# MasterNobody/x264vfw

Hardware: AMD Instinct MI355X
Metric: 1080p yuv420p frames/sec at preset=medium as the device runs it (see config.toolset_gaps), hot path on MI355X (higher is better)
Workload: dtype u8

## Files before the change

include/x264gpu.h:

```cpp
#ifndef X264GPU_H
#define X264GPU_H
#include <stdint.h>
#include <stddef.h>

#ifdef __cplusplus
extern "C" {
#endif

#define X264GPU_ABI_VERSION 2
enum { X264GPU_OK = 0, X264GPU_EINVAL = -1, X264GPU_EHIP = -2, X264GPU_ENOMEM = -3, X264GPU_ENODEV = -4 };

int  x264gpu_abi_version(void);
int  x264gpu_device_count(void);
int  x264gpu_set_device(int dev);
int  x264gpu_get_device(int *dev);
const char *x264gpu_last_error(void);
int  x264gpu_malloc(void **d_ptr, size_t bytes);
int  x264gpu_free(void *d_ptr);
int  x264gpu_memcpy_h2d(void *d_dst, const void *h_src, size_t bytes, void *stream);
int  x264gpu_memcpy_d2h(void *h_dst, const void *d_src, size_t bytes, void *stream);
int  x264gpu_memcpy_d2d(void *d_dst, const void *d_src, size_t bytes, void *stream);
int  x264gpu_memset(void *d_dst, int value, size_t bytes, void *stream);
int  x264gpu_stream_sync(void *stream);
int  x264gpu_stream_create(void **stream);
int  x264gpu_stream_destroy(void *stream);
int  x264gpu_event_create(void **event);
int  x264gpu_event_destroy(void *event);
int  x264gpu_event_record(void *event, void *stream);
int  x264gpu_event_sync(void *event);
int  x264gpu_stream_wait_event(void *stream, void *event);

int x264gpu_pixel_metric(int metric, const uint8_t *d_a, const uint8_t *d_b, int n, int w, int h,
                         int32_t *d_out, void *stream);
int x264gpu_pixel_var(const uint8_t *d_a, int n, int w, int h, uint64_t *d_out, void *stream);
int x264gpu_pixel_hadamard_ac(const uint8_t *d_a, int n, int w, int h, uint64_t *d_out, void *stream);

int x264gpu_dctq4x4(const uint8_t *d_enc, const uint8_t *d_pred, int n, int qp, int list,
                    int16_t *d_coef, int16_t *d_levels, uint8_t *d_recon, void *stream);
int x264gpu_dctq8x8(const uint8_t *d_enc, const uint8_t *d_pred, int n, int qp, int list,
                    int16_t *d_coef, int16_t *d_levels, uint8_t *d_recon, void *stream);

int x264gpu_intra_predict(int kind, const uint8_t *d_plane, int stride, const int32_t *d_xy,
                          const int32_t *d_mode, const int32_t *d_avail, int n, uint8_t *d_out, void *stream);

int x264gpu_hpel_filter(uint8_t *d_planes, size_t plane_bytes, int stride, int w, int h, int pad, void *stream);
int x264gpu_lowres(const uint8_t *d_src, int ss, int w, int h, uint8_t *d_dst, size_t plane_bytes, int ds,
                   void *stream);
int x264gpu_mc_luma(const uint8_t *d_planes00, size_t plane_bytes, int stride, const int32_t *d_xy,
                    const int32_t *d_mv, int n, int w, int h, uint8_t *d_out, void *stream);
int x264gpu_mc_chroma(const uint8_t *d_nv12_00, int stride, const int32_t *d_xy, const int32_t *d_mv,
                      int n, int w, int h, uint8_t *d_out, void *stream);
int x264gpu_mc_avg(const uint8_t *d_a, const uint8_t *d_b, size_t bytes, int weight1, uint8_t *d_out, void *stream);
int x264gpu_trellis_blocks(const int16_t *d_coefs, int nblk, int cat, int qp, int intra, const uint8_t *d_states460, int16_t *d_levels, uint8_t *d_nz, void *stream);
int x264gpu_trellis_blocks_ex(const int16_t *d_coefs, int nblk, int cat, int qp, int intra, const uint8_t *d_states460, int16_t *d_levels, uint8_t *d_nz, int force_general,
                              uint8_t *d_paths, void *stream);
int x264gpu_trellis_blocks_psy(const int16_t *d_coefs, const int16_t *d_fenc_dct, int nblk, int cat, int qp, int intra, int psy_trellis_q8, const uint8_t *d_states460,
                               int16_t *d_levels, uint8_t *d_nz, int force_general, uint8_t *d_paths, void *stream);
int x264gpu_mc_weight(const uint8_t *d_src, size_t bytes, int scale, int denom, int offset, uint8_t *d_out, void *stream);
int x264gpu_gather_rows(const void *const *d_rows, size_t row_bytes, void *d_dst, int rows, void *stream);
int x264gpu_cabac_level_walk(const int16_t *d_levels, const int32_t *d_what, int n, const uint32_t *d_r, const uint32_t *d_r8, uint32_t *d_r_out, uint32_t *d_r8_out, int32_t *d_bits, void *stream);

enum { X264GPU_CSP_MASK = 0xff, X264GPU_CSP_I420 = 1, X264GPU_CSP_YV12 = 2, X264GPU_CSP_YV16 = 3, X264GPU_CSP_YV24 = 4,
       X264GPU_CSP_NV12 = 5, X264GPU_CSP_YUYV = 6, X264GPU_CSP_UYVY = 7, X264GPU_CSP_BGR = 8, X264GPU_CSP_BGRA = 9,
       X264GPU_CSP_VFLIP = 0x1000 };
long x264gpu_csp_img_fill(int csp, int width, int height, long off[3], int stride[3]);
int x264gpu_csp_to_i420(const uint8_t *const d_src[3], const int src_stride[3], int csp, int width, int height,
                        int colmatrix709, int fullrange, uint8_t *const d_dst[3], const int dst_stride[3], void *stream);
int x264gpu_csp_to_i420_batch(const uint8_t *const d_src[3], const int src_stride[3], size_t src_frame_bytes, int csp, int width,
                              int height, int colmatrix709, int fullrange, uint8_t *const d_dst[3], const int dst_stride[3],
                              size_t dst_frame_bytes, int frames, void *stream);

enum { X264GPU_MB_I4x4 = 0, X264GPU_MB_I8x8 = 1, X264GPU_MB_I16x16 = 2, X264GPU_MB_P_L0 = 4, X264GPU_MB_P_8x8 = 5,
       X264GPU_MB_P_SKIP = 6,
       X264GPU_MB_B_DIRECT = 7, X264GPU_MB_B_SKIP = 8, X264GPU_MB_B_INTER = 9, X264GPU_MB_B_8x8 = 10 };
enum { X264GPU_SLICE_P = 0, X264GPU_SLICE_B = 1, X264GPU_SLICE_I = 2 ,
       X264GPU_SLICE_I_NONIDR = 3  };

typedef struct x264gpu_mb {
    uint8_t  type;
    union {
    uint8_t  i16_mode;
    uint8_t  direct8;
    };
    uint8_t  chroma_mode;
    uint8_t  qp;
    uint8_t  cbp_luma;
    uint8_t  cbp_chroma;
    uint8_t  partition;
    int8_t   ref[4];
    union {
    uint8_t  i4_mode[16];
    int8_t   ref1[4];
    };
    uint8_t  transform8x8;
    int16_t  mv[4][2];
    uint32_t nnz;
    union {
    struct {
    int32_t  cost;
    int32_t  aux[3];
    };
    int16_t  mv1[4][2];
    };
} x264gpu_mb;

#define X264GPU_MB_LEVELS 416
#define X264GPU_LV_LUMA 0
#define X264GPU_LV_LUMA_DC 256
#define X264GPU_LV_CHROMA_DC 272
#define X264GPU_LV_CHROMA_AC 280

typedef struct x264gpu_encoder x264gpu_encoder;

typedef struct x264gpu_config {
    int width, height;
    int streams;
    int refs;
    int qp_i, qp_p;
    int me_range;
    int subme;
    int deblock;
    int deblock_alpha, deblock_beta;
    int chroma_qp_offset;
    int deadzone_inter, deadzone_intra;
    int dct_decimate;
    int partitions;
    int dct8x8;
    int me_method;
    int chroma_me;
    int mixed_refs;
    int aq_mode;
    float aq_strength;
    int fast_pskip;
    int mv_range;
    int cabac;
    int rd;
    int psy;
    int psy_rd_q8;
    int slices;
    int trellis;
    int slices_plain;
    int dpb;
    int weightb;
    int psy_trellis_q8;
} x264gpu_config;

#define X264GPU_MAX_LIST 8
typedef struct x264gpu_pic {
    int slice_type;
    int qp;
    int poc;
    int dst;
    int keep;
    int nref[2];
    int8_t slot[2][X264GPU_MAX_LIST];
    struct { int8_t on, denom; int16_t scale, offset; } wl0[X264GPU_MAX_LIST];
    int blind_dupe;
    float qpm;
    struct { int8_t on[2], denom, pad; int16_t scale[2], offset[2]; } wc0[X264GPU_MAX_LIST];
    int direct_temporal, direct_auto;
} x264gpu_pic;

int  x264gpu_encoder_direct_scores(x264gpu_encoder *enc, int *h_scores);
int  x264gpu_encoder_create(x264gpu_encoder **enc, const x264gpu_config *cfg);
int  x264gpu_encoder_create_view(x264gpu_encoder **enc, x264gpu_encoder *parent);
void x264gpu_encoder_destroy(x264gpu_encoder *enc);
int  x264gpu_encoder_mb_count(const x264gpu_encoder *enc);
int  x264gpu_encode_frames(x264gpu_encoder *enc, const uint8_t *d_i420, int slice_type,
                           x264gpu_mb *d_mb, int16_t *d_levels, void *stream);
int  x264gpu_encode_pictures(x264gpu_encoder *enc, const uint8_t *d_i420, const x264gpu_pic *pics,
                             x264gpu_mb *d_mb, int16_t *d_levels, void *stream);
typedef struct x264gpu_level_index { uint32_t at, groups; } x264gpu_level_index;
int  x264gpu_pack_levels(int16_t *d_levels, int streams, int mb_count, x264gpu_level_index *d_index, uint32_t *d_kept , void *stream);
int x264gpu_encoder_deblock_pictures(x264gpu_encoder *e, const uint8_t *d_i420, const x264gpu_mb *d_mb, uint8_t *d_out, void *stream);
int  x264gpu_encoder_get_recon(x264gpu_encoder *enc, int stream_idx, uint8_t *d_i420_out, void *stream);
int  x264gpu_encoder_get_recon_slot(x264gpu_encoder *enc, int stream_idx, int slot, uint8_t *d_i420_out, void *stream);
typedef struct x264gpu_quality { uint64_t ssd[3]; double ssim_sum; uint32_t ssim_cnt, pad; } x264gpu_quality;
#define X264GPU_QUALITY_PSNR 1
#define X264GPU_QUALITY_SSIM 2
int x264gpu_picture_quality(const uint8_t *d_a, const uint8_t *d_b, int n, int w, int h, int flags, x264gpu_quality *d_out, void *stream);
int x264gpu_encoder_quality(x264gpu_encoder *enc, int flags, x264gpu_quality *d_out , void *stream);
typedef struct x264gpu_nr_offsets { uint16_t off[3][64]; } x264gpu_nr_offsets;
typedef struct x264gpu_nr_sums { uint64_t sum[3][64]; uint32_t count[3], pad; } x264gpu_nr_sums;
int x264gpu_encoder_set_nr(x264gpu_encoder *enc, const x264gpu_nr_offsets *d_off , x264gpu_nr_sums *d_pic );
int x264gpu_nr_update(x264gpu_nr_offsets *d_off, x264gpu_nr_sums *d_state, const x264gpu_nr_sums *d_pic, int streams, int strength, void *stream);
int x264gpu_denoise_blocks(int16_t *d_coefs, int nblk, int cat, const x264gpu_nr_offsets *d_off, x264gpu_nr_sums *d_out, void *stream);
int  x264gpu_encoder_stage_count(void);
const char *x264gpu_encoder_stage_name(int i);
int  x264gpu_encoder_profile_begin(x264gpu_encoder *enc, int max_calls);
int  x264gpu_encoder_set_debug(x264gpu_encoder *enc, void *d_counters);
int  x264gpu_mb_kernels_seen(uint32_t *ids, int max, int reset);
int  x264gpu_encoder_profile_end(x264gpu_encoder *enc, void *stream, double *ms_sum, int *launches);
int  x264gpu_encoder_set_qp(x264gpu_encoder *enc, int qp_i, int qp_p);
int  x264gpu_encoder_set_mb_qp_offsets(x264gpu_encoder *enc, const float *d_offsets);
int  x264gpu_encoder_set_stream_qps(x264gpu_encoder *enc, const int8_t *qps);
int  x264gpu_encoder_set_stream_qpms(x264gpu_encoder *enc, const int8_t *qps, const float *qpms);
int  x264gpu_encoder_set_qpm(x264gpu_encoder *enc, float qpm);
int  x264gpu_encoder_set_lowres_mvs(x264gpu_encoder *enc, const int16_t *d_mvs);
int  x264gpu_encoder_set_lowres_mvs1(x264gpu_encoder *enc, const int16_t *d_mvs);
int  x264gpu_encoder_cabac_states(x264gpu_encoder *enc, int stream, int slice, uint8_t *out460);

typedef struct x264gpu_slicetype x264gpu_slicetype;
int  x264gpu_slicetype_create(x264gpu_slicetype **st, int width, int height, int streams, int slots, int bframes, int me_method, int subme, int me_range,
                              int weightb, int mv_range, int do_edges );
void x264gpu_slicetype_destroy(x264gpu_slicetype *st);
int  x264gpu_slicetype_put_frame(x264gpu_slicetype *st, int slot, const uint8_t *d_i420, void *stream);
int  x264gpu_slicetype_frame_cost(x264gpu_slicetype *st, int slot_p0, int slot_p1, int slot_b, int d0, int d1, int32_t *h_score, void *stream);
int  x264gpu_slicetype_frame_cost_w(x264gpu_slicetype *st, int slot_p0, int slot_p1, int slot_b, int d0, int d1, int on, int scale, int denom, int offset, int32_t *h_score, void *stream);
int  x264gpu_slicetype_intra_mbs(x264gpu_slicetype *st, int slot, int d0, int stream_idx);
int  x264gpu_slicetype_cost_est(x264gpu_slicetype *st, int slot, int d0, int d1, int stream_idx);
const int16_t  *x264gpu_slicetype_lowres_mvs(x264gpu_slicetype *st, int slot, int list, int dist);
const int      *x264gpu_slicetype_lowres_mv_costs(x264gpu_slicetype *st, int slot, int list, int dist);
const int      *x264gpu_slicetype_intra_costs(x264gpu_slicetype *st, int slot);
// ... 31 lines not shown
```

x264vfw_amd/csrc/cabac_layout.hip.h:

```cpp
#pragma once

namespace x264gpu {

__host__ __device__ inline bool cab_locate(int ctx, int &reg, int &lane, int &sh)
{
    const int sig_off[6] = { 105, 120, 134, 149, 152, 402 }, last_off[6] = { 166, 181, 195, 210, 213, 417 }, abs_off[6] = { 227, 237, 247, 257, 266, 426 };
    const int n_sig[6] = { 15, 14, 15, 3, 14, 15 }, n_last[6] = { 15, 14, 15, 3, 14, 9 }, n_abs[6] = { 10, 10, 10, 9, 10, 10 }, byte_of[6] = { 3, 1, 0, 3, 2, 0 };
    if (ctx < 105) { reg = 0; lane = ctx >> 2; sh = (ctx & 3) * 8; return true; }
    if (ctx >= 399 && ctx <= 401) { const int c = ctx - 399 + 105; reg = 0; lane = c >> 2; sh = (c & 3) * 8; return true; }
    for (int cat = 0; cat < 6; cat++) {
        int role = -1, i = 0;
        if (ctx >= sig_off[cat] && ctx < sig_off[cat] + n_sig[cat]) { role = 0; i = ctx - sig_off[cat]; }
        else if (ctx >= last_off[cat] && ctx < last_off[cat] + n_last[cat]) { role = 1; i = ctx - last_off[cat]; }
        else if (ctx >= abs_off[cat] && ctx < abs_off[cat] + n_abs[cat]) { role = 2; i = ctx - abs_off[cat]; }
        if (role < 0) continue;
        reg = cat == 5 ? 2 : 1; sh = 8 * byte_of[cat];
        lane = cat == 3 ? (role == 0 ? 48 + i : role == 1 ? 52 + i : 55 + i) : role * 16 + i;
        return true;
    }
    return false;
}

}
```

x264vfw_amd/csrc/cabac_rd.hip.h:

```cpp
#pragma once
#include <type_traits>
#include "enc_common.hip.h"
#include "cabac_layout.hip.h"
#define CABAC_TABLE static __constant__ const
#define CABAC_NAMESPACE x264gpu_cabac
#include "../host/cabac_tables.hpp"
#undef CABAC_TABLE
#undef CABAC_NAMESPACE

#ifndef CAB_WALK_BINS
#define CAB_WALK_BINS 8
#endif
namespace x264gpu {

static __constant__ const uint16_t c_cabac_entropy[128] = {
#include "cabac_entropy.inc"
};

struct Cab { uint32_t a, r, r8; int f8; int f8v; };

__device__ __forceinline__ uint32_t cab_model(int lane)
{
    return (uint32_t)c_cabac_entropy[2 * lane] | ((uint32_t)c_cabac_entropy[2 * lane + 1] << 9) | ((uint32_t)x264gpu_cabac::cabac_trans_lps[lane] << 20);
}

__device__ __forceinline__ int cab_total(const Cab &cb) { return cb.f8 + wave_sum(cb.f8v); }

__device__ __forceinline__ void cab_init(Cab &cb, int lane, bool pslice, int qp)
{
    namespace T = x264gpu_cabac;
    qp = min(max(qp, 0), 51);
    uint32_t w[3] = { 0, 0, 0 };
    auto seed = [&](int ctx) {
        int m = 0, n = 0;
        if (ctx < 276) { const T::CabacInitRow row = T::cabac_init_0_275[ctx]; m = pslice ? row.mp : row.mi; n = pslice ? row.np : row.ni; }
        else { const T::CabacInitRow row = T::cabac_init_399_435[ctx - 399]; m = pslice ? row.mp : row.mi; n = pslice ? row.np : row.ni; }
        const int pre = min(max(((m * qp) >> 4) + n, 1), 126);
        return (uint32_t)(pre <= 63 ? (63 - pre) << 1 : ((pre - 64) << 1) | 1);
    };
    for (int j = 0; j < 4; j++) {
        const int c = lane * 4 + j;
        if (c < 105) w[0] |= seed(c) << (8 * j); else if (c < 108) w[0] |= seed(399 + c - 105) << (8 * j);
    }
    {
        const int role = lane >> 4, i = lane & 15;
        const int sig_off[5] = { 105, 120, 134, 149, 152 }, last_off[5] = { 166, 181, 195, 210, 213 }, abs_off[5] = { 227, 237, 247, 257, 266 }, n1[5] = { 15, 14, 15, 3, 14 };
        const int cats[3] = { 2, 1, 4 };
        for (int b = 0; b < 3; b++) {
            const int cat = cats[b];
            if (role == 0 && i < n1[cat]) w[1] |= seed(sig_off[cat] + i) << (8 * b);
            else if (role == 1 && i < n1[cat]) w[1] |= seed(last_off[cat] + i) << (8 * b);
            else if (role == 2 && i < 10) w[1] |= seed(abs_off[cat] + i) << (8 * b);
        }
        if (lane < 48) {
            if (role == 0 && i < 15) w[1] |= seed(105 + i) << 24; else if (role == 1 && i < 15) w[1] |= seed(166 + i) << 24; else if (role == 2 && i < 10) w[1] |= seed(227 + i) << 24;
        } else {
            const int l = lane - 48;
            if (l < 3) w[1] |= seed(149 + l) << 24; else if (l >= 4 && l < 7) w[1] |= seed(210 + l - 4) << 24; else if (l >= 7) w[1] |= seed(257 + l - 7) << 24;
        }
        if (role == 0 && i < 15) w[2] = seed(402 + i); else if (role == 1 && i < 9) w[2] = seed(417 + i); else if (role == 2 && i < 10) w[2] = seed(426 + i);
    }
    cb.a = w[0]; cb.r = w[1]; cb.r8 = w[2]; cb.f8 = 0; cb.f8v = 0;
}

__device__ __forceinline__ void cab_bin(Cab &cb, uint32_t model, int lane, int ctx, int bin)
{
    ctx = __builtin_amdgcn_readfirstlane(ctx >= 399 ? ctx - 399 + 105 : ctx); bin = __builtin_amdgcn_readfirstlane(bin);
    const int li = ctx >> 2, sh = (ctx & 3) * 8;
    const uint32_t w = __builtin_amdgcn_readlane(cb.a, li);
    const int st = (w >> sh) & 255, sg = st >> 1, mps = st & 1;
    const uint32_t t = __builtin_amdgcn_readlane(model, sg);
    const bool lps = (mps ^ bin) != 0;
    cb.f8 += lps ? (t >> 9) & 0x7ff : t & 0x1ff;
    const int ns = lps ? (int)(t >> 20) : min(sg + 1, 62);
    const int nm = lps && sg == 0 ? mps ^ 1 : mps;
    const uint32_t nw = (w & ~(255u << sh)) | ((uint32_t)((ns << 1) | nm) << sh);
    cb.a = lane == li ? nw : cb.a;
}
__device__ __forceinline__ void cab_bypass(Cab &cb, int n = 1) { cb.f8 += 256 * n; }
__device__ __forceinline__ void cab_ue_bypass(Cab &cb, int k, int v)
{
    int n = 0;
    while (v >= (1 << k)) { n++; v -= 1 << k; k++; }
    cb.f8 += 256 * (n + 1 + k);
}

__device__ __forceinline__ void cab_step(int &st, int &f8v, uint32_t model, bool mine, int bin)
{
    const int sg = st >> 1, mps = st & 1;
    const uint32_t t = (uint32_t)__builtin_amdgcn_ds_bpermute(sg << 2, (int)model);
    const bool lps = (mps ^ bin) != 0;
    const int cost = lps ? (t >> 9) & 0x7ff : t & 0x1ff;
    const int ns = lps ? (int)(t >> 20) : min(sg + 1, 62);
    const int nm = lps && sg == 0 ? mps ^ 1 : mps;
    f8v += mine ? cost : 0;
    st = mine ? (ns << 1) | nm : st;
}

struct CabLv {
    int cat0;
    unsigned nz0;
    unsigned nzac;
    unsigned nzdc;
    bool ldc;
};

__device__ __forceinline__ int wave_scan_add(int v)
{
    v += __builtin_amdgcn_update_dpp(0, v, 0x111, 0xf, 0xf, false);
    v += __builtin_amdgcn_update_dpp(0, v, 0x112, 0xf, 0xf, false);
    v += __builtin_amdgcn_update_dpp(0, v, 0x114, 0xf, 0xf, false);
    v += __builtin_amdgcn_update_dpp(0, v, 0x118, 0xf, 0xf, false);
    v += __builtin_amdgcn_update_dpp(0, v, 0x142, 0xa, 0xf, false);
    v += __builtin_amdgcn_update_dpp(0, v, 0x143, 0xc, 0xf, false);
    return v;
}
__device__ __forceinline__ int cab_mbcnt(unsigned long long m) { return (int)__builtin_amdgcn_mbcnt_hi((unsigned)(m >> 32), __builtin_amdgcn_mbcnt_lo((unsigned)m, 0u)); }

#define CAB_CHAIN_ENTRIES (511 * 128)
template <int LN>
__device__ __forceinline__ void cab_writelane3(unsigned &lo, unsigned &hi, int &n, unsigned long long val, int nval)
{
    asm("s_nop 1\n\tv_writelane_b32 %0, %3, %6\n\tv_writelane_b32 %1, %4, %6\n\tv_writelane_b32 %2, %5, %6"
        : "+v"(lo), "+v"(hi), "+v"(n) : "s"((unsigned)val), "s"((unsigned)(val >> 32)), "s"(nval), "n"(LN));
}
struct CabChain { int sg, mps; };
__device__ __forceinline__ void cab_run_mps(CabChain &c, int &f8, int cumv, int m62, int n)
{
    const int hi = min(c.sg + n, 62);
    f8 += __builtin_amdgcn_readlane(cumv, hi) - __builtin_amdgcn_readlane(cumv, c.sg) + (c.sg + n - hi) * m62;
    c.sg = hi;
}
__device__ __forceinline__ void cab_one_lps(CabChain &c, int &f8, uint32_t model)
{
    const uint32_t t = (uint32_t)__builtin_amdgcn_readlane((int)model, c.sg);
    f8 += (int)((t >> 9) & 0x7ff);
    c.mps ^= c.sg == 0 ? 1 : 0;
    c.sg = (int)(t >> 20);
}

template <int LANE0, class PROF>
__device__ __forceinline__ void cab_strings_c1(int a, int c1, unsigned &blo, unsigned &bhi, int &N, PROF &pf)
{
    unsigned long long cur[5];
    int pushed[5];
#pragma unroll
    for (int v = 0; v < 5; v++) {
        const bool member = a != 0 && c1 == v;
        cur[v] = __ballot(member);
        pushed[v] = __builtin_amdgcn_ds_permute((member ? cab_mbcnt(cur[v]) : 63) << 2, member && a > 1 ? 1 : 0);
    }
    if (cur[0]) { pf.count(20); cab_writelane3<LANE0 + 0>(blo, bhi, N, __ballot(pushed[0] != 0), __builtin_popcountll(cur[0])); }
    if (cur[1]) { pf.count(20); cab_writelane3<LANE0 + 1>(blo, bhi, N, __ballot(pushed[1] != 0), __builtin_popcountll(cur[1])); }
    if (cur[2]) { pf.count(20); cab_writelane3<LANE0 + 2>(blo, bhi, N, __ballot(pushed[2] != 0), __builtin_popcountll(cur[2])); }
    if (cur[3]) { pf.count(20); cab_writelane3<LANE0 + 3>(blo, bhi, N, __ballot(pushed[3] != 0), __builtin_popcountll(cur[3])); }
    if (cur[4]) { pf.count(20); cab_writelane3<LANE0 + 4>(blo, bhi, N, __ballot(pushed[4] != 0), __builtin_popcountll(cur[4])); }
}
template <int LANE0, int V, class PROF>
__device__ __forceinline__ void cab_strings_cg(int a, int a15, int cg, unsigned &blo, unsigned &bhi, int &N, unsigned long long &serial, PROF &pf)
{
    const bool member = a > 1 && cg == V;
    if (__ballot(member)) {
        pf.count(20);
        const int incl = wave_scan_add(member ? (a15 < 15 ? a15 - 1 : 13) : 0);
        const int total = __builtin_amdgcn_readlane(incl, 63);
        if (total <= 63) {
            const bool closes = member && a15 < 15;
            const int pushed = __builtin_amdgcn_ds_permute((closes ? incl - 1 : 63) << 2, closes ? 1 : 0);
            cab_writelane3<LANE0 + V>(blo, bhi, N, ((1ull << total) - 1ull) & ~__ballot(pushed != 0), total);
        } else serial |= 1ull << (V - 5);
    }
    if constexpr (V < 9 && LANE0 + V + 1 < 64) cab_strings_cg<LANE0, V + 1>(a, a15, cg, blo, bhi, N, serial, pf);
}

template <class PROF>
__device__ __forceinline__ void cab_levels_all(Cab &cb, uint32_t model, int lane, const int16_t *lvs, const CabLv &W, const uint32_t *ctab, PROF &pf)
{
    if (W.cat0 < 0 && !W.nzac && !W.nzdc && !W.ldc) return;
    lane = relane(lane);
    const int cumv = wave_scan_add((int)(model & 0x1ff)) - (int)(model & 0x1ff);
    const int m62 = (int)(__builtin_amdgcn_readlane((int)model, 62) & 0x1ff);
    int f8 = 0;
    auto group = [&](auto a_of, int nwords, unsigned wordmask, int gshift, uint32_t &reg, int sh, auto lane0_tag, int bac, int ncm1, int sigbase, int lastbase) {
        constexpr int LANE0 = decltype(lane0_tag)::value;
        for (int w = 0; w < nwords; w++) {
            if (!((wordmask >> w) & 1u)) continue;
            const int a = a_of(w);
            const unsigned long long nzm = __ballot(a != 0);
            if (!nzm) continue;
            const unsigned long long m1 = __ballot(a == 1), mg = nzm & ~m1;
            int ngt, n1;
            if (gshift == 6) { ngt = cab_mbcnt(mg); n1 = cab_mbcnt(m1); }
            else {
                const int base = lane & ~((1 << gshift) - 1);
                const unsigned sel = (1u << (lane - base)) - 1u;
                ngt = __builtin_popcount((unsigned)(mg >> base) & sel); n1 = __builtin_popcount((unsigned)(m1 >> base) & sel);
            }
            const int node = ngt == 0 ? min(n1, 3) : min(3 + ngt, 7);
            const int c1 = node < 4 ? node + 1 : 0, cg = node < 4 ? 5 : node + 2;
            cb.f8v += a ? 256 + (a >= 15 ? 256 * (2 * (31 - __builtin_clz(a - 14)) + 1) : 0) : 0;
            const int a15 = min(a, 15);
            pf.count(21, __builtin_popcountll(nzm));
            unsigned blo = 0, bhi = 0; int N = 0;
            cab_strings_c1<LANE0>(a, c1, blo, bhi, N, pf);
            unsigned long long serial = 0;
            if (mg) cab_strings_cg<LANE0, 5>(a, a15, cg, blo, bhi, N, serial, pf);
            if (ncm1) {
                const int nslots = 1 << gshift;
                const bool is_s = lane >= sigbase && lane < sigbase + ncm1, is_l = lane >= lastbase && lane < lastbase + ncm1;
                const int pp = is_s ? lane - sigbase : lane - lastbase;
                const int sbit = min(max(nslots - 1 - (pp + bac), 0), 31);
                for (int j = 0; j < (gshift == 4 ? 4 : gshift == 2 ? 2 : 1); j++) {
                    const unsigned field = (unsigned)(nzm >> (j * nslots)) & ((1u << nslots) - 1u);
                    if (!field) continue;
                    const int lastp = nslots - 1 - __builtin_ctz(field) - bac;
                    const unsigned nzb = (field >> sbit) & 1u;
                    const bool cond = is_s ? pp <= lastp : is_l && nzb && pp <= lastp;
                    const unsigned bit = is_s ? nzb : (pp == lastp ? 1u : 0u);
                    blo |= cond ? bit << N : 0u; N += cond ? 1 : 0;
                }
            }
            {
                int st = (int)((reg >> sh) & 255u);
                unsigned long long B = ((unsigned long long)bhi << 32) | blo;
                while (__ballot(N > 0)) {
                    const int k = min(N, CAB_WALK_BINS);
                    const uint32_t e = ctab[((((1 << k) - 1) + ((int)(unsigned)B & ((1 << k) - 1))) << 7) + st];
                    st = (int)(e & 127u); cb.f8v += (int)(e >> 7);
                    B >>= k; N -= k;
                }
                reg = (reg & ~(255u << sh)) | ((uint32_t)st << sh);
            }
            for (int v = 5; serial && v < 10; v++) {
                if (!((serial >> (v - 5)) & 1ull)) continue;
                unsigned long long cur = __ballot(a > 1 && cg == v);
                const int stv = (__builtin_amdgcn_readlane((int)reg, LANE0 + v) >> sh) & 255;
                CabChain c = { stv >> 1, stv & 1 };
                while (cur) {
                    pf.count(20);
                    const int f = __builtin_ctzll(cur);
                    cur &= cur - 1ull;
                    const int av = __builtin_amdgcn_readlane(a15, f);
                    int ones = av - 2;
                    while (ones > 0) {
                        if (c.mps) { cab_run_mps(c, f8, cumv, m62, ones); ones = 0; }
                        else { cab_one_lps(c, f8, model); ones--; }
                    }
                    if (av != 15) { if (c.mps) cab_one_lps(c, f8, model); else cab_run_mps(c, f8, cumv, m62, 1); }
                }
                const uint32_t nst = (uint32_t)((c.sg << 1) | c.mps);
                reg = lane == LANE0 + v ? (reg & ~(255u << sh)) | (nst << sh) : reg;
            }
        }
    };
    const int g = lane >> 4, q = lane & 15;
    if (W.cat0 == 5)
        group([&](int w) { const int pos = 63 - lane; return abs((int)lvs[(w * 4 + (pos & 3)) * 16 + (pos >> 2)]); }, 4, W.nz0 & 15u, 6, cb.r8, 0, std::integral_constant<int, 32>{}, 0, 0, 0, 0);
    else if (W.cat0 >= 0) {
        const bool ac = W.cat0 == 1;
        const unsigned wm = ((W.nz0 & 0xfu) ? 1u : 0u) | ((W.nz0 & 0xf0u) ? 2u : 0u) | ((W.nz0 & 0xf00u) ? 4u : 0u) | ((W.nz0 & 0xf000u) ? 8u : 0u);
        group([&](int w) { const int blk = 4 * w + g, pos = 15 - q; return ((W.nz0 >> blk) & 1u) && !(ac && pos == 0) ? abs((int)lvs[blk * 16 + pos]) : 0; }, 4, wm, 4, cb.r, ac ? 8 : 0, std::integral_constant<int, 32>{}, ac ? 1 : 0, ac ? 14 : 15, 0, 16);
    }
    if (W.ldc) group([&](int) { return lane < 16 ? abs((int)lvs[X264GPU_LV_LUMA_DC + 15 - lane]) : 0; }, 1, 1u, 4, cb.r, 24, std::integral_constant<int, 32>{}, 0, 15, 0, 16);
    if (W.nzdc) group([&](int) { return lane < 8 && ((W.nzdc >> (lane >> 2)) & 1u) ? abs((int)lvs[X264GPU_LV_CHROMA_DC + (lane >> 2) * 4 + 3 - (lane & 3)]) : 0; }, 1, 1u, 2, cb.r, 24, std::integral_constant<int, 55>{}, 0, 3, 48, 52);
    if (W.nzac) {
        const unsigned wm = ((W.nzac & 0xfu) ? 1u : 0u) | ((W.nzac & 0xf0u) ? 2u : 0u);
        group([&](int w) { const int blk = 4 * w + g, pos = 15 - q; return ((W.nzac >> blk) & 1u) && pos ? abs((int)lvs[X264GPU_LV_CHROMA_AC + blk * 16 + pos]) : 0; }, 2, wm, 4, cb.r, 16, std::integral_constant<int, 32>{}, 1, 14, 0, 16);
    }
    cb.f8 += f8;
}

template <int CAT>
__device__ __forceinline__ void cab_block4(Cab &cb, int &st, uint32_t model, int lane, int coef)
{
    constexpr int n1 = CAT == 3 ? 3 : (CAT == 1 || CAT == 4) ? 14 : 15;
    constexpr int sig0 = CAT == 3 ? 48 : 0, last0 = CAT == 3 ? 52 : 16;
    const unsigned long long mask = __ballot(coef != 0);
    const int last = 63 - __builtin_clzll(mask);
    const bool is_s = lane >= sig0 && lane < sig0 + n1, is_l = lane >= last0 && lane < last0 + n1;
    const int p = is_s ? lane - sig0 : lane - last0;
    const int nzp = (int)((mask >> (p & 63)) & 1);
    cab_step(st, cb.f8v, model, (is_s && p <= last) || (is_l && nzp && p <= last), is_s ? nzp : p == last);
}

static __constant__ const unsigned long long c_cabac_pos8[24] = {
#include "cabac_masks8x8.inc"
};

__device__ __forceinline__ void cab_block8(Cab &cb, int &st, uint32_t model, int lane, int coef, bool size)
{
    const unsigned long long mask = __ballot(coef != 0);
    const int last = 63 - __builtin_clzll(mask);
    const unsigned long long upto = last < 63 ? (2ull << last) - 1 : 0x7fffffffffffffffull;
    unsigned long long mine = 0;
    if (lane < 15) mine = c_cabac_pos8[lane] & upto;
    else if (lane >= 16 && lane < 25) mine = c_cabac_pos8[15 + lane - 16] & upto & mask;
    while (__ballot(mine != 0)) {
        const bool have = mine != 0;
        const int i = have ? (size ? 63 - __builtin_clzll(mine) : __builtin_ctzll(mine)) : 0;
        cab_step(st, cb.f8v, model, have, lane < 15 ? (int)((mask >> i) & 1) : i == last);
        mine &= ~(1ull << i);
    }
}

struct CabIn {
    bool pslice, left, top, size;
    int nref, t8mode;
    int type, part, t8, cbp_luma, cbp_chroma, i16mode, cmode, qp, last_qp, last_dqp;
    unsigned nnz;
    int ltype, ttype, lcbp_luma, tcbp_luma, lcbp_chroma, tcbp_chroma, lcmode, tcmode, lt8, tt8;
    unsigned lnnz, tnnz;
    unsigned long long lamvd, tamvd;
    bool bslice; int nref1; unsigned buse;
    int b_r0, b_x0, b_y0, b_r1, b_x1, b_y1;
    unsigned long long lamvd1, tamvd1;
    int pm, pm_b0, pm_b1, pm_dx, pm_dy, pm_sx, pm_sy;
    int pm_lists, pm_dx1, pm_dy1, pm_sx1, pm_sy1;
    unsigned pm_nnzc;
};

static __constant__ const uint8_t c_btype_len[24] = { 1, 3, 3, 6, 6, 6, 6, 6, 6, 6, 6, 6, 7, 7, 7, 7, 7, 7, 7, 7, 7, 7, 6, 6 };
static __constant__ const uint8_t c_btype_bits[24] = { 0, 1, 5, 3, 35, 19, 51, 11, 43, 27, 59, 31, 7, 71, 39, 103, 23, 87, 55, 119, 15, 79, 63, 47 };
__device__ __forceinline__ bool cab_is_skip(int t) { return t == X264GPU_MB_P_SKIP || t == X264GPU_MB_B_SKIP; }
__device__ __forceinline__ bool cab_is_intra(int t) { return t < X264GPU_MB_P_L0; }

__device__ __forceinline__ int cab_luma_cbf_of(int type, int cbp_luma, int t8, unsigned nnz, int bx, int by)
{
    if (type == X264GPU_MB_P_SKIP || type == X264GPU_MB_B_SKIP) return 0;
    if (!((cbp_luma >> ((by >> 1) * 2 + (bx >> 1))) & 1)) return 0;
    if (t8) return 1;
    return (nnz >> blkidx_of(bx, by)) & 1;
}

__device__ __forceinline__ void cab_mb_type_intra(Cab &cb, uint32_t model, int lane, const CabIn &in, int c0, int c1, int c2, int c3, int c4, int c5)
{
    if (in.type != X264GPU_MB_I16x16) { cab_bin(cb, model, lane, c0, 0); return; }
    cab_bin(cb, model, lane, c0, 1);
    if (in.size) cb.f8 += 7;
    cab_bin(cb, model, lane, c1, in.cbp_luma != 0);
    if (!in.cbp_chroma) cab_bin(cb, model, lane, c2, 0);
    else { cab_bin(cb, model, lane, c2, 1); cab_bin(cb, model, lane, c3, in.cbp_chroma >> 1); }
    cab_bin(cb, model, lane, c4, in.i16mode >> 1);
    cab_bin(cb, model, lane, c5, in.i16mode & 1);
}

__device__ __forceinline__ void cab_mvd(Cab &cb, uint32_t model, int lane, int base, int sum, int val)
{
    const int a = abs(val), inc = (sum > 2) + (sum > 32);
    if (!a) { cab_bin(cb, model, lane, base + inc, 0); return; }
    cab_bin(cb, model, lane, base + inc, 1);
    for (int i = 1; i < min(a, 9); i++) cab_bin(cb, model, lane, base + min(i + 2, 6), 1);
    if (a < 9) cab_bin(cb, model, lane, base + min(a + 2, 6), 0); else cab_ue_bypass(cb, 3, a - 9);
    cab_bypass(cb);
}

template <class PROF>
__device__ __forceinline__ unsigned long long cab_mb(Cab &cb, uint32_t model, int lane, const CabIn &in, MeState &S, const int16_t *lvs,
                                                     const uint8_t *modes4, const uint8_t *modes8, const uint8_t *nmodes, int mbx, int sy, int &dqp_out,
                                                     unsigned long long &amvd1_out, const uint32_t *ctab, PROF &pf)
{
    pf.begin2(); pf.count(16);
    lane = relane(lane);
    amvd1_out = 0;
    unsigned long long amvd = 0;
    dqp_out = 0;
    const bool lavail = in.left, tavail = in.top;
    const bool intra = in.type < X264GPU_MB_P_L0;
    if (!in.pm) {
    if (in.bslice && !in.size) {
        cab_bin(cb, model, lane, 24 + (lavail && !cab_is_skip(in.ltype)) + (tavail && !cab_is_skip(in.ttype)), in.type == X264GPU_MB_B_SKIP);
        if (in.type == X264GPU_MB_B_SKIP) return 0;
    }
    if (in.pslice && !in.bslice && !in.size) {
        cab_bin(cb, model, lane, 11 + (lavail && in.ltype != X264GPU_MB_P_SKIP) + (tavail && in.ttype != X264GPU_MB_P_SKIP), in.type == X264GPU_MB_P_SKIP);
        if (in.type == X264GPU_MB_P_SKIP) return 0;
    }
    if (in.bslice) {
        const int ctx0 = (lavail && in.ltype != X264GPU_MB_B_SKIP && in.ltype != X264GPU_MB_B_DIRECT) + (tavail && in.ttype != X264GPU_MB_B_SKIP && in.ttype != X264GPU_MB_B_DIRECT);
        int value;
        if (intra) value = 23;
        else if (in.type == X264GPU_MB_B_DIRECT) value = 0;
        else if (in.part == D_8x8) value = 22;
        else if (in.part == D_16x16) value = 1 + (int)(in.buse & 3);
        else {
            const int u0 = (int)(in.buse & 3), u1 = (int)((in.part == D_16x8 ? in.buse >> 4 : in.buse >> 2) & 3);
            const int pair = u0 == 0 ? (u1 == 0 ? 0 : u1 == 1 ? 2 : 4) : u0 == 1 ? (u1 == 0 ? 3 : u1 == 1 ? 1 : 5) : 6 + u1;
            value = 4 + 2 * pair + (in.part == D_8x16);
        }
        const int len = c_btype_len[value], bits = c_btype_bits[value];
        for (int i = 0; i < len; i++) cab_bin(cb, model, lane, i == 0 ? 27 + ctx0 : i == 1 ? 27 + 3 : i == 2 ? 27 + 5 - ((bits >> 1) & 1) : 27 + 5, (bits >> i) & 1);
        if (intra) cab_mb_type_intra(cb, model, lane, in, 32, 32 + 1, 32 + 2, 32 + 2, 32 + 3, 32 + 3);
    } else if (!in.pslice) {
        const int ctx = (lavail && in.ltype != X264GPU_MB_I4x4 && in.ltype != X264GPU_MB_I8x8) + (tavail && in.ttype != X264GPU_MB_I4x4 && in.ttype != X264GPU_MB_I8x8);
        cab_mb_type_intra(cb, model, lane, in, 3 + ctx, 3 + 3, 3 + 4, 3 + 5, 3 + 6, 3 + 7);
    } else if (intra) { cab_bin(cb, model, lane, 14, 1); cab_mb_type_intra(cb, model, lane, in, 17, 17 + 1, 17 + 2, 17 + 2, 17 + 3, 17 + 3); }
    else if (in.part == D_8x8) { cab_bin(cb, model, lane, 14, 0); cab_bin(cb, model, lane, 15, 0); cab_bin(cb, model, lane, 16, 1); }
    else {
        cab_bin(cb, model, lane, 14, 0);
        if (in.part == D_16x16) { cab_bin(cb, model, lane, 15, 0); cab_bin(cb, model, lane, 16, 0); }
        else { cab_bin(cb, model, lane, 15, 1); cab_bin(cb, model, lane, 17, in.part == D_16x8); }
    }
    }
    const int t8ctx = 399 + (lavail && in.lt8) + (tavail && in.tt8);
    if (in.pm == 1) {
        if (in.pm_lists & 1) { cab_mvd(cb, model, lane, 40, in.pm_sx, in.pm_dx); cab_mvd(cb, model, lane, 47, in.pm_sy, in.pm_dy); }
        if (in.pm_lists & 2) { cab_mvd(cb, model, lane, 40, in.pm_sx1, in.pm_dx1); cab_mvd(cb, model, lane, 47, in.pm_sy1, in.pm_dy1); }
        if (in.part == D_8x8 && !in.bslice) cab_bin(cb, model, lane, 21, 1);
    } else if (intra) {
        if (in.type != X264GPU_MB_I16x16 && (!in.pm || in.pm == 2 || in.pm == 3)) {
            const bool i8 = in.type == X264GPU_MB_I8x8;
            if (in.t8mode && !in.pm) cab_bin(cb, model, lane, t8ctx, i8);
            int mode = 0, pm = 0;
            if (lane < 16) { const uint8_t *cur = i8 ? modes8 : modes4; mode = cur[lane]; pm = i4_pred_mode(nmodes, mbx, sy, lane, cur); }
            const uint32_t w68 = __builtin_amdgcn_readlane(cb.a, 68 >> 2);
            int stp = lane == 0 ? (int)(w68 & 255) : (int)((w68 >> 8) & 255);
            for (int b = 0; b < 16; b += i8 ? 4 : 1) {
                if (in.pm && b != (i8 ? 4 * in.pm_b0 : in.pm_b0)) continue;
                int m = __builtin_amdgcn_readlane(mode, b);
                const int p = __builtin_amdgcn_readlane(pm, b);
                const bool same = m == p;
                if (m > p) m--;
                cab_step(stp, cb.f8v, model, lane == 0 || (lane == 1 && !same), lane == 0 ? same : m & 1);
                if (!same) { cab_step(stp, cb.f8v, model, lane == 1, (m >> 1) & 1); cab_step(stp, cb.f8v, model, lane == 1, m >> 2); }
            }
            {
                const uint32_t s68 = (uint32_t)__builtin_amdgcn_readlane(stp, 0), s69 = (uint32_t)__builtin_amdgcn_readlane(stp, 1);
                cb.a = lane == (68 >> 2) ? (cb.a & ~0xffffu) | s68 | (s69 << 8) : cb.a;
            }
        }
        if (!in.pm || in.pm == 4) {
        const int ctx = (lavail && in.ltype < X264GPU_MB_P_L0 && in.lcmode != 0) + (tavail && in.ttype < X264GPU_MB_P_L0 && in.tcmode != 0);
        if (!in.cmode) cab_bin(cb, model, lane, 64 + ctx, 0);
        else { cab_bin(cb, model, lane, 64 + ctx, 1); cab_bin(cb, model, lane, 64 + 3, in.cmode > 1); if (in.cmode > 1) cab_bin(cb, model, lane, 64 + 3, in.cmode > 2); }
        }
    } else if (in.bslice) {
        if (in.type != X264GPU_MB_B_DIRECT) {
            const int part = in.part, np = part == D_16x16 ? 1 : part == D_8x8 ? 4 : 2;
            const int w8 = part == D_16x16 || part == D_16x8 ? 2 : 1, h8 = part == D_16x16 || part == D_8x16 ? 2 : 1;
            auto use_of = [&](int kp) { const int b8 = part == D_16x8 ? 2 * kp : kp; return (int)((in.buse >> (2 * b8)) & 3); };
            if (part == D_8x8)
                for (int kp = 0; kp < 4; kp++) {
                    const int u = use_of(kp);
                    if (u == 3) { cab_bin(cb, model, lane, 36, 0); continue; }
                    cab_bin(cb, model, lane, 36, 1);
                    if (u == 2) { cab_bin(cb, model, lane, 37, 1); cab_bin(cb, model, lane, 38, 0); cab_bin(cb, model, lane, 39, 0); cab_bin(cb, model, lane, 39, 0); }
                    else { cab_bin(cb, model, lane, 37, 0); cab_bin(cb, model, lane, 39, u == 1); }
                }
            const int sc0 = S.cref, sc1 = S.cmvx, sc2 = S.cmvy, sc3 = S.cdir;
            for (int l = 0; l < 2; l++) {
                const int go = 16 * l;
                if ((l ? in.nref1 : in.nref) <= 1) continue;
                if (lane == 5 + go || lane == 6 + go || lane == 9 + go || lane == 10 + go) S.cref = -2;
                for (int kp = 0; kp < np; kp++) {
                    const int x8 = part == D_8x16 ? kp : part == D_8x8 ? kp & 1 : 0, y8 = part == D_16x8 ? kp : part == D_8x8 ? kp >> 1 : 0;
                    const int u = use_of(kp), b8 = y8 * 2 + x8, g0 = (y8 + 1) * 4 + x8 + 1 + go;
                    const bool sends = u == 2 || u == l;
                    const int r = rl(l ? in.b_r1 : in.b_r0, b8 * 16);
                    if (sends) {
                        int ctx = (rl(S.cref, g0 - 1) > 0 && !rl(S.cdir, g0 - 1)) + 2 * (rl(S.cref, g0 - 4) > 0 && !rl(S.cdir, g0 - 4));
                        for (int q = r; q > 0; q--) { cab_bin(cb, model, lane, 54 + ctx, 1); ctx = (ctx >> 2) + 4; }
                        cab_bin(cb, model, lane, 54 + ctx, 0);
                    }
                    const bool mine = lane == g0 || (w8 == 2 && lane == g0 + 1) || (h8 == 2 && lane == g0 + 4) || (w8 == 2 && h8 == 2 && lane == g0 + 5);
                    S.cref = mine ? (sends ? r : u == 3 ? r : -1) : S.cref;
                    S.cdir = mine ? (u == 3) : S.cdir;
                }
            }
            unsigned long long amvd1 = 0;
            for (int l = 0; l < 2; l++) {
                const int go = 16 * l;
                if (lane == 5 + go || lane == 6 + go || lane == 9 + go || lane == 10 + go) S.cref = -2;
                unsigned long long am = 0;
                const unsigned long long nl = l ? in.lamvd1 : in.lamvd, nt = l ? in.tamvd1 : in.tamvd;
                for (int kp = 0; kp < np; kp++) {
                    const int x8 = part == D_8x16 ? kp : part == D_8x8 ? kp & 1 : 0, y8 = part == D_16x8 ? kp : part == D_8x8 ? kp >> 1 : 0;
                    const int u = use_of(kp), b8 = y8 * 2 + x8, g0 = (y8 + 1) * 4 + x8 + 1 + go;
                    const bool sends = u == 2 || u == l;
                    const int r = rl(l ? in.b_r1 : in.b_r0, b8 * 16), vx = rl(l ? in.b_x1 : in.b_x0, b8 * 16), vy = rl(l ? in.b_y1 : in.b_y0, b8 * 16);
                    if (sends) {
                        int px, py;
                        mb_predict_mv(S, part, x8, y8, w8, r, px, py, go);
                        for (int comp = 0; comp < 2; comp++) {
                            const int la = x8 > 0 ? (int)((am >> (8 * ((y8 * 2 + x8 - 1) * 2 + comp))) & 255) : lavail ? (int)((nl >> (8 * ((y8 * 2 + 1) * 2 + comp))) & 255) : 0;
                            const int ta = y8 > 0 ? (int)((am >> (8 * (((y8 - 1) * 2 + x8) * 2 + comp))) & 255) : tavail ? (int)((nt >> (8 * ((2 + x8) * 2 + comp))) & 255) : 0;
                            const int d = comp ? vy - py : vx - px;
                            cab_mvd(cb, model, lane, comp ? 47 : 40, la + ta, d);
                            const unsigned long long capped = (unsigned long long)min(abs(d), 66);
                            for (int yy = y8; yy < y8 + h8; yy++) for (int xx = x8; xx < x8 + w8; xx++) am |= capped << (8 * ((yy * 2 + xx) * 2 + comp));
                        }
                    }
                    const bool mine = lane == g0 || (w8 == 2 && lane == g0 + 1) || (h8 == 2 && lane == g0 + 4) || (w8 == 2 && h8 == 2 && lane == g0 + 5);
                    S.cref = mine ? (r >= 0 ? r : -1) : S.cref; S.cmvx = mine ? (r >= 0 ? vx : 0) : S.cmvx; S.cmvy = mine ? (r >= 0 ? vy : 0) : S.cmvy;
                }
                if (l) amvd1 = am; else amvd = am;
            }
            S.cref = sc0; S.cmvx = sc1; S.cmvy = sc2; S.cdir = sc3;
            amvd1_out = amvd1;
        }
    } else {
        const int part = in.part, np = part == D_16x16 ? 1 : part == D_8x8 ? 4 : 2;
        const int w8 = part == D_16x16 || part == D_16x8 ? 2 : 1, h8 = part == D_16x16 || part == D_8x16 ? 2 : 1;
        if (part == D_8x8) for (int kp = 0; kp < 4; kp++) cab_bin(cb, model, lane, 21, 1);
        const int sc0 = S.cref, sc1 = S.cmvx, sc2 = S.cmvy;
        if (lane == 5 || lane == 6 || lane == 9 || lane == 10) S.cref = -2;
        if (in.nref > 1)
            for (int kp = 0; kp < np; kp++) {
                const int x8 = part == D_8x16 ? kp : part == D_8x8 ? kp & 1 : 0, y8 = part == D_16x8 ? kp : part == D_8x8 ? kp >> 1 : 0;
                const int slot = part == D_16x16 ? ME_16 : part == D_16x8 ? ME_16x8 + kp : part == D_8x16 ? ME_8x16 + kp : ME_8 + kp;
                const int r = rl(S.ref, slot), g0 = (y8 + 1) * 4 + x8 + 1;
                int ctx = (rl(S.cref, g0 - 1) > 0) + 2 * (rl(S.cref, g0 - 4) > 0);
                for (int q = r; q > 0; q--) { cab_bin(cb, model, lane, 54 + ctx, 1); ctx = (ctx >> 2) + 4; }
                cab_bin(cb, model, lane, 54 + ctx, 0);
                const bool mine = lane == g0 || (w8 == 2 && lane == g0 + 1) || (h8 == 2 && lane == g0 + 4) || (w8 == 2 && h8 == 2 && lane == g0 + 5);
                S.cref = mine ? r : S.cref;
            }
        else if (lane == 5 || lane == 6 || lane == 9 || lane == 10) S.cref = 0;
        for (int kp = 0; kp < np; kp++) {
            const int x8 = part == D_8x16 ? kp : part == D_8x8 ? kp & 1 : 0, y8 = part == D_16x8 ? kp : part == D_8x8 ? kp >> 1 : 0;
            const int slot = part == D_16x16 ? ME_16 : part == D_16x8 ? ME_16x8 + kp : part == D_8x16 ? ME_8x16 + kp : ME_8 + kp;
            const int r = rl(S.ref, slot), vx = rl(S.mvx, slot), vy = rl(S.mvy, slot), g0 = (y8 + 1) * 4 + x8 + 1;
            int px, py;
            mb_predict_mv(S, part, x8, y8, w8, r, px, py);
            for (int comp = 0; comp < 2; comp++) {
                const int la = x8 > 0 ? (int)((amvd >> (8 * ((y8 * 2 + x8 - 1) * 2 + comp))) & 255) : lavail ? (int)((in.lamvd >> (8 * ((y8 * 2 + 1) * 2 + comp))) & 255) : 0;
                const int ta = y8 > 0 ? (int)((amvd >> (8 * (((y8 - 1) * 2 + x8) * 2 + comp))) & 255) : tavail ? (int)((in.tamvd >> (8 * ((2 + x8) * 2 + comp))) & 255) : 0;
                const int d = comp ? vy - py : vx - px;
                cab_mvd(cb, model, lane, comp ? 47 : 40, la + ta, d);
                const unsigned long long capped = (unsigned long long)min(abs(d), 66);
                for (int yy = y8; yy < y8 + h8; yy++) for (int xx = x8; xx < x8 + w8; xx++) amvd |= capped << (8 * ((yy * 2 + xx) * 2 + comp));
            }
            const bool mine = lane == g0 || (w8 == 2 && lane == g0 + 1) || (h8 == 2 && lane == g0 + 4) || (w8 == 2 && h8 == 2 && lane == g0 + 5);
            S.cmvx = mine ? vx : S.cmvx; S.cmvy = mine ? vy : S.cmvy;
        }
        S.cref = sc0; S.cmvx = sc1; S.cmvy = sc2;
    }
    if (in.pm ? in.pm == 3 : in.type != X264GPU_MB_I16x16)
        for (int b8 = 0; b8 < 4; b8++) {
            const int x = b8 & 1, y = b8 >> 1;
            const int a = x ? !((in.cbp_luma >> (b8 - 1)) & 1) : lavail ? !((in.lcbp_luma >> (b8 + 1)) & 1) : 0;
            const int b = y ? !((in.cbp_luma >> (b8 - 2)) & 1) : tavail ? !((in.tcbp_luma >> (b8 + 2)) & 1) : 0;
            cab_bin(cb, model, lane, 73 + a + 2 * b, (in.cbp_luma >> b8) & 1);
        }
    if (in.pm ? in.pm == 4 : in.type != X264GPU_MB_I16x16) {
        cab_bin(cb, model, lane, 77 + (lavail && in.lcbp_chroma) + 2 * (tavail && in.tcbp_chroma), in.cbp_chroma != 0);
        if (in.cbp_chroma) cab_bin(cb, model, lane, 77 + 4 + (lavail && in.lcbp_chroma == 2) + 2 * (tavail && in.tcbp_chroma == 2), in.cbp_chroma == 2);
    }
    if (!in.pm && !intra && in.t8mode && in.cbp_luma) cab_bin(cb, model, lane, t8ctx, in.t8);
    if (in.pm || in.cbp_luma || in.cbp_chroma || in.type == X264GPU_MB_I16x16) {
        const bool i16 = !in.pm && in.type == X264GPU_MB_I16x16;
        int dqp = in.qp - in.last_qp;
        if (i16 && !in.cbp_luma && !in.cbp_chroma && !((in.nnz >> 24) & 1) && dqp > 0) dqp = 0;
        if (!in.pm) {
        int ctx = in.last_dqp != 0;
        if (dqp) {
            if (dqp < -26) dqp += 52; else if (dqp > 25) dqp -= 52;
            int val = dqp > 0 ? 2 * dqp - 1 : -2 * dqp;
            do { cab_bin(cb, model, lane, 60 + ctx, 1); ctx = 2 + (ctx >> 1); } while (--val);
        }
        cab_bin(cb, model, lane, 60 + ctx, 0);
        dqp_out = dqp;
        }
        pf.mark2(17);
        const int un = intra ? 1 : 0;
        auto luma_in = [&](int bx, int by) { return in.pm ? (int)((in.pm_nnzc >> blkidx_of(bx, by)) & 1) : cab_luma_cbf_of(in.type, in.cbp_luma, in.t8, in.nnz, bx, by); };
        auto luma_inc = [&](int blk) {
            const int bx = z_bx(blk), by = z_by(blk);
            const int a = bx > 0 ? luma_in(bx - 1, by) : lavail ? cab_luma_cbf_of(in.ltype, in.lcbp_luma, in.lt8, in.lnnz, 3, by) : un;
            const int b = by > 0 ? luma_in(bx, by - 1) : tavail ? cab_luma_cbf_of(in.ttype, in.tcbp_luma, in.tt8, in.tnnz, bx, 3) : un;
            return a + 2 * b;
        };
        auto dc_inc = [&](int bit) {
            auto of = [&](bool avail, int type, int cbp_chroma, unsigned nnz) {
                if (!avail) return un;
                if (cab_is_skip(type)) return 0;
                if (bit == 24) return type == X264GPU_MB_I16x16 ? (int)((nnz >> 24) & 1) : 0;
                return cbp_chroma ? (int)((nnz >> bit) & 1) : 0;
            };
            return of(lavail, in.ltype, in.lcbp_chroma, in.lnnz) + 2 * of(tavail, in.ttype, in.tcbp_chroma, in.tnnz);
        };
        auto ac_inc = [&](int pl, int i) {
            const int bx = i & 1, by = i >> 1;
            auto of = [&](int type, int cbp_chroma, unsigned nnz, int x, int y) { return !cab_is_skip(type) && cbp_chroma == 2 ? (int)((nnz >> (16 + pl * 4 + y * 2 + x)) & 1) : 0; };
            auto inside = [&](int x, int y) { return in.pm ? (int)((in.pm_nnzc >> (16 + pl * 4 + y * 2 + x)) & 1) : of(in.type, in.cbp_chroma, in.nnz, x, y); };
            const int a = bx > 0 ? inside(0, by) : lavail ? of(in.ltype, in.lcbp_chroma, in.lnnz, 1, by) : un;
            const int b = by > 0 ? inside(bx, 0) : tavail ? of(in.ttype, in.tcbp_chroma, in.tnnz, bx, 1) : un;
            return a + 2 * b;
        };
        CabLv W = { -1, 0u, 0u, 0u, false };
        auto flush_levels = [&]() { pf.mark2(18); cab_levels_all(cb, model, lane, lvs, W, ctab, pf); pf.mark2(19); W.cat0 = -1; W.nz0 = 0; W.nzac = 0; W.nzdc = 0; W.ldc = false; };
        auto blocks = [&](auto cat_tag, int shift, int nblk, auto coef_of, auto inc_of, auto coded) {
            constexpr int CAT = decltype(cat_tag)::value;
            static_assert(CAT == 0 || CAT == 3, "the DC categories");
            (void)shift;
            for (int b = 0; b < nblk; b++) {
                if (!coded(b)) continue;
                const int coef = coef_of(b);
                const bool nz = __ballot(coef != 0) != 0;
                cab_bin(cb, model, lane, 85 + CAT * 4 + inc_of(b), nz);
                if (nz) { if (CAT == 0) W.ldc = true; else W.nzdc |= 1u << b; }
            }
        };
        auto always = [](int) { return true; };
        auto blocks_many = [&](auto cat_tag, int shift, int nblk, unsigned codedmask, unsigned nzbits, auto coef_of, auto inc_of) {
            constexpr int CAT = decltype(cat_tag)::value;
            const int b_lane = lane & 15;
            const bool mine_blk = lane < nblk && ((codedmask >> b_lane) & 1);
            const int inc = inc_of(b_lane);
            const unsigned long long nzm = (unsigned long long)(nzbits & codedmask);
            unsigned long long seq = 0;
#pragma unroll
            for (int j = 0; j < 4; j++) { const unsigned long long m = __ballot(mine_blk && inc == j); seq = lane == j ? m : seq; }
            const int cbase = 85 + CAT * 4;
            int stc = 0;
#pragma unroll
            for (int j = 0; j < 4; j++) { const int c = cbase + j; const uint32_t w = __builtin_amdgcn_readlane(cb.a, c >> 2); stc = lane == j ? (int)((w >> ((c & 3) * 8)) & 255) : stc; }
            while (__ballot(seq != 0)) {
                const bool have = seq != 0;
                const int b = have ? __builtin_ctzll(seq) : 0;
                cab_step(stc, cb.f8v, model, have, (int)((nzm >> b) & 1));
                seq &= seq - 1;
            }
#pragma unroll
            for (int j = 0; j < 4; j++) {
                const int c = cbase + j, li = c >> 2, sh = (c & 3) * 8;
                const uint32_t v = (uint32_t)__builtin_amdgcn_readlane(stc, j);
                cb.a = lane == li ? (cb.a & ~(255u << sh)) | (v << sh) : cb.a;
            }
            (void)coef_of; (void)shift;
            if (CAT == 4) W.nzac |= (unsigned)nzm; else { W.cat0 = CAT; W.nz0 |= (unsigned)nzm; }
        };
        if (i16) {
            blocks(std::integral_constant<int, 0>{}, 24, 1, [&](int) { return lane < 16 ? (int)lvs[X264GPU_LV_LUMA_DC + lane] : 0; }, [&](int) { return dc_inc(24); }, always);
            if (in.cbp_luma) blocks_many(std::integral_constant<int, 1>{}, 8, 16, 0xffffu, in.nnz & 0xffffu, [&](int b) { return lane < 15 ? (int)lvs[b * 16 + 1 + lane] : 0; }, luma_inc);
        } else if (in.pm == 4) {
        } else if (in.t8) {
            const int pmask = in.pm ? (1 << in.pm_b0) | (in.pm_b1 >= 0 ? 1 << in.pm_b1 : 0) : 15;
            int st = cb.r8 & 255;
            for (int i8 = 0; i8 < 4; i8++)
                if (((in.cbp_luma & pmask) >> i8) & 1) cab_block8(cb, st, model, lane, (int)lvs[(i8 * 4 + (lane & 3)) * 16 + (lane >> 2)], in.size);
            cb.r8 = (uint32_t)st;
            W.cat0 = 5; W.nz0 = (unsigned)(in.cbp_luma & pmask);
        } else {
            unsigned coded = ((in.cbp_luma & 1) ? 0x000fu : 0) | ((in.cbp_luma & 2) ? 0x00f0u : 0) | ((in.cbp_luma & 4) ? 0x0f00u : 0) | ((in.cbp_luma & 8) ? 0xf000u : 0);
            if (in.pm == 1) coded &= (0xfu << (4 * in.pm_b0)) | (in.pm_b1 >= 0 ? 0xfu << (4 * in.pm_b1) : 0u);
            if (in.pm == 2) coded = 1u << in.pm_b0;
            blocks_many(std::integral_constant<int, 2>{}, 0, 16, coded, in.nnz & 0xffffu, [&](int b) { return lane < 16 ? (int)lvs[b * 16 + lane] : 0; }, luma_inc);
        }
        if (in.pm == 1) {
            for (int t = 0; t < 2; t++) {
                const int b8 = t ? in.pm_b1 : in.pm_b0;
                if (b8 < 0) continue;
                blocks_many(std::integral_constant<int, 4>{}, 16, 8, (1u << b8) | (16u << b8), (in.nnz >> 16) & 0xffu, [&](int k) { return lane < 15 ? (int)lvs[X264GPU_LV_CHROMA_AC + k * 16 + 1 + lane] : 0; }, [&](int k) { return ac_inc((k >> 2) & 1, k & 3); });
                flush_levels();
            }
        } else if (in.cbp_chroma && (!in.pm || in.pm == 4)) {
            blocks(std::integral_constant<int, 3>{}, 24, 2, [&](int pl) { return lane < 4 ? (int)lvs[X264GPU_LV_CHROMA_DC + pl * 4 + lane] : 0; }, [&](int pl) { return dc_inc(25 + pl); }, always);
            if (in.cbp_chroma == 2)
                blocks_many(std::integral_constant<int, 4>{}, 16, 8, 0xffu, (in.nnz >> 16) & 0xffu, [&](int k) { return lane < 15 ? (int)lvs[X264GPU_LV_CHROMA_AC + k * 16 + 1 + lane] : 0; }, [&](int k) { return ac_inc((k >> 2) & 1, k & 3); });
        }
        flush_levels();
    }
    return amvd;
}

}
```

x264vfw_amd/csrc/encoder.hip:

```cpp
#include "enc_common.hip.h"
#include "k_encode.hip.h"
#include <stdlib.h>
#include "k_deblock.hip.h"
#include "cabac_layout.hip.h"
#include "quality.hip.h"
#include <math.h>
#include <vector>
#include <string.h>
#include <new>

namespace x264gpu {
void launch_mb_slice_dia(const EncK &k, int streams, bool big_margin, hipStream_t st);
void launch_mb_slice_hex(const EncK &k, int streams, bool big_margin, hipStream_t st);
void launch_mb_slice_umh(const EncK &k, int streams, bool big_margin, hipStream_t st);
void launch_mb_slice_esa(const EncK &k, int streams, bool big_margin, hipStream_t st);
void launch_mb_slice_intra(const EncK &k, int streams, hipStream_t st);
void launch_mb_slice_b_hex(const EncK &k, int streams, hipStream_t st);
void launch_mb_slice_b_dia(const EncK &k, int streams, hipStream_t st);
void launch_mb_slice_b_umh(const EncK &k, int streams, hipStream_t st);
void launch_mb_slice_b_esa(const EncK &k, int streams, hipStream_t st);
void launch_mb_slice_psy(const EncK &k, int streams, int slice_type, hipStream_t st);
void launch_mb_slice_nr(const EncK &k, int streams, int slice_type, hipStream_t st);
void launch_nr_gather(const x264gpu_nr_sums *part, int slices, x264gpu_nr_sums *pic, int streams, hipStream_t st);
int trellis_table_ptrs(const uint16_t **su, const uint8_t **tu, const int **l2);
int cabac_chain_table(const uint32_t **out);
int launch_hpel_filter(uint8_t *planes, size_t plane_bytes, int stride, int w, int h, int pad, int batch,
                       size_t batch_bytes, hipStream_t st);
}
using namespace x264gpu;

struct x264gpu_encoder {
    x264gpu_config cfg;
    EncK k;
    uint8_t *fenc_y = nullptr, *fenc_uv = nullptr;
    uint8_t *luma[8] = {}, *chroma[8] = {};
    int slots = 2, have = 0;
    int16_t *mv16[8] = {};
    uint8_t *mbtype[8] = {};
    int8_t *colref[8] = {}; int16_t *colmv[8] = {};
    int8_t *colref0[8] = {};
    struct DpbMeta { int slot_l0poc[8][8] = {}; int slot_nref[8] = {}, slot_poc[8] = {}, slot_ref0poc[8] = {}; } meta_own, *meta = &meta_own;
    x264gpu_encoder *view_of = nullptr;
    hipStream_t last_stream = nullptr;
    uint8_t *direct_flags = nullptr, *direct_flags_base = nullptr; int direct_flags_sel = 0; int *dscore = nullptr; bool use_direct_flags = false;
    int16_t *mvr[8] = {};
    int poc = 0, ring = 2;
    const int16_t *lowres_mv = nullptr, *lowres_mv1 = nullptr;
    int cur = 0, last = 0;
    unsigned long long *dbg = nullptr;
    uint8_t *tc = nullptr;
    uint8_t *amvd = nullptr;
    uint32_t *cab_out = nullptr;
    int *perm = nullptr; unsigned *wtime = nullptr; bool wt_valid[4] = { false, false, false, false };
    int *sl_stat = nullptr, *sl_rerun = nullptr;
    unsigned long long *prof = nullptr;
    int *wf_progress = nullptr;
    void *qslab = nullptr;
    const x264gpu_nr_offsets *nr_off = nullptr; x264gpu_nr_sums *nr_pic = nullptr, *nr_part = nullptr;
    uint8_t *mbqp = nullptr;
    const float *ext_off = nullptr;
    int8_t *stream_qp = nullptr; float *stream_qpm = nullptr;
    int stream_qp_sel = 0;
    bool use_stream_qp = false;
    float qpm_next = 0.f;
    Q4 *q4tab = nullptr; Q8 *q8tab = nullptr; int *lambda_tab = nullptr; uint16_t *cost_all = nullptr;
    hipEvent_t *ev = nullptr;
    int *ev_mask = nullptr;
    int prof_calls = 0, prof_cap = 0;
};
enum { NSTAGE = 6 };

static const char *const kStageNames[] = { "ingest", "macroblocks", "unused", "settle_qp", "deblock", "hpel_filter" };

static int build_aq_tables(x264gpu_encoder *e)
{
    QuantCfg qc; qc.deadzone_inter = e->cfg.deadzone_inter; qc.deadzone_intra = e->cfg.deadzone_intra;
    std::vector<Q4> q4(52 * 4); std::vector<Q8> q8(52 * 2); std::vector<int> lam(52);
    std::vector<uint16_t> cost((size_t)52 * 2 * MVCOST_HALF);
    for (int qp = 0; qp < 52; qp++) {
        for (int l = 0; l < 4; l++) q4[qp * 4 + l] = make_q4(qp, l, qc);
        for (int l = 0; l < 2; l++) q8[qp * 2 + l] = make_q8(qp, l, qc);
        lam[qp] = lambda_of(qp);
        uint16_t *h = cost.data() + (size_t)qp * 2 * MVCOST_HALF;
        for (int i = 0; i < MVCOST_HALF; i++) {
            const float logs = i ? log2f((float)(i + 1)) * 2.0f + 1.718f : 0.718f;
            int c = (int)((float)lam[qp] * logs + 0.5f);
            if (c > 65535) c = 65535;
            h[MVCOST_HALF + i] = (uint16_t)c; h[MVCOST_HALF - i] = (uint16_t)c;
        }
        h[0] = h[1];
    }
    hipError_t er = hipMalloc((void **)&e->q4tab, q4.size() * sizeof(Q4));
    if (er == hipSuccess) er = hipMalloc((void **)&e->q8tab, q8.size() * sizeof(Q8));
    if (er == hipSuccess) er = hipMalloc((void **)&e->lambda_tab, lam.size() * sizeof(int));
    if (er == hipSuccess) er = hipMalloc((void **)&e->cost_all, cost.size() * sizeof(uint16_t));
    if (er == hipSuccess) er = hipMalloc((void **)&e->mbqp, (size_t)e->cfg.streams * e->k.nmb);
    if (er == hipSuccess) er = hipMemcpy(e->q4tab, q4.data(), q4.size() * sizeof(Q4), hipMemcpyHostToDevice);
    if (er == hipSuccess) er = hipMemcpy(e->q8tab, q8.data(), q8.size() * sizeof(Q8), hipMemcpyHostToDevice);
    if (er == hipSuccess) er = hipMemcpy(e->lambda_tab, lam.data(), lam.size() * sizeof(int), hipMemcpyHostToDevice);
    if (er == hipSuccess) er = hipMemcpy(e->cost_all, cost.data(), cost.size() * sizeof(uint16_t), hipMemcpyHostToDevice);
    if (er != hipSuccess) return set_err(er == hipErrorOutOfMemory ? X264GPU_ENOMEM : X264GPU_EHIP, "aq tables", er);
    return X264GPU_OK;
}

extern "C" {

static int encoder_create_impl(x264gpu_encoder **out, const x264gpu_config *cfg, x264gpu_encoder *parent)
{
    ARG_TRY(out && cfg);
    ARG_TRY(cfg->width >= 16 && cfg->height >= 16 && !(cfg->width & 1) && !(cfg->height & 1) && cfg->streams >= 1);
    ARG_TRY(cfg->qp_i >= 0 && cfg->qp_i <= 51 && cfg->qp_p >= 0 && cfg->qp_p <= 51 && cfg->refs >= 1 && cfg->refs <= 5);
    ARG_TRY(cfg->trellis == 0 || (cfg->trellis > 0 && cfg->trellis < 128 && (cfg->trellis & 63) && cfg->rd && cfg->cabac));
    ARG_TRY(cfg->psy_trellis_q8 == 0 || (cfg->psy_trellis_q8 > 0 && cfg->psy_trellis_q8 <= 640 && cfg->trellis && cfg->cabac && cfg->rd && (cfg->me_method == 1 || cfg->me_method == 2)));
    ARG_TRY(!cfg->rd || (cfg->subme >= 6 && cfg->subme <= 9 && cfg->psy_rd_q8 >= 0 && cfg->psy_rd_q8 <= 2560));
    ARG_TRY(cfg->rd >= 0 && cfg->rd < 128 && (cfg->rd < 2 || (cfg->rd & 1)) && (!(cfg->rd & 62) || (cfg->cabac && cfg->subme >= 8 && (cfg->me_method == 1 || cfg->me_method == 2))));
    ARG_TRY(!cfg->rd || cfg->subme < 8 || (cfg->cabac && (cfg->me_method == 1 || cfg->me_method == 2)));
    ARG_TRY(!(cfg->rd & 64) || (cfg->cabac && (cfg->me_method == 1 || cfg->me_method == 2)));
    ARG_TRY(cfg->dpb == 0 || cfg->subme < 9 || (cfg->rd && cfg->cabac && (cfg->me_method == 1 || cfg->me_method == 2)));
    ARG_TRY(cfg->slices >= 0 && (cfg->slices <= 1 || cfg->slices <= (cfg->height + 15) / 16 / (cfg->slices_plain ? 1 : 4)));
    ARG_TRY(cfg->slices_plain == 0 || cfg->slices_plain == 1);
    ARG_TRY(cfg->width <= 4096 && cfg->height <= 2304 && cfg->me_range >= 4 && cfg->me_range <= (cfg->me_method == 2 ? 64 : 16));
    ARG_TRY(cfg->me_method >= 0 && cfg->me_method <= 3);
    ARG_TRY(cfg->dpb == 0 || (cfg->dpb >= cfg->refs && cfg->dpb <= 7));
    x264gpu_encoder *e = new (std::nothrow) x264gpu_encoder();
    if (!e) return set_err(X264GPU_ENOMEM, "encoder", hipSuccess);
    e->cfg = *cfg;
    EncK &k = e->k;
    memset(&k, 0, sizeof(k));
    k.w = cfg->width; k.h = cfg->height;
    k.mbw = (k.w + 15) / 16; k.mbh = (k.h + 15) / 16; k.nmb = k.mbw * k.mbh;
    k.cw = k.mbw * 16; k.ch = k.mbh * 16;
    k.fs = (k.cw + 63) / 64 * 64;
    k.rs = (k.cw + 2 * PAD + 63) / 64 * 64;
    k.fency_bytes = (size_t)k.fs * k.ch;
    k.fencuv_bytes = (size_t)k.fs * k.ch / 2;
    k.plane_bytes = (size_t)k.rs * (k.ch + 2 * PAD);
    k.luma_bytes = 4 * k.plane_bytes;
    k.cplane_bytes = (size_t)k.rs * (k.ch / 2 + 2 * CPAD);
    k.me_range = cfg->me_range; k.subme = cfg->subme; k.dct_decimate = cfg->dct_decimate;
    k.slices = cfg->slices > 1 ? cfg->slices : 1; k.slices_plain = cfg->slices_plain != 0; k.cabac = cfg->cabac != 0;
    k.rd = cfg->rd; k.psy = cfg->psy != 0; k.psy_rd_q8 = cfg->psy_rd_q8;
    k.partitions = cfg->partitions; k.chroma_qp_offset = cfg->chroma_qp_offset; k.dct8x8 = cfg->dct8x8; k.me_method = cfg->me_method; k.chroma_me = cfg->chroma_me != 0; k.mixed_refs = cfg->mixed_refs != 0;
    k.alpha_off = cfg->deblock_alpha * 2; k.beta_off = cfg->deblock_beta * 2;
    k.deblock_rdo = cfg->deblock && (cfg->rd & 64) ? 1 : 0;
    const size_t S = (size_t)cfg->streams;
    hipError_t er = hipSuccess;
    auto alloc = [&](void **p, size_t n, int fill) {
        if (er != hipSuccess) return;
        er = hipMalloc(p, n);
        if (er == hipSuccess) er = hipMemset(*p, fill, n);
    };
    alloc((void **)&e->fenc_y, S * k.fency_bytes, 0);
    alloc((void **)&e->fenc_uv, S * k.fencuv_bytes, 0);
    e->slots = (cfg->dpb > 0 ? cfg->dpb : cfg->refs) + 1; e->ring = cfg->refs + 1;
    if (parent) {
        e->view_of = parent; e->meta = &parent->meta_own;
        for (int i = 0; i < 8; i++) { e->luma[i] = parent->luma[i]; e->chroma[i] = parent->chroma[i]; e->mv16[i] = parent->mv16[i]; e->mbtype[i] = parent->mbtype[i];
                                      e->colref[i] = parent->colref[i]; e->colmv[i] = parent->colmv[i]; e->colref0[i] = parent->colref0[i]; }
    } else {
    for (int i = 0; i < e->slots; i++) {
        alloc((void **)&e->luma[i], S * k.luma_bytes, 0);
        alloc((void **)&e->chroma[i], S * k.cplane_bytes, 0);
    }
    for (int i = 0; i < e->slots; i++) {
        alloc((void **)&e->mv16[i], S * k.nmb * 2 * sizeof(int16_t), 0);
        alloc((void **)&e->mbtype[i], S * k.nmb, 0);
        if (cfg->dpb > 0) { alloc((void **)&e->colref[i], S * k.nmb * 4, 0); alloc((void **)&e->colmv[i], S * k.nmb * 8 * sizeof(int16_t), 0); alloc((void **)&e->colref0[i], S * k.nmb * 4, 0xff); }
    }
    }
    for (int r = 1; r < (cfg->dpb > 0 ? 8 : cfg->refs); r++) alloc((void **)&e->mvr[r], S * k.nmb * 2 * sizeof(int16_t), 0);
    alloc((void **)&e->wf_progress, S * 2 * WFG_ROWS * sizeof(int), 0);
    if (cfg->rd && !cfg->cabac) alloc((void **)&e->tc, S * k.nmb * 24, 0);
    if (cfg->rd && cfg->cabac) { alloc((void **)&e->amvd, S * k.nmb * (cfg->dpb > 0 ? 16 : 8), 0); alloc((void **)&e->cab_out, S * (cfg->slices > 1 ? cfg->slices : 1) * 192 * sizeof(uint32_t), 0); }
    if (S >= 512 && !getenv("X264GPU_NO_BALANCE")) { alloc((void **)&e->perm, S * sizeof(int), 0); alloc((void **)&e->wtime, 4 * S * sizeof(unsigned), 0); }
    if (cfg->slices_plain && cfg->slices > 1) { alloc((void **)&e->sl_stat, 3 * S * cfg->slices * 4 * sizeof(int), 0);       alloc((void **)&e->sl_rerun, S * cfg->slices * sizeof(int), 0); }
#ifdef MB_PROF
    alloc((void **)&e->prof, S * 32 * sizeof(unsigned long long), 0);
#endif
    if (er != hipSuccess) { x264gpu_encoder_destroy(e); return set_err(er == hipErrorOutOfMemory ? X264GPU_ENOMEM : X264GPU_EHIP, "encoder buffers", er); }
    const int rc = build_aq_tables(e);
    if (rc) { x264gpu_encoder_destroy(e); return rc; }
    if (cfg->rd && cfg->cabac) { const uint32_t *ct; const int r2 = cabac_chain_table(&ct); if (r2 != X264GPU_OK) { x264gpu_encoder_destroy(e); return r2; } }
    if (cfg->trellis) { const uint16_t *a; const uint8_t *b; const int *c; const int r2 = trellis_table_ptrs(&a, &b, &c); if (r2 != X264GPU_OK) { x264gpu_encoder_destroy(e); return r2; } }
    *out = e;
    return X264GPU_OK;
}
int x264gpu_encoder_create(x264gpu_encoder **out, const x264gpu_config *cfg) { return encoder_create_impl(out, cfg, nullptr); }
int x264gpu_encoder_create_view(x264gpu_encoder **out, x264gpu_encoder *parent)
{
    ARG_TRY(out && parent && !parent->view_of && parent->cfg.dpb > 0);
    return encoder_create_impl(out, &parent->cfg, parent);
}

int x264gpu_encoder_set_qp(x264gpu_encoder *e, int qp_i, int qp_p)
{
    ARG_TRY(e && qp_i >= 0 && qp_i <= 51 && qp_p >= 0 && qp_p <= 51);
    e->cfg.qp_i = qp_i; e->cfg.qp_p = qp_p;
    return X264GPU_OK;
}

int x264gpu_encoder_set_mb_qp_offsets(x264gpu_encoder *e, const float *d_offsets)
{
    ARG_TRY(e);
    e->ext_off = d_offsets;
    return X264GPU_OK;
}

static int set_stream_qps_f(x264gpu_encoder *e, const int8_t *qps, const float *qpms)
{
    const size_t S = (size_t)e->cfg.streams;
    for (size_t s = 0; s < S; s++) ARG_TRY(qps[s] >= 0 && qps[s] <= 51);
    if (!e->stream_qp) HIP_TRY(hipMalloc((void **)&e->stream_qp, 2 * S));
    if (!e->stream_qpm) HIP_TRY(hipMalloc((void **)&e->stream_qpm, 2 * S * sizeof(float)));
    e->stream_qp_sel ^= 1;
    std::vector<float> f(S);
    for (size_t s = 0; s < S; s++) f[s] = qpms && qpms[s] != 0.f ? qpms[s] : (float)qps[s];
    HIP_TRY(hipMemcpy(e->stream_qp + (size_t)e->stream_qp_sel * S, qps, S, hipMemcpyHostToDevice));
    HIP_TRY(hipMemcpy(e->stream_qpm + (size_t)e->stream_qp_sel * S, f.data(), S * sizeof(float), hipMemcpyHostToDevice));
    e->use_stream_qp = true;
    return X264GPU_OK;
}

int x264gpu_encoder_set_stream_qps(x264gpu_encoder *e, const int8_t *qps)
{
    ARG_TRY(e);
    if (!qps) { e->use_stream_qp = false; return X264GPU_OK; }
    return set_stream_qps_f(e, qps, nullptr);
}
int x264gpu_encoder_set_stream_qpms(x264gpu_encoder *e, const int8_t *qps, const float *qpms)
{
    ARG_TRY(e);
    if (!qps) { e->use_stream_qp = false; return X264GPU_OK; }
    if (qpms) for (int s = 0; s < e->cfg.streams; s++) ARG_TRY(qpms[s] == 0.f || (qpms[s] > (float)qps[s] - 1.f && qpms[s] < (float)qps[s] + 1.f));
    return set_stream_qps_f(e, qps, qpms);
}
int x264gpu_encoder_set_qpm(x264gpu_encoder *e, float qpm)
{
    ARG_TRY(e && qpm >= 0.f && qpm < 52.f);
    e->qpm_next = qpm;
    return X264GPU_OK;
}

static void profile_free(x264gpu_encoder *e)
{
    if (e->ev) {
        for (int i = 0; i < e->prof_cap * (NSTAGE + 1); i++) (void)hipEventDestroy(e->ev[i]);
        delete[] e->ev; delete[] e->ev_mask;
    }
    e->ev = nullptr; e->ev_mask = nullptr; e->prof_cap = e->prof_calls = 0;
}

int x264gpu_encoder_profile_begin(x264gpu_encoder *e, int max_calls)
{
    ARG_TRY(e && max_calls > 0 && max_calls <= 100000);
    profile_free(e);
    e->ev = new (std::nothrow) hipEvent_t[(size_t)max_calls * (NSTAGE + 1)];
    e->ev_mask = new (std::nothrow) int[max_calls];
    if (!e->ev || !e->ev_mask) return set_err(X264GPU_ENOMEM, "profile events", hipSuccess);
    for (int i = 0; i < max_calls * (NSTAGE + 1); i++) HIP_TRY(hipEventCreate(&e->ev[i]));
    e->prof_cap = max_calls;
    return X264GPU_OK;
}

int x264gpu_encoder_profile_end(x264gpu_encoder *e, void *stream, double *ms_sum, int *launches)
{
    ARG_TRY(e && ms_sum && launches);
    HIP_TRY(hipStreamSynchronize((hipStream_t)stream));
    for (int i = 0; i < NSTAGE; i++) { ms_sum[i] = 0; launches[i] = 0; }
    for (int c = 0; c < e->prof_calls; c++) {
        hipEvent_t *ev = e->ev + (size_t)c * (NSTAGE + 1);
        for (int i = 0; i < NSTAGE; i++) {
            if (!(e->ev_mask[c] >> i & 1)) continue;
            float ms = 0;
            HIP_TRY(hipEventElapsedTime(&ms, ev[i], ev[i + 1]));
            ms_sum[i] += ms; launches[i]++;
        }
    }
    profile_free(e);
    return X264GPU_OK;
}

void x264gpu_encoder_destroy(x264gpu_encoder *e)
{
    if (!e) return;
    profile_free(e);
    (void)hipFree(e->fenc_y); (void)hipFree(e->fenc_uv);
    if (!e->view_of)
    for (int i = 0; i < 8; i++) { (void)hipFree(e->luma[i]); (void)hipFree(e->chroma[i]); (void)hipFree(e->mv16[i]); (void)hipFree(e->mbtype[i]); (void)hipFree(e->colref[i]); (void)hipFree(e->colmv[i]); (void)hipFree(e->colref0[i]); }
    (void)hipFree(e->direct_flags_base); (void)hipFree(e->dscore);
    for (int i = 0; i < 8; i++) (void)hipFree(e->mvr[i]);
    (void)hipFree(e->wf_progress);
    (void)hipFree(e->qslab);
    (void)hipFree(e->nr_part);
    (void)hipFree(e->tc);
    (void)hipFree(e->amvd);
    (void)hipFree(e->cab_out);
    (void)hipFree(e->sl_stat); (void)hipFree(e->sl_rerun); (void)hipFree(e->perm); (void)hipFree(e->wtime);
    (void)hipFree(e->prof);
    (void)hipFree(e->stream_qp); (void)hipFree(e->stream_qpm); (void)hipFree(e->mbqp); (void)hipFree(e->q4tab); (void)hipFree(e->q8tab); (void)hipFree(e->lambda_tab); (void)hipFree(e->cost_all);
    delete e;
}

int x264gpu_encoder_mb_count(const x264gpu_encoder *e) { return e ? e->k.nmb : 0; }
int x264gpu_encoder_set_nr(x264gpu_encoder *e, const x264gpu_nr_offsets *d_off, x264gpu_nr_sums *d_pic)
{
    ARG_TRY(e && (d_off != nullptr) == (d_pic != nullptr));
    if (!d_off) { e->nr_off = nullptr; e->nr_pic = nullptr; return X264GPU_OK; }
    ARG_TRY(e->cfg.cabac && e->cfg.rd && e->cfg.trellis && e->cfg.subme >= 6 && (e->cfg.me_method == 1 || e->cfg.me_method == 2) && e->cfg.dpb > 0 && !e->cfg.psy_trellis_q8);
    if (!e->nr_part) {
        const size_t n = (size_t)e->cfg.streams * (e->cfg.slices > 1 ? e->cfg.slices : 1) * sizeof(x264gpu_nr_sums);
        hipError_t er = hipMalloc((void **)&e->nr_part, n);
        if (er == hipSuccess) er = hipMemset(e->nr_part, 0, n);
        if (er != hipSuccess) return set_err(er == hipErrorOutOfMemory ? X264GPU_ENOMEM : X264GPU_EHIP, "nr rows", er);
    }
    e->nr_off = d_off; e->nr_pic = d_pic;
    return X264GPU_OK;
}
int x264gpu_encoder_set_debug(x264gpu_encoder *e, void *d_counters) { ARG_TRY(e); e->dbg = (unsigned long long *)d_counters; return X264GPU_OK; }
int x264gpu_encoder_stage_count(void) { return (int)(sizeof(kStageNames) / sizeof(kStageNames[0])); }
const char *x264gpu_encoder_stage_name(int i) { return i >= 0 && i < x264gpu_encoder_stage_count() ? kStageNames[i] : ""; }

int x264gpu_encoder_mb_prof(x264gpu_encoder *e, unsigned long long *out)
{
    ARG_TRY(e && out);
    if (!e->prof) return X264GPU_EINVAL;
    HIP_TRY(hipDeviceSynchronize());
    HIP_TRY(hipMemcpy(out, e->prof, (size_t)e->cfg.streams * 32 * sizeof(unsigned long long), hipMemcpyDeviceToHost));
    return X264GPU_OK;
}

int x264gpu_encoder_cabac_states(x264gpu_encoder *e, int stream, int slice, uint8_t *out460)
{
    ARG_TRY(e && out460 && stream >= 0 && stream < e->cfg.streams && slice >= 0 && slice < (e->cfg.slices > 1 ? e->cfg.slices : 1));
    if (!e->cab_out) return X264GPU_EINVAL;
    uint32_t w[192];
    HIP_TRY(hipDeviceSynchronize());
    HIP_TRY(hipMemcpy(w, e->cab_out + ((size_t)stream * (e->cfg.slices > 1 ? e->cfg.slices : 1) + slice) * 192, sizeof(w), hipMemcpyDeviceToHost));
    for (int c = 0; c < 460; c++) {
        int reg, lane, sh;
        out460[c] = cab_locate(c, reg, lane, sh) ? (uint8_t)(w[reg * 64 + lane] >> sh) : 0;
    }
    return X264GPU_OK;
}

int x264gpu_encoder_set_lowres_mvs(x264gpu_encoder *e, const int16_t *d_mvs) { ARG_TRY(e); e->lowres_mv = d_mvs; return X264GPU_OK; }
int x264gpu_encoder_set_lowres_mvs1(x264gpu_encoder *e, const int16_t *d_mvs) { ARG_TRY(e); e->lowres_mv1 = d_mvs; return X264GPU_OK; }

__global__ void __launch_bounds__(1024) k_balance(const unsigned *wtime, int *perm, int streams)
{
    for (int s = threadIdx.x; s < streams; s += blockDim.x) {
        const unsigned t = wtime[s];
        int rank = 0;
        for (int o = 0; o < streams; o++) { const unsigned u = wtime[o]; rank += (u > t || (u == t && o < s)) ? 1 : 0; }
        const int half = (streams + 1) / 2;
        perm[rank < half ? rank : half + (streams - 1 - rank)] = s;
    }
}

__global__ void k_slice_priors(EncK k, int streams, int guess)
{
    const int s = blockIdx.x * blockDim.x + threadIdx.x;
    if (s >= streams) return;
    int sum = 0;
    for (int sl = 0; sl < k.slices; sl++) {
        int *st = k.sl_stat + ((size_t)s * k.slices + sl) * 4;
        const bool again = guess || !(st[1] <= sum && sum < st[2]);
        k.sl_rerun[(size_t)s * k.slices + sl] = again;
        if (again) st[3] = sum;
        sum += st[0];
    }
}

}

__global__ __launch_bounds__(64) void k_pack_levels(int16_t *lv, x264gpu_level_index *index, uint32_t *kept, int nmb)
{
    constexpr int Q = X264GPU_MB_LEVELS / 8;
    static_assert(X264GPU_MB_LEVELS % 16 == 0 && Q <= 64, "two lanes a group of 16 levels");
    const int s = blockIdx.x, lane = threadIdx.x;
    uint4 *base = reinterpret_cast<uint4 *>(lv + (size_t)s * nmb * X264GPU_MB_LEVELS);
    x264gpu_level_index *ix = index + (size_t)s * nmb;
    unsigned at = 0;
    uint4 nxt = lane < Q && nmb > 0 ? base[lane] : make_uint4(0, 0, 0, 0);
    for (int i = 0; i < nmb; i++) {
        const uint4 v = nxt;
        if (i + 1 < nmb && lane < Q) nxt = base[(size_t)(i + 1) * Q + lane];
        const unsigned long long nzq = __ballot((v.x | v.y | v.z | v.w) != 0);
        const unsigned groups = (unsigned)__ballot(lane < Q / 2 && ((nzq >> (2 * lane)) & 3));
        if (lane < Q && (groups >> (lane >> 1) & 1)) base[(size_t)(at + __popc(groups & ((1u << (lane >> 1)) - 1u))) * 2 + (lane & 1)] = v;
        if (lane == 0) { ix[i].at = at; ix[i].groups = groups; }
        at += __popc(groups);
    }
    if (kept && lane == 0) kept[s] = at;
}

extern "C" int x264gpu_pack_levels(int16_t *d_levels, int streams, int mb_count, x264gpu_level_index *d_index, uint32_t *d_kept, void *stream)
{
    if (!d_levels || !d_index || streams < 1 || mb_count < 1) return set_err(X264GPU_EINVAL, "x264gpu_pack_levels", hipSuccess);
    hipLaunchKernelGGL(k_pack_levels, dim3(streams), dim3(64), 0, (hipStream_t)stream, d_levels, d_index, d_kept, mb_count);
    HIP_TRY(hipGetLastError());
    return X264GPU_OK;
}

__global__ void k_col_from_records(EncK k)
{
    const int i = blockIdx.x * 256 + threadIdx.x, s = blockIdx.y;
    if (i >= k.nmb * 4) return;
    const int mbi = i >> 2, b8 = i & 3;
    const x264gpu_mb *m = k.mb + (size_t)s * k.nmb + mbi;
    const int t = m->type;
    int r = -1, vx = 0, vy = 0;
    if (t > X264GPU_MB_I16x16) {
        const bool use1 = t >= X264GPU_MB_B_DIRECT && m->ref[b8] < 0;
        r = use1 ? m->ref1[b8] : m->ref[b8]; vx = use1 ? m->mv1[b8][0] : m->mv[b8][0]; vy = use1 ? m->mv1[b8][1] : m->mv[b8][1];
    }
    k.colref_cur[((size_t)s * k.nmb + mbi) * 4 + b8] = (int8_t)r;
    k.colref0_cur[((size_t)s * k.nmb + mbi) * 4 + b8] = (int8_t)(t > X264GPU_MB_I16x16 ? m->ref[b8] : -1);
    int16_t *o = k.colmv_cur + (((size_t)s * k.nmb + mbi) * 4 + b8) * 2;
    o[0] = (int16_t)vx; o[1] = (int16_t)vy;
}

static int encode_core(x264gpu_encoder *e, const uint8_t *d_i420, const x264gpu_pic &pic, x264gpu_mb *d_mb, int16_t *d_levels, hipStream_t st)
{
    int slice_type = pic.slice_type;
    e->last_stream = st;
    if (slice_type == X264GPU_SLICE_I_NONIDR) slice_type = X264GPU_SLICE_I;
    const bool bslice = slice_type == X264GPU_SLICE_B;
    ARG_TRY(pic.dst >= 0 && pic.dst < e->slots && pic.qp >= 0 && pic.qp <= 51);
    ARG_TRY(!bslice || e->cfg.dpb > 0);
    const int n0 = slice_type == X264GPU_SLICE_I ? 0 : pic.nref[0], n1 = bslice ? pic.nref[1] : 0;
    ARG_TRY(pic.qpm == 0.f || (pic.qpm > (float)pic.qp - 1.f && pic.qpm < (float)pic.qp + 1.f));
    ARG_TRY(n0 >= 0 && n0 <= 7 && n1 >= 0 && n1 <= 3 && n0 + n1 <= 8 && (slice_type == X264GPU_SLICE_I || n0 > 0) && (!bslice || n1 > 0));
    for (int l = 0; l < 2; l++) for (int r = 0; r < (l ? n1 : n0); r++) ARG_TRY(pic.slot[l][r] >= 0 && pic.slot[l][r] < e->slots && pic.slot[l][r] != pic.dst);
    const int S = e->cfg.streams;
    EncK k = e->k;
    const int qp = pic.qp;
    e->poc = pic.poc;
    k.i420 = d_i420; k.fenc_y = e->fenc_y; k.fenc_uv = e->fenc_uv;
    const int cur = pic.dst;
    k.rec_luma = e->luma[cur]; k.rec_chroma = e->chroma[cur];
    k.nref = n0; k.nref1 = n1;
    k.blind_dupe = 0; k.wp_any = 0;
    for (int r = 0; r < 8; r++) { k.wl0[r] = 0; k.refpic[r] = r; k.wc0[2 * r] = k.wc0[2 * r + 1] = 0; }
    k.wc_any = 0;
    if (slice_type == X264GPU_SLICE_P) {
        for (int r = 0; r < n0; r++)
            if (pic.wl0[r].on) {
                ARG_TRY(pic.wl0[r].denom >= 0 && pic.wl0[r].denom <= 7 && pic.wl0[r].scale >= -128 && pic.wl0[r].scale <= 127 && pic.wl0[r].offset >= -128 && pic.wl0[r].offset <= 127);
                k.wl0[r] = (int)(uint8_t)(int8_t)pic.wl0[r].offset | (int)(uint8_t)(int8_t)pic.wl0[r].scale << 8 | pic.wl0[r].denom << 16 | 1 << 24;
                k.wp_any = 1;
            }
        for (int r = 0; r < n0; r++)
            for (int c = 0; c < 2; c++)
                if (pic.wc0[r].on[c]) {
                    ARG_TRY(pic.wc0[r].denom >= 0 && pic.wc0[r].denom <= 7 && pic.wc0[r].scale[c] >= -128 && pic.wc0[r].scale[c] <= 127 && pic.wc0[r].offset[c] >= -128 && pic.wc0[r].offset[c] <= 127);
                    k.wc0[2 * r + c] = (int)(uint8_t)(int8_t)pic.wc0[r].offset[c] | (int)(uint8_t)(int8_t)pic.wc0[r].scale[c] << 8 | pic.wc0[r].denom << 16 | 1 << 24;
                    k.wp_any = 1; k.wc_any = 1;
                }
        if (pic.blind_dupe > 0) {
            ARG_TRY(pic.blind_dupe == 1 && n0 >= 2 && pic.slot[0][1] == pic.slot[0][0]);
            k.blind_dupe = 1; k.wp_any = 1;
        }
        int npics = 0;
        for (int r = 0; r < n0; r++) {
            int first = r;
            for (int q = 0; q < r; q++) if (pic.slot[0][q] == pic.slot[0][r]) { first = q; break; }
            k.refpic[r] = first == r ? npics++ : k.refpic[first];
            if (first != r) k.wp_any = 1;
        }
    }
    auto slot_of = [&](int ri) { return (int)(ri < n0 ? pic.slot[0][ri] : pic.slot[1][ri - n0]); };
    for (int r = 0; r < 8; r++) {
        const int slot = n0 + n1 > 0 ? slot_of(r < n0 + n1 ? r : 0) : cur;
        k.ref_luma[r] = e->luma[slot]; k.ref_chroma[r] = e->chroma[slot];
    }
    const int s0 = n0 ? slot_of(0) : cur;
    k.mv16_cur = e->mv16[cur]; k.mv16_ref0 = e->mv16[s0]; k.mbtype_cur = e->mbtype[cur]; k.mbtype_ref0 = e->mbtype[s0];
    for (int r = 0; r < 8; r++) k.mvr[r] = e->mvr[r];
    k.temporal = k.nref > 0 && e->meta->slot_nref[s0] > 0;
    for (int r = 0; r < 8; r++) k.tscale[r] = 0;
    if (k.temporal) {
        const int delta = e->meta->slot_poc[s0] - e->meta->slot_ref0poc[s0], inv = (256 + delta / 2) / delta;
        for (int r = 0; r < n0 + n1; r++) k.tscale[r] = (e->poc - e->meta->slot_poc[slot_of(r)]) * inv;
    }
    memset(k.biw, 32, sizeof(k.biw));
    if (bslice) {
        for (int r0 = 0; r0 < n0; r0++)
            for (int r1 = 0; r1 < n1; r1++) {
                const int poc0 = e->meta->slot_poc[pic.slot[0][r0]], poc1 = e->meta->slot_poc[pic.slot[1][r1]];
                const int td = min(max(poc1 - poc0, -128), 127);
// ... 280 lines not shown
```

x264vfw_amd/csrc/k_mb.hip.h:

```cpp
#pragma once
#include "deblock_line.hip.h"
#include "enc_common.hip.h"
#include "k_analyse.hip.h"
#include "intra8.hip.h"
#include "rd.hip.h"

namespace x264gpu {

constexpr int IT_STRIDE = 32;
constexpr int IT_ORG = IT_STRIDE + 4;
constexpr int IT_SIZE = 17 * IT_STRIDE + 8;
constexpr int MB_COST_MAX = 1 << 28;
enum { D_16x16 = 0, D_16x8 = 1, D_8x16 = 2, D_8x8 = 3 };
enum { ME_16 = 0, ME_8 = 1, ME_16x8 = 5, ME_8x16 = 7, ME_COUNT = 9 };

constexpr int MVC_N = 512;
constexpr int RC_ROWS = 30, RC_PD = 10, RC_COLS = 4 * RC_PD, RC_PLANE_DW = RC_ROWS * RC_PD, RC_SLOT_DW = 4 * RC_PLANE_DW, RC_MX = 12, RC_MY = 7;
template <int PD_, int ROWS_> struct RcGeo {
    static constexpr int PD = PD_, ROWS = ROWS_, COLS = 4 * PD_, PLANE_DW = ROWS_ * PD_, SLOT_DW = 4 * PLANE_DW, NT = (PLANE_DW + 63) / 64;
    static_assert(PD_ == 10 || PD_ == 16, "row length: 10 dwords (division by multiplication below) or 16");
    static __device__ __forceinline__ int row_of(int i) { return PD_ == 16 ? i >> 4 : (i * 205) >> 11; }
};
struct WinTags { int tref, tx, ty; };

// ... 1288 lines not shown
        const int big = quad_or(any_big(v) ? 1 : 0);
        const int sc = mask ? (big ? 9 : decimate_from_mask(mask, 1)) : 0;
        const int score = row16_sum(j == 0 ? sc : 0);
        const bool fail = ssd >= thresh && (nzdc != 0 || (ssd >= thresh * 4 && score >= 7));
        ok = ok && !__builtin_amdgcn_readlane((int)fail, 0) && !__builtin_amdgcn_readlane((int)fail, 16);
    }
    return ok;
}

__device__ __forceinline__ bool mb_probe_pskip(const EncK &k, const MbCtx &c, uint32_t cz, int pmx, int pmy, const Q4 &ql, const Q4 &qc, const uint16_t *nro = nullptr)
{
    const int lane = relane(c.lane), j = lane & 3, zx = z_x0(lane), zy = z_y(lane);
    const int mvx = clampi(pmx, c.mvmin0, c.mvmax0), mvy = clampi(pmy, c.mvmin1, c.mvmax1);
    uint32_t pred = mc_luma_row4(ref_plane00(k, c.s, 0), k.plane_bytes, k.rs, c.px + zx, c.py + zy, mvx, mvy);
    if (k.wp_any && (k.wl0[0] >> 24)) pred = wp4(pred, k.wl0[0]);
    const int pl = (lane >> 4) & 1, ci = (lane >> 2) & 3, cx0 = (ci & 1) * 4, cyy = (ci >> 1) * 4 + j;
    uint32_t pu, pv;
    mc_chroma_row4(ref_chroma00(k, c.s, 0), k.rs, c.mbx * 8 + cx0, c.mby * 8 + cyy, mvx, mvy, pu, pv);
    if (k.wc_any) { if (k.wc0[0] >> 24) pu = wp4(pu, k.wc0[0]); if (k.wc0[1] >> 24) pv = wp4(pv, k.wc0[1]); }
    const uint2 fe = *(const uint2 *)(c.fuv + (size_t)cyy * k.fs + 2 * cx0);
    return mb_probe_skip_pred(c, cz, pred, nv12_pick(fe.x, fe.y, pl), pl ? pv : pu, ql, qc, nro);
}

struct BCfg { int r0, x0, y0, r1, x1, y1; };
#define D4(a, b, c, d) ((uint32_t)(uint8_t)(int8_t)(a) | ((uint32_t)(uint8_t)(int8_t)(b) << 8) | ((uint32_t)(uint8_t)(int8_t)(c) << 16) | ((uint32_t)(uint8_t)(int8_t)(d) << 24))
static __constant__ const uint32_t c_dia4d[33] = {
    D4(0, 0, 0, 0),
    D4(0, 0, 0, 1), D4(0, 0, 0, -1), D4(0, 0, 1, 0), D4(0, 0, -1, 0), D4(0, 1, 0, 0), D4(0, -1, 0, 0), D4(1, 0, 0, 0), D4(-1, 0, 0, 0),
    D4(0, 0, 1, 1), D4(0, 0, -1, -1), D4(0, 1, 1, 0), D4(0, -1, -1, 0), D4(1, 1, 0, 0), D4(-1, -1, 0, 0), D4(1, 0, 0, 1), D4(-1, 0, 0, -1),
    D4(0, 1, 0, 1), D4(0, -1, 0, -1), D4(1, 0, 1, 0), D4(-1, 0, -1, 0), D4(0, 0, -1, 1), D4(0, 0, 1, -1), D4(0, -1, 1, 0), D4(0, 1, -1, 0),
    D4(-1, 1, 0, 0), D4(1, -1, 0, 0), D4(1, 0, 0, -1), D4(-1, 0, 0, 1), D4(0, -1, 0, 1), D4(0, 1, 0, -1), D4(-1, 0, 1, 0), D4(1, 0, -1, 0) };
#undef D4

__device__ __forceinline__ BCfg b_clip(const MbCtx &c, const BCfg &g0)
{
    BCfg g = g0;
    g.x0 = clampi(g.x0, c.mvmin0, c.mvmax0); g.y0 = clampi(g.y0, c.mvmin1, c.mvmax1); g.x1 = clampi(g.x1, c.mvmin0, c.mvmax0); g.y1 = clampi(g.y1, c.mvmin1, c.mvmax1);
    return g;
}
__device__ __forceinline__ void b_fetch_luma(const EncK &k, const MbCtx &c, const BCfg &g, uint32_t &p0, uint32_t &p1)
{
    const int lane = relane(c.lane), zx = z_x0(lane), zy = z_y(lane);
    p0 = mc_luma_row4(ref_plane00(k, c.s, max(g.r0, 0)), k.plane_bytes, k.rs, c.px + zx, c.py + zy, g.x0, g.y0);
    p1 = mc_luma_row4(ref_plane00(k, c.s, k.nref + max(g.r1, 0)), k.plane_bytes, k.rs, c.px + zx, c.py + zy, g.x1, g.y1);
}
__device__ __forceinline__ void b_combine_luma(const BCfg &g, int biwv, uint32_t p0, uint32_t p1, uint32_t &pred)
{
    const int w = __shfl(biwv, max(g.r0, 0) * 4 + max(g.r1, 0));
    pred = g.r0 >= 0 ? (g.r1 >= 0 ? avg_weight4_u8(p0, p1, w) : p0) : p1;
}
__device__ __forceinline__ void b_fetch_chroma(const EncK &k, const MbCtx &c, const BCfg &g, uint32_t &c0, uint32_t &c1)
{
    const int lane = relane(c.lane), j4 = lane & 3;
    const int pl = (lane >> 4) & 1, ci = (lane >> 2) & 3, cx0 = (ci & 1) * 4, cyy = (ci >> 1) * 4 + j4;
    const int r0 = __shfl(g.r0, ci * 16), x0 = __shfl(g.x0, ci * 16), y0 = __shfl(g.y0, ci * 16);
    const int r1 = __shfl(g.r1, ci * 16), x1 = __shfl(g.x1, ci * 16), y1 = __shfl(g.y1, ci * 16);
    uint32_t u0 = 0, v0 = 0, u1 = 0, v1 = 0;
    mc_chroma_row4(ref_chroma00(k, c.s, max(r0, 0)), k.rs, c.mbx * 8 + cx0, c.mby * 8 + cyy, x0, y0, u0, v0);
    mc_chroma_row4(ref_chroma00(k, c.s, k.nref + max(r1, 0)), k.rs, c.mbx * 8 + cx0, c.mby * 8 + cyy, x1, y1, u1, v1);
    c0 = pl ? v0 : u0; c1 = pl ? v1 : u1;
}
__device__ __forceinline__ void b_combine_chroma(const MbCtx &c, const BCfg &g, int biwv, uint32_t c0, uint32_t c1, uint32_t &cpred)
{
    const int ci = (relane(c.lane) >> 2) & 3;
    const int r0 = __shfl(g.r0, ci * 16), r1 = __shfl(g.r1, ci * 16);
    const int w = __shfl(biwv, max(r0, 0) * 4 + max(r1, 0));
    cpred = r0 >= 0 ? (r1 >= 0 ? avg_weight4_u8(c0, c1, w) : c0) : c1;
}

__device__ __forceinline__ void b_fetch(const EncK &k, const MbCtx &c, const BCfg &g0, uint32_t &p0, uint32_t &p1, uint32_t &c0, uint32_t &c1)
{
    const BCfg g = b_clip(c, g0);
    b_fetch_luma(k, c, g, p0, p1);
    b_fetch_chroma(k, c, g, c0, c1);
}

__device__ __forceinline__ void b_combine(const MbCtx &c, const BCfg &g, int biwv, uint32_t p0, uint32_t p1, uint32_t c0, uint32_t c1, uint32_t &pred, uint32_t &cpred)
{
    b_combine_luma(g, biwv, p0, p1, pred);
    b_combine_chroma(c, g, biwv, c0, c1, cpred);
}

__device__ __forceinline__ void b_predict(const EncK &k, const MbCtx &c, const BCfg &g0, int biwv, uint32_t &pred, uint32_t &cpred)
{
    const BCfg g = b_clip(c, g0);
    uint32_t p0, p1, c0, c1;
    b_fetch_luma(k, c, g, p0, p1);
    b_combine_luma(g, biwv, p0, p1, pred);
    b_fetch_chroma(k, c, g, c0, c1);
    b_combine_chroma(c, g, biwv, c0, c1, cpred);
}

#ifndef MB_WAVES_PER_EU
#define MB_WAVES_PER_EU 2
#endif
template <int M, int ME, bool PS, int RD = 0, bool BS = false, bool PSY = false, bool NR = false>
__global__ __launch_bounds__(64) __attribute__((amdgpu_waves_per_eu(MB_WAVES_PER_EU, 4))) void k_mb_slice(EncK k)
{
    static_assert(!PSY || RD >= 3, "psy-trellis: instantiations with the trellis quantiser");
    static_assert(!NR || (RD >= 3 && PS && !PSY), "nr: inter slices of trellis sessions, without psy-trellis");
    using TRC = std::conditional_t<PSY, TrCtxPsy, TrCtx>;
    __shared__ __attribute__((aligned(16))) int16_t psy_fd[PSY ? 512 : 1];
    static_assert(!BS || PS, "B slices are inter slices");
    static_assert(RD != 7 || BS, "RD 7: B slices only");
    __shared__ __attribute__((aligned(16))) MbLds<M> L;
    static_assert(!BS || CSubGeo<M>::DWORDS >= 128, "b_visited aliases L.csub");
#define b_visited L.csub
    const int lane0 = threadIdx.x, s = k.perm ? uni(k.perm[blockIdx.x]) : (int)blockIdx.x;
    int lane = lane0;
    const unsigned long long wt0 = k.wtime ? __builtin_readcyclecounter() : 0ull;
#ifdef X264GPU_POISON
    for (int i = lane; i < (int)(sizeof(L) / 4); i += 64) ((uint32_t *)&L)[i] = 0xCDCDCDCDu;
    __builtin_amdgcn_s_waitcnt(0); __builtin_amdgcn_wave_barrier();
#endif
    const int nsl = k.slices > 1 ? k.slices : 1, row0 = (k.mbh * (int)blockIdx.y + nsl / 2) / nsl, row1 = (k.mbh * ((int)blockIdx.y + 1) + nsl / 2) / nsl;
    const int mb_first = row0 * k.mbw, mb_end = row1 * k.mbw;
    int intra_prior = 0;
    if (PS && k.sl_stat) {
        const size_t si = (size_t)s * nsl + blockIdx.y;
        if (k.sl_pass && !k.sl_rerun[si]) return;
        intra_prior = uni(k.sl_stat[si * 4 + 3]);
        if (lane == 0) { L.slw[0] = 0; L.slw[1] = 0x7fffffff; L.slw[2] = intra_prior; }
    }
    const uint32_t t4 = (lane >> 2) < 9 ? ((const uint32_t *)c_pred4_table.t)[lane] : 0x01010101u * U_DC;
    for (int i = lane; i < 144; i += 64) ((uint32_t *)L.pred8tab)[i] = ((const uint32_t *)c_pred8_table)[i];
    lds_sync();
    x264gpu_mb *mbs = k.mb + (size_t)s * k.nmb;
    constexpr bool pslice = PS;
    constexpr bool TRL = RD >= 3;
    constexpr bool TRL2 = RD == 4 || RD == 6;
    constexpr bool NORD = RD == 0 || RD == 7;
    constexpr bool REF = RD == 5 || RD == 6;
    int j4 = lane & 3, zx = z_x0(lane), zy = z_y(lane);
#define RELANE() do { lane = relane(lane0); c.lane = lane; j4 = lane & 3; zx = z_x0(lane); zy = z_y(lane); } while (0)
    int intra_count = intra_prior, cost_qp = -1;
    __shared__ __attribute__((aligned(16))) int16_t rd_lvs[RD ? X264GPU_MB_LEVELS + (NR ? NR_OFF_N : 0) : 1];
    __shared__ uint8_t rd_ntc[2][RD == 1 ? 24 : 1];
    const uint16_t *nro = nullptr;
    x264gpu_nr_sums *nr_row = nullptr;
    if constexpr (NR) {
        nro = (const uint16_t *)(rd_lvs + X264GPU_MB_LEVELS);
        const uint32_t *src = (const uint32_t *)(k.nr_off + s);
        if (lane < NR_OFF_N / 2) ((uint32_t *)(rd_lvs + X264GPU_MB_LEVELS))[lane] = src[nr_stage_src(lane)];
        nr_row = k.nr_part + (size_t)s * nsl + blockIdx.y;
        nr_row->sum[0][lane] = 0; nr_row->sum[1][lane] = 0; nr_row->sum[2][lane] = 0;
        if (lane < 4) (&nr_row->count[0])[lane] = 0;
    }
    if constexpr (NR) lds_sync();
#ifdef X264GPU_POISON
    for (int i = lane; i < (RD ? X264GPU_MB_LEVELS : 1); i += 64) rd_lvs[i] = (int16_t)0xCDCD;
    __builtin_amdgcn_s_waitcnt(0); __builtin_amdgcn_wave_barrier();
#endif
    int last_qp = uni((int)k.mbqp[(size_t)s * k.nmb + mb_first]);
    Cab cab = { 0, 0, 0, 0, 0 };
    uint32_t cab_modelv = 0;
    int last_dqp = 0;
    if constexpr (RD >= 2) { cab_init(cab, lane, pslice, last_qp); cab_modelv = cab_model(lane); }
    Prof pf;
    pf.start();
    int biwv = 32;
    if constexpr (BS) {
#pragma unroll
        for (int r0 = 0; r0 < 5; r0++)
#pragma unroll
            for (int r1 = 0; r1 < 4; r1++) biwv = lane == r0 * 4 + r1 ? (int)k.biw[r0][r1] : biwv;
    }
    int16_t *mv16 = k.mv16_cur + (size_t)s * k.nmb * 2;
    uint8_t *mbtype_cur = k.mbtype_cur + (size_t)s * k.nmb;

    int ds_t = 0, ds_s = 0;
    for (int mbi = mb_first; mbi < mb_end; mbi++) {
        MbCtx c;
        RELANE();
        c.s = s; c.mbi = mbi; c.mbx = mbi % k.mbw; c.mby = mbi / k.mbw; c.sy = c.mby - row0; c.px = c.mbx * 16; c.py = c.mby * 16;
        c.fenc = k.fenc_y + (size_t)s * k.fency_bytes + (size_t)c.py * k.fs + c.px;
        c.fuv = k.fenc_uv + (size_t)s * k.fencuv_bytes + (size_t)c.mby * 8 * k.fs + c.px;
        c.qp = __builtin_amdgcn_readfirstlane((int)k.mbqp[(size_t)s * k.nmb + mbi]);
        last_qp = uni(last_qp); last_dqp = uni(last_dqp); intra_count = uni(intra_count); cost_qp = uni(cost_qp); ds_t = uni(ds_t); ds_s = uni(ds_s);
        if (k.qp_snap && abs(c.qp - last_qp) == 1) c.qp = last_qp;
        c.qpc = (int)d_chroma_qp_table[min(max(c.qp + k.chroma_qp_offset, 0), 51)];
        c.lambda = k.lambda_tab[c.qp];
        c.subme = min(max(k.subme, 0), 11);
        if (BS && (c.subme == 6 || c.subme == 8)) c.subme--;
        c.satd = c.subme > 1; c.chroma_me = pslice && k.chroma_me && (BS ? REF && c.subme >= 9 : c.subme >= 5);
        c.cost_base = k.cost_all + (size_t)c.qp * 2 * MVCOST_HALF;
        if (pslice && c.qp != cost_qp) {
            cost_qp = c.qp;
            lds_sync();
            const uint32_t *src = (const uint32_t *)(c.cost_base + MVCOST_HALF);
            for (int i = lane; i < MVC_N / 2; i += 64) ((uint32_t *)L.mvcost)[i] = src[i];
            lds_sync();
        }
        c.nref = k.nref;
        const Q4 &q_li = k.q4tab[c.qp * 4 + 0], &q_lp = k.q4tab[c.qp * 4 + 1], &q_ci = k.q4tab[c.qpc * 4 + 2], &q_cp = k.q4tab[c.qpc * 4 + 3];
        const Q8 &q8i = k.q8tab[c.qp * 2 + 0], &q8p = k.q8tab[c.qp * 2 + 1];
        const bool left = c.mbx > 0, top = c.sy > 0, topright = top && c.mbx + 1 < k.mbw, topleft = top && left;
        const int mbx = c.mbx, mby = c.mby;
        __builtin_amdgcn_fence(__ATOMIC_ACQUIRE, "workgroup");
        auto intra_t = [](int t) { return t >= 0 && t <= 3; };
        uint8_t *rec = rec_plane00(k, s) + (size_t)c.py * k.rs + c.px;
        uint8_t *ruv = rec_chroma00(k, s) + (size_t)(mby * 8) * k.rs + c.px;
        int16_t *lv = k.levels + ((size_t)s * k.nmb + mbi) * X264GPU_MB_LEVELS;
        uint8_t *tile = L.tile + IT_ORG, *tile8 = L.tile8 + IT_ORG;

        uint8_t v_y = 128, v_c = 128;
        int n_type = -1, n_mode = 2, nb_type = -1, mc_type = -1, mc_ref = 0, mc_vx = 0, mc_vy = 0;
        if (lane < 25) {
            const int x = lane - 1;
            if (top && (x >= 0 || left) && (x < 16 || topright)) v_y = rec[-(long)k.rs + x];
        } else if (lane >= 32 && lane < 48) {
            if (left) v_y = rec[(long)(lane - 32) * k.rs - 1];
        } else if (lane >= 48 && lane < 56) {
            const int i = lane - 48;
            const x264gpu_mb *n = i < 4 ? (left ? mbs + mbi - 1 : nullptr) : (top ? mbs + mbi - k.mbw : nullptr);
            if (n) { n_type = n->type; n_mode = n->i4_mode[i < 4 ? blkidx_of(3, i) : blkidx_of(i - 4, 3)]; }
        } else if (lane >= 56 && lane < 60) {
            const int q = lane - 56;
            const int nbi = q == 0 ? (left ? mbi - 1 : -1) : q == 1 ? (top ? mbi - k.mbw : -1) : q == 2 ? (topleft ? mbi - k.mbw - 1 : -1) : (topright ? mbi - k.mbw + 1 : -1);
            if (nbi >= 0) nb_type = mbs[nbi].type;
        }
        {
            const int t = lane & 15, pl = (lane >> 4) & 1;
            if (lane < 32) { if (t < 9) { const int x = t - 1; if (top && (x >= 0 || left)) v_c = ruv[-(long)k.rs + 2 * x + pl]; } }
            else if (lane < 48) { if (left) v_c = ruv[(long)(t & 7) * k.rs - 2 + ((t >> 3) & 1)]; }
        }
        int mc_dir = 0;
        if (BS ? (lane < 32 && (lane & 15) < 12) : (lane < 12 && pslice)) {
            const int gl = lane & 15, gx = (gl & 3) - 1, gy = (gl >> 2) - 1;
            int nbi = -1, blk = 0;
            if (gy < 0) {
                if (gx < 0) { if (topleft) { nbi = mbi - k.mbw - 1; blk = 3; } }
                else if (gx < 2) { if (top) { nbi = mbi - k.mbw; blk = 2 + gx; } }
                else if (topright) { nbi = mbi - k.mbw + 1; blk = 2; }
            } else if (gx < 0 && left) { nbi = mbi - 1; blk = 1 + 2 * gy; }
            if (nbi >= 0) {
                const x264gpu_mb *n = mbs + nbi; mc_type = n->type;
                if (BS && lane >= 16) { mc_ref = n->ref1[blk]; mc_vx = n->mv1[blk][0]; mc_vy = n->mv1[blk][1]; }
                else { mc_ref = n->ref[blk]; mc_vx = n->mv[blk][0]; mc_vy = n->mv[blk][1]; }
                if constexpr (BS) mc_dir = mc_type == X264GPU_MB_B_DIRECT || mc_type == X264GPU_MB_B_SKIP || (mc_type == X264GPU_MB_B_8x8 && ((n->direct8 >> blk) & 1));
            }
        }
        const uint32_t cz = *(const uint32_t *)(c.fenc + (size_t)zy * k.fs + zx);
        uint32_t csv = 0;
        if (lane < 32) csv = *(const uint32_t *)(c.fuv + (size_t)(lane >> 2) * k.fs + (lane & 3) * 4);
        uint8_t ntcv = 0;
        uint32_t cnbv = 0;
        if constexpr (RD >= 2) {
            if (lane < 8) { const bool av = lane < 4 ? left : top; static_assert(sizeof(x264gpu_mb) == 64, "record"); const int dw = (lane & 3) == 0 ? 0 : (lane & 3) == 1 ? 1 : (lane & 3) == 2 ? 6 : 11;
                            if (av) cnbv = ((const uint32_t *)(mbs + (lane < 4 ? mbi - 1 : mbi - k.mbw)))[dw]; }
            else if (lane < (BS ? 16 : 12)) {
                const bool lf = (lane & 3) < 2, av = lf ? left : top;
                if (av) cnbv = ((const uint32_t *)(k.amvd + ((size_t)s * k.nmb + (lf ? mbi - 1 : mbi - k.mbw)) * (BS ? 16 : 8)))[(lane & 1) + (lane >= 12 ? 2 : 0)];
            }
        }
        if constexpr (RD == 1) {
            if (k.rd) {
                if (lane < 24) { if (left) ntcv = k.tc[((size_t)s * k.nmb + mbi - 1) * 24 + lane]; }
                else if (lane < 48) { if (top) ntcv = k.tc[((size_t)s * k.nmb + mbi - k.mbw) * 24 + lane - 24]; }
            }
        }
        lds_sync();
        if (lane < 25) {
            const int x = lane - 1;
            tile[-IT_STRIDE + x] = v_y; tile8[-IT_STRIDE + x] = v_y;
            if (lane < 21) L.nb[NB_TOP + x] = v_y;
        } else if (lane >= 32 && lane < 48) {
            const int y = lane - 32;
            tile[y * IT_STRIDE - 1] = v_y; tile8[y * IT_STRIDE - 1] = v_y; L.nb[NB_LEFT + y] = v_y;
        } else if (lane >= 48 && lane < 56) {
            L.nmodes[lane - 48] = (uint8_t)((n_type == X264GPU_MB_I4x4 || n_type == X264GPU_MB_I8x8) ? n_mode : 2);
        }
        {
            const int t = lane & 15, pl = (lane >> 4) & 1;
            if (lane < 32) { if (t < 9) L.cnb[pl][CNB_TOP + t - 1] = v_c; }
            else if (lane < 48) L.cnb[(t >> 3) & 1][CNB_LEFT + (t & 7)] = v_c;
        }
        const int type_left = rl(nb_type, 56), type_top = rl(nb_type, 57), type_tl = rl(nb_type, 58), type_tr = rl(nb_type, 59);
        MeState S = {};
        if (BS ? (lane < 32 && (lane & 15) < 12) : lane < 12) {
            int ref = -2, vx = 0, vy = 0;
            if (mc_type >= 0) { if (mc_type <= 3) ref = -1; else { ref = mc_ref; vx = mc_vx; vy = mc_vy; } }
            if (BS && ref < 0) { vx = 0; vy = 0; if (ref != -2) ref = -1; }
            S.cref = ref; S.cmvx = vx; S.cmvy = vy; S.cdir = mc_dir;
        }
        *(uint32_t *)(L.src + zy * 16 + zx) = cz;
        if constexpr (RD == 1) { if (lane < 48) rd_ntc[lane >= 24][lane >= 24 ? lane - 24 : lane] = ntcv; }
        if (lane < 32) *(uint32_t *)(L.csrc + (lane >> 2) * 16 + (lane & 3) * 4) = csv;
        if constexpr (PSY) {
            {
                int e[4];
                unpack4(cz, e);
                dct4_quad(e, lane);
                store_levels_scan(psy_fd + (lane >> 2) * 16, e, j4);
            }
            if (k.dct8x8) {
                uint32_t elo, ehi;
                z_to_r8(cz, lane, elo, ehi);
                const int row = lane & 7, i8 = (lane >> 3) & 3;
                int v[8];
                unpack8(elo, ehi, v);
                fwd8_1d(v); transpose8(v, lane); fwd8_1d(v); transpose8(v, lane);
                if (lane < 32)
#pragma unroll
                    for (int i = 0; i < 8; i++) psy_fd[256 + i8 * 64 + c_zigzag8_inv[row * 8 + i]] = (int16_t)v[i];
            }
        }
        lds_sync();
// ... 1202 lines not shown
                const bool skp = rec_type == X264GPU_MB_P_SKIP || rec_type == X264GPU_MB_B_SKIP;
                if (skp) coded = false;
                if (coded && lane < 24) for (int i = 0; i < myn; i++) my_tc += myl[i] != 0;
                int na = -1, nb = -1;
                {
                    const bool chroma = lane >= 16 && lane < 24;
                    const int b = lane == 24 ? 0 : lane & 15, ci = (lane - 16) & 3, cb = 16 + ((lane - 16) & 4);
                    const int bx = chroma ? ci & 1 : z_bx(b), by = chroma ? ci >> 1 : z_by(b);
                    const int l_in = chroma ? cb + by * 2 : blkidx_of(bx - 1, by), t_in = chroma ? cb + bx : blkidx_of(bx, by - 1);
                    const int l_out = chroma ? cb + by * 2 + 1 : blkidx_of(3, by), t_out = chroma ? cb + 2 + bx : blkidx_of(bx, 3);
                    const int tl = __shfl(my_tc, bx > 0 ? l_in : 0), tt = __shfl(my_tc, by > 0 ? t_in : 0);
                    if (lane < 25) {
                        if (bx > 0 && lane != 24) na = tl; else if (left) na = rd_ntc[0][l_out];
                        if (by > 0 && lane != 24) nb = tt; else if (top) nb = rd_ntc[1][t_out];
                    }
                }
                const int nC = lane >= 25 ? -1 : (na >= 0 && nb >= 0 ? (na + nb + 1) >> 1 : na >= 0 ? na : nb >= 0 ? nb : 0);
                if (rd_run && !commit && !skp) {
                    mb_bits = wave_sum(coded ? cavlc_block_bits(myl, myn, nC) : 0);
                    if (BS && !intra) {
                        if (e_type == X264GPU_MB_B_DIRECT) mb_bits += 1;
                        else {
                            const int np = e_part == D_16x16 ? 1 : e_part == D_8x8 ? 4 : 2;
                            auto b8_of = [&](int kp) { return e_part == D_8x8 ? kp : e_part == D_16x8 ? 2 * kp : kp; };
                            if (e_part == D_8x8) { mb_bits += bs_size_ue_d(22); for (int kp = 0; kp < 4; kp++) { const int u = (int)((euse >> (2 * kp)) & 3); mb_bits += bs_size_ue_d(u == 3 ? 0 : 1 + u); } }
                            else if (e_part == D_16x16) mb_bits += bs_size_ue_d(1 + (int)(euse & 3));
                            else {
                                const int u0 = (int)(euse & 3), u1 = (int)((e_part == D_16x8 ? euse >> 4 : euse >> 2) & 3);
                                const int pair = u0 == 0 ? (u1 == 0 ? 0 : u1 == 1 ? 2 : 4) : u0 == 1 ? (u1 == 0 ? 3 : u1 == 1 ? 1 : 5) : 6 + u1;
                                mb_bits += bs_size_ue_d(4 + 2 * pair + (e_part == D_8x16 ? 1 : 0));
                            }
                            const int sc0 = S.cref, sc1 = S.cmvx, sc2 = S.cmvy;
                            for (int l = 0; l < 2; l++) {
                                const int nr = l ? k.nref1 : k.nref, go = 16 * l;
                                for (int kp = 0; kp < np; kp++) {
                                    const int b8 = b8_of(kp), u = (int)((euse >> (2 * b8)) & 3);
                                    if (nr > 1 && !(u == 3 || u == 1 - l)) mb_bits += nr == 2 ? 1 : bs_size_ue_d(rl(l ? ecfg.r1 : ecfg.r0, b8 * 16));
                                }
                                if ((lane == 5 + go || lane == 6 + go || lane == 9 + go || lane == 10 + go)) S.cref = -2;
                                for (int kp = 0; kp < np; kp++) {
                                    const int b8 = b8_of(kp), u = (int)((euse >> (2 * b8)) & 3), x8 = b8 & 1, y8 = b8 >> 1;
                                    const int w8 = e_part == D_16x16 || e_part == D_16x8 ? 2 : 1, h8 = e_part == D_16x16 || e_part == D_8x16 ? 2 : 1;
                                    const int r = rl(l ? ecfg.r1 : ecfg.r0, b8 * 16), vx = rl(l ? ecfg.x1 : ecfg.x0, b8 * 16), vy = rl(l ? ecfg.y1 : ecfg.y0, b8 * 16);
                                    const int g0 = (y8 + 1) * 4 + x8 + 1 + go;
                                    const bool mine = lane == g0 || (w8 == 2 && lane == g0 + 1) || (h8 == 2 && lane == g0 + 4) || (w8 == 2 && h8 == 2 && lane == g0 + 5);
                                    if (!(u == 3 || u == 1 - l)) {
                                        S.cref = mine ? r : S.cref;
                                        int px, py;
                                        mb_predict_mv(S, e_part, x8, y8, w8, r, px, py, go);
                                        mb_bits += bs_size_se_d(vx - px) + bs_size_se_d(vy - py);
                                    }
                                    S.cref = mine ? (r >= 0 ? r : -1) : S.cref; S.cmvx = mine ? (r >= 0 ? vx : 0) : S.cmvx; S.cmvy = mine ? (r >= 0 ? vy : 0) : S.cmvy;
                                }
                            }
                            S.cref = sc0; S.cmvx = sc1; S.cmvy = sc2;
                        }
                        mb_bits += cavlc_cbp_bits(cbp_luma | (cbp_chroma << 4), true);
                        if (k.dct8x8 && cbp_luma) mb_bits += 1;
                    } else
                    if (!intra) {
                        const int np = e_part == D_16x16 ? 1 : e_part == D_8x8 ? 4 : 2;
                        mb_bits += bs_size_ue_d(e_part) + (e_part == D_8x8 ? 4 : 0);
                        const int sc0 = S.cref, sc1 = S.cmvx, sc2 = S.cmvy;
                        if (lane == 5 || lane == 6 || lane == 9 || lane == 10) S.cref = -2;
                        for (int kp = 0; kp < np; kp++) {
                            const int x8 = e_part == D_8x16 ? kp : e_part == D_8x8 ? kp & 1 : 0, y8 = e_part == D_16x8 ? kp : e_part == D_8x8 ? kp >> 1 : 0;
                            const int w8 = e_part == D_16x16 || e_part == D_16x8 ? 2 : 1, h8 = e_part == D_16x16 || e_part == D_8x16 ? 2 : 1;
                            const int slot = e_part == D_16x16 ? ME_16 : e_part == D_16x8 ? ME_16x8 + kp : e_part == D_8x16 ? ME_8x16 + kp : ME_8 + kp;
                            const int r = rl(S.ref, slot), vx = rl(S.mvx, slot), vy = rl(S.mvy, slot);
                            if (c.nref > 1) mb_bits += c.nref == 2 ? 1 : bs_size_ue_d(r);
                            const int g0 = (y8 + 1) * 4 + x8 + 1;
                            const bool mine = lane == g0 || (w8 == 2 && lane == g0 + 1) || (h8 == 2 && lane == g0 + 4) || (w8 == 2 && h8 == 2 && lane == g0 + 5);
                            S.cref = mine ? r : S.cref;
                            int px, py;
                            mb_predict_mv(S, e_part, x8, y8, w8, r, px, py);
                            mb_bits += bs_size_se_d(vx - px) + bs_size_se_d(vy - py);
                            S.cmvx = mine ? vx : S.cmvx; S.cmvy = mine ? vy : S.cmvy;
                        }
                        S.cref = sc0; S.cmvx = sc1; S.cmvy = sc2;
                        mb_bits += cavlc_cbp_bits(cbp_luma | (cbp_chroma << 4), true);
                        if (k.dct8x8 && cbp_luma) mb_bits += 1;
                    } else {
                        const int off = BS ? 23 : pslice ? 5 : 0;
                        if (i16) { const int m16 = IR.pred16 > PRED16_P ? PRED16_DC : IR.pred16; mb_bits += bs_size_ue_d(off + 1 + m16 + 4 * cbp_chroma + (cbp_luma ? 12 : 0)); }
                        else {
                            mb_bits += bs_size_ue_d(off) + (k.dct8x8 ? 1 : 0);
                            int fb = 0;
                            if (e_type == X264GPU_MB_I4x4) { if (lane < 16) fb = i4_pred_mode(L.nmodes, c.mbx, c.sy, lane, L.modes4) == L.modes4[lane] ? 1 : 4; }
                            else if (lane < 4) fb = i4_pred_mode(L.nmodes, c.mbx, c.sy, lane * 4, L.modes8) == L.modes8[lane * 4] ? 1 : 4;
                            mb_bits += wave_sum(fb);
                            mb_bits += cavlc_cbp_bits(cbp_luma | (cbp_chroma << 4), false);
                        }
                        mb_bits += bs_size_ue_d(predc > PREDC_P ? PREDC_DC : predc);
                    }
                    if (cbp_luma || cbp_chroma || i16) mb_bits += bs_size_se_d(c.qp - last_qp);
                }
            }
            if (rd_run && !commit) {
                int dist = wave_sum(ssd_y);
                if (k.psy_rd_q8) {
                    const int e4 = wave_sum(en4) >> 1, e8 = wave_sum(en8) >> 2;
                    dist += (((abs(e4 - fenc_e4) + abs(e8 - fenc_e8)) >> 1) * k.psy_rd_q8 * c.lambda + 128) >> 8;
                }
                dist += (int)(((long long)wave_sum(ssd_c) * chroma_l2off + 128) >> 8);
                const int cost = rec_type == X264GPU_MB_P_SKIP || rec_type == X264GPU_MB_B_SKIP ? dist + ((lambda2 + 128) >> 8) : dist + (int)(((long long)mb_bits * lambda2 + 128) >> 8);
                if constexpr (BS) {
                    if (rd_ph == 1 || rd_ph == 7) rd_dir = cost;
                    else if (rd_ph == 2 || rd_ph == 8) rd_l0 = cost;
                    else if (rd_ph == 3 || rd_ph == 9) rd_l1 = cost;
                    else if (rd_ph == 4 || rd_ph == 10) rd_bi = cost;
                    else if (rd_ph == 11) rd_8x8 = cost;
                    else if (rd_ph == 12) rd_16x8 = cost;
                    else if (rd_ph == 13) rd_8x16 = cost;
                    else if (rd_ph == 14) { if (rd_best >= cost) { if (rd_best > 0) rd_satd_inter = (int)((long long)rd_satd_inter * cost / rd_best); rd_best = cost; rd_t8 = 1; } }
                    else if (rd_ph == 15) rd_i16 = cost;
                    else if (rd_ph == 16) rd_i4 = cost;
                    else if (rd_ph == 17) rd_i8 = cost;
                } else
                if (rd_ph == 0) {
                    rd16 = cost;
                    if (rec_type == X264GPU_MB_P_SKIP) {
                        rd_best = cost; rd_part = D_16x16; rd_t8 = 0; rd_i16 = rd_i4 = rd_i8 = MB_COST_MAX; rd_ph = 8 - 1; rd_skip16 = true;
                    }
                } else if (rd_ph == 1) rd16x8 = cost;
                else if (rd_ph == 2) rd8x16 = cost;
                else if (rd_ph == 3) rd8x8 = cost;
                else if (rd_ph == 4) { if (rd_best >= cost) { if (rd_best > 0) rd_satd_inter = (int)((long long)rd_satd_inter * cost / rd_best); rd_best = cost; rd_t8 = 1; } }
                else if (rd_ph == 5) rd_i16 = cost;
                else if (rd_ph == 6) rd_i4 = cost;
                else if (rd_ph == 7) rd_i8 = cost;
                rd_ph++;
                continue;
            }
            for (int i = lane; i < X264GPU_MB_LEVELS / 2; i += 64) ((uint32_t *)lv)[i] = ((const uint32_t *)rd_lvs)[i];
            if (rdon && lane < 24) k.tc[((size_t)s * k.nmb + mbi) * 24 + lane] = (uint8_t)my_tc;
        }
        {
            const bool i16e = rec_type == X264GPU_MB_I16x16;
            if (rec_type != X264GPU_MB_P_SKIP && (cbp_luma || cbp_chroma || i16e) && !(i16e && !cbp_luma && !cbp_chroma && !((nnz >> 24) & 1) && c.qp > last_qp)) last_qp = c.qp;
        }
        break;
        }
        if (lane == 0) { recd.nnz = nnz; recd.cbp_luma = (uint8_t)cbp_luma; recd.cbp_chroma = (uint8_t)cbp_chroma; recd.type = (uint8_t)rec_type; mbtype_cur[mbi] = (uint8_t)rec_type; }
        lds_sync();
        if (lane < 16) ((uint32_t *)(mbs + mbi))[lane] = ((const uint32_t *)&L.rec)[lane];
        __builtin_amdgcn_fence(__ATOMIC_RELEASE, "workgroup");
        __builtin_amdgcn_s_waitcnt(0);
        pf.mark(PH_STORE);
    }
    if (BS && k.dscore && k.direct_auto && lane == 0) { int *d = k.dscore + ((size_t)s * nsl + blockIdx.y) * 2; d[0] = ds_t; d[1] = ds_s; }
    if (PS && k.sl_stat && lane == 0) { int *st = k.sl_stat + ((size_t)s * nsl + blockIdx.y) * 4; st[0] = intra_count - L.slw[2]; st[1] = L.slw[0]; st[2] = L.slw[1]; }
    if (k.wtime && lane == 0 && blockIdx.y == 0) k.wtime[s] = (unsigned)min((unsigned long long)(__builtin_readcyclecounter() - wt0) >> 6, 0xffffffffull);
    if constexpr (RD >= 2) {
        if (k.cab_out) { uint32_t *o = k.cab_out + ((size_t)s * (k.slices > 1 ? k.slices : 1) + blockIdx.y) * 192; o[lane] = cab.a; o[64 + lane] = cab.r; o[128 + lane] = cab.r8; }
    }
#ifdef MB_PROF
    if (lane == 0 && k.prof) for (int i = 0; i < 32; i++) k.prof[(size_t)s * 32 + i] = pf.acc[i];
#endif
}

void mb_kernel_note(uint32_t id);
template <int M, int ME, bool PS, int RD = 0, bool BS = false, bool PSY = false, bool NR = false>
static inline void mb_launch(const EncK &k, int streams, hipStream_t st)
{
    static_assert(M < 16 && ME < 16 && RD < 16, "the id holds one hex digit each");
    mb_kernel_note((uint32_t)(M << 12 | ME << 8 | RD << 4 | PS << 3 | BS << 2 | PSY << 1 | (int)NR));
    hipLaunchKernelGGL((k_mb_slice<M, ME, PS, RD, BS, PSY, NR>), dim3(streams, k.slices > 1 ? k.slices : 1), dim3(64), 0, st, k);
}

}
```

x264vfw_amd/csrc/prim_kernels.hip:

```cpp
#include "common.hip.h"
#include "mc.hip.h"
#include "k_mb.hip.h"
#include "trellis.hip.h"
#include <math.h>
#include <mutex>
#include <vector>
#include <stddef.h>

using namespace x264gpu;

__global__ __launch_bounds__(256) void k_pixel_metric(int metric, const uint8_t *__restrict__ a,
                                                      const uint8_t *__restrict__ b, int n, int w, int h,
                                                      int32_t *__restrict__ out)
{
    const int lane = threadIdx.x & 63;
    const int idx = blockIdx.x * 4 + (threadIdx.x >> 6);
    if (idx >= n) return;
    const int nbx = w >> 2, nblk = nbx * (h >> 2);
    const int blk = lane >> 2, j = lane & 3;
    int bx, by;
    if (w == 16 && h == 16) { bx = z_bx(blk); by = z_by(blk); }
    else { bx = blk % nbx; by = blk / nbx; }
    const bool valid = blk < nblk;
    uint32_t pa = 0, pb = 0;
// ... 283 lines not shown
        }
        uint32_t *a = nullptr;
        HIP_TRY(hipMalloc((void **)&a, h.size() * sizeof(uint32_t)));
        const hipError_t ce = hipMemcpy(a, h.data(), h.size() * sizeof(uint32_t), hipMemcpyHostToDevice);
        if (ce != hipSuccess) { (void)hipFree(a); HIP_TRY(ce); }
        tab[dev] = a;
    }
    *out = tab[dev];
    return X264GPU_OK;
}

int trellis_table_ptrs(const uint16_t **su, const uint8_t **tu, const int **l2)
{
    TrellisTab tt;
    const int rc = trellis_tables(&tt);
    if (rc == X264GPU_OK) { *su = tt.size_unary; *tu = tt.trans_unary; *l2 = tt.lambda2; }
    return rc;
}

template <int CAT, bool FORCE_GENERAL>
__global__ void __launch_bounds__(64) k_trellis_blocks_psy(const int16_t *coefs, const int16_t *fdct, int nblk, int qp, int intra, int psy_q8, const uint8_t *states, TrellisTab tt,
                                                           int16_t *levels, uint8_t *nz, uint8_t *paths)
{
    constexpr int NC = CAT == 5 ? 64 : 16;
    __shared__ int16_t buf[8 * 64], fbuf[8 * 64];
    __shared__ uint8_t st[460];
    const int lane = threadIdx.x;
    for (int i = lane; i < 460; i += 64) st[i] = states[i];
    const uint32_t model = cab_model(lane);
    __syncthreads();
    const int sig_off = CAT == 1 ? 120 : CAT == 2 ? 134 : 402, last_off = CAT == 1 ? 181 : CAT == 2 ? 195 : 417, abs_off = CAT == 1 ? 237 : CAT == 2 ? 247 : 426;
    uint32_t reg = 0;
    for (int ctx = 0; ctx < 460; ctx++) {
        int rg, ln, sh;
        if (!cab_locate(ctx, rg, ln, sh) || ln != lane) continue;
        const bool mine = (ctx >= sig_off && ctx < sig_off + 16) || (ctx >= last_off && ctx < last_off + 16) || (ctx >= abs_off && ctx < abs_off + 10);
        if (mine && rg == (CAT == 5 ? 2 : 1)) reg |= (uint32_t)st[ctx] << sh;
    }
    TrellisPsy<true> psy;
    psy.fdct = (const lds_i16 *)fbuf; psy.fstride = NC; psy.q8 = psy_q8;
    for (int b0 = 0; b0 < nblk; b0 += 8) {
        const int nb = min(8, nblk - b0);
        for (int i = lane; i < nb * NC; i += 64) { buf[i] = coefs[(size_t)b0 * NC + i]; fbuf[i] = fdct[(size_t)b0 * NC + i]; }
        __syncthreads();
        const unsigned m = trellis_blocks<CAT, FORCE_GENERAL, true>((lds_i16 *)buf, NC, nb, qp, intra != 0, model, tt, reg, psy);
        __syncthreads();
        for (int i = lane; i < nb * NC; i += 64) levels[(size_t)b0 * NC + i] = buf[i];
        if (lane < nb) nz[b0 + lane] = (uint8_t)((m >> lane) & 1);
        if (paths && lane == 0) paths[b0 >> 3] = (uint8_t)((m >> 8) & 3);
        __syncthreads();
    }
}

template <int CAT, bool FORCE_GENERAL>
__global__ void __launch_bounds__(64) k_trellis_blocks(const int16_t *coefs, int nblk, int qp, int intra, const uint8_t *states, TrellisTab tt, int16_t *levels, uint8_t *nz, uint8_t *paths)
{
    constexpr int NC = CAT == 5 ? 64 : CAT == 3 ? 4 : 16;
    __shared__ int16_t buf[8 * 64];
    __shared__ uint8_t st[460];
    const int lane = threadIdx.x;
    for (int i = lane; i < 460; i += 64) st[i] = states[i];
    const uint32_t model = cab_model(lane);
    __syncthreads();
    const int sig_off = CAT == 0 ? 105 : CAT == 1 ? 120 : CAT == 2 ? 134 : CAT == 3 ? 149 : CAT == 4 ? 152 : 402;
    const int last_off = CAT == 0 ? 166 : CAT == 1 ? 181 : CAT == 2 ? 195 : CAT == 3 ? 210 : CAT == 4 ? 213 : 417;
    const int abs_off = CAT == 0 ? 227 : CAT == 1 ? 237 : CAT == 2 ? 247 : CAT == 3 ? 257 : CAT == 4 ? 266 : 426;
    uint32_t reg = 0;
    for (int ctx = 0; ctx < 460; ctx++) {
        int rg, ln, sh;
        if (!cab_locate(ctx, rg, ln, sh) || ln != lane) continue;
        const bool mine = (ctx >= sig_off && ctx < sig_off + 16) || (ctx >= last_off && ctx < last_off + 16) || (ctx >= abs_off && ctx < abs_off + 10);
        if (mine && rg == (CAT == 5 ? 2 : 1)) reg |= (uint32_t)st[ctx] << sh;
    }
    for (int b0 = 0; b0 < nblk; b0 += 8) {
        const int nb = min(8, nblk - b0);
        for (int i = lane; i < nb * NC; i += 64) buf[i] = coefs[(size_t)b0 * NC + i];
        __syncthreads();
        const unsigned m = trellis_blocks<CAT, FORCE_GENERAL>((lds_i16 *)buf, NC, nb, qp, intra != 0, model, tt, reg);
        __syncthreads();
        for (int i = lane; i < nb * NC; i += 64) levels[(size_t)b0 * NC + i] = buf[i];
        if (lane < nb) nz[b0 + lane] = (uint8_t)((m >> lane) & 1);
        if (paths && lane == 0) paths[b0 >> 3] = (uint8_t)((m >> 8) & 3);
        __syncthreads();
    }
}

}

extern "C" {

int x264gpu_trellis_blocks_ex(const int16_t *d_coefs, int nblk, int cat, int qp, int intra, const uint8_t *d_states460, int16_t *d_levels, uint8_t *d_nz, int force_general,
                             uint8_t *d_paths, void *stream)
{
    ARG_TRY(d_coefs && d_states460 && d_levels && d_nz && nblk >= 0 && cat >= 0 && cat <= 5 && qp >= 0 && qp <= 51);
    if (!nblk) return X264GPU_OK;
    TrellisTab tt;
    const int rc = trellis_tables(&tt);
    if (rc != X264GPU_OK) return rc;
    const hipStream_t st = (hipStream_t)stream;
#define TRELLIS_LAUNCH(CAT_) \
    if (force_general) hipLaunchKernelGGL((k_trellis_blocks<CAT_, true>), dim3(1), dim3(64), 0, st, d_coefs, nblk, qp, intra, d_states460, tt, d_levels, d_nz, d_paths); \
    else hipLaunchKernelGGL((k_trellis_blocks<CAT_, false>), dim3(1), dim3(64), 0, st, d_coefs, nblk, qp, intra, d_states460, tt, d_levels, d_nz, d_paths)
    switch (cat) {
    case 0: TRELLIS_LAUNCH(0); break;
    case 1: TRELLIS_LAUNCH(1); break;
    case 2: TRELLIS_LAUNCH(2); break;
    case 3: TRELLIS_LAUNCH(3); break;
    case 4: TRELLIS_LAUNCH(4); break;
    default: TRELLIS_LAUNCH(5); break;
    }
#undef TRELLIS_LAUNCH
    HIP_TRY(hipGetLastError());
    return X264GPU_OK;
}

int x264gpu_trellis_blocks_psy(const int16_t *d_coefs, const int16_t *d_fenc_dct, int nblk, int cat, int qp, int intra, int psy_trellis_q8, const uint8_t *d_states460,
                               int16_t *d_levels, uint8_t *d_nz, int force_general, uint8_t *d_paths, void *stream)
{
    ARG_TRY(psy_trellis_q8 >= 0 && psy_trellis_q8 <= 640 && cat >= 0 && cat <= 5);
    if (!psy_trellis_q8 || !(cat == 1 || cat == 2 || cat == 5)) return x264gpu_trellis_blocks_ex(d_coefs, nblk, cat, qp, intra, d_states460, d_levels, d_nz, force_general, d_paths, stream);
    ARG_TRY(d_coefs && d_fenc_dct && d_states460 && d_levels && d_nz && nblk >= 0 && qp >= 0 && qp <= 51);
    if (!nblk) return X264GPU_OK;
    TrellisTab tt;
    const int rc = trellis_tables(&tt);
    if (rc != X264GPU_OK) return rc;
    const hipStream_t st = (hipStream_t)stream;
#define TRELLIS_LAUNCH(CAT_) \
    if (force_general) hipLaunchKernelGGL((k_trellis_blocks_psy<CAT_, true>), dim3(1), dim3(64), 0, st, d_coefs, d_fenc_dct, nblk, qp, intra, psy_trellis_q8, d_states460, tt, d_levels, d_nz, d_paths); \
    else hipLaunchKernelGGL((k_trellis_blocks_psy<CAT_, false>), dim3(1), dim3(64), 0, st, d_coefs, d_fenc_dct, nblk, qp, intra, psy_trellis_q8, d_states460, tt, d_levels, d_nz, d_paths)
    switch (cat) {
    case 1: TRELLIS_LAUNCH(1); break;
    case 2: TRELLIS_LAUNCH(2); break;
    default: TRELLIS_LAUNCH(5); break;
    }
#undef TRELLIS_LAUNCH
    HIP_TRY(hipGetLastError());
    return X264GPU_OK;
}

int x264gpu_trellis_blocks(const int16_t *d_coefs, int nblk, int cat, int qp, int intra, const uint8_t *d_states460, int16_t *d_levels, uint8_t *d_nz, void *stream)
{
    return x264gpu_trellis_blocks_ex(d_coefs, nblk, cat, qp, intra, d_states460, d_levels, d_nz, 0, nullptr, stream);
}


}
namespace x264gpu {
__global__ void k_cab_level_walk(const int16_t *lv, const int *what, const uint32_t *r_in, const uint32_t *r8_in, uint32_t *r_out, uint32_t *r8_out, int *bits, const uint32_t *ctab)
{
    __shared__ int16_t l[X264GPU_MB_LEVELS];
    const int i = blockIdx.x, lane = threadIdx.x;
    for (int j = lane; j < X264GPU_MB_LEVELS; j += 64) l[j] = lv[(size_t)i * X264GPU_MB_LEVELS + j];
    __syncthreads();
    Cab cb; cb.a = 0; cb.r = r_in[i * 64 + lane]; cb.r8 = r8_in[i * 64 + lane]; cb.f8 = 0; cb.f8v = 0;
    const uint32_t model = cab_model(lane);
    CabLv W = { what[i * 5], (unsigned)what[i * 5 + 1], (unsigned)what[i * 5 + 2], (unsigned)what[i * 5 + 3], what[i * 5 + 4] != 0 };
    Prof pf;
    cab_levels_all(cb, model, lane, l, W, ctab, pf);
    r_out[i * 64 + lane] = cb.r; r8_out[i * 64 + lane] = cb.r8;
    const int t = cab_total(cb);
    if (lane == 0) bits[i] = t;
}
}
extern "C" {
int x264gpu_cabac_level_walk(const int16_t *d_levels, const int32_t *d_what, int n, const uint32_t *d_r, const uint32_t *d_r8, uint32_t *d_r_out, uint32_t *d_r8_out, int32_t *d_bits, void *stream)
{
    ARG_TRY(d_levels && d_what && d_r && d_r8 && d_r_out && d_r8_out && d_bits && n >= 0);
    if (!n) return X264GPU_OK;
    const uint32_t *ctab = nullptr;
    { const int rc = x264gpu::cabac_chain_table(&ctab); if (rc != X264GPU_OK) return rc; }
    hipLaunchKernelGGL(x264gpu::k_cab_level_walk, dim3(n), dim3(64), 0, (hipStream_t)stream, d_levels, d_what, d_r, d_r8, d_r_out, d_r8_out, d_bits, ctab);
    HIP_TRY(hipGetLastError());
    return X264GPU_OK;
}
}
```

x264vfw_amd/lib.py:

```python
import ctypes as C
import os

_HERE = os.path.dirname(os.path.abspath(__file__))
LIB_PATH = os.environ.get("X264GPU_LIB") or os.path.join(_HERE, "libx264gpu.so")


class X264GpuError(RuntimeError):
    pass


def _load():
    try:
        import torch
    except ImportError:
        pass
    if not os.path.exists(LIB_PATH):
        raise X264GpuError(
            f"{LIB_PATH} not built — run `python -c 'import __graft_entry__ as g; g.build()'` "
            "(there is no CPU fallback for the HIP hot path)")
    return C.CDLL(LIB_PATH)


_lib = _load()
_vp, _i, _sz = C.c_void_p, C.c_int, C.c_size_t


class MbRecord(C.Structure):
    _fields_ = [("type", C.c_uint8), ("i16_mode", C.c_uint8), ("chroma_mode", C.c_uint8), ("qp", C.c_uint8),
                ("cbp_luma", C.c_uint8), ("cbp_chroma", C.c_uint8), ("partition", C.c_uint8),
                ("ref", C.c_int8 * 4), ("i4_mode", C.c_uint8 * 16),                ("transform8x8", C.c_uint8), ("mv", (C.c_int16 * 2) * 4),
                ("nnz", C.c_uint32), ("cost", C.c_int32), ("aux", C.c_int32 * 3)]


class Config(C.Structure):
    _fields_ = [(n, C.c_float if n == "aq_strength" else C.c_int) for n in (
        "width", "height", "streams", "refs", "qp_i", "qp_p", "me_range", "subme", "deblock",
        "deblock_alpha", "deblock_beta", "chroma_qp_offset", "deadzone_inter", "deadzone_intra",
        "dct_decimate", "partitions", "dct8x8", "me_method", "chroma_me", "mixed_refs", "aq_mode", "aq_strength", "fast_pskip", "mv_range", "cabac", "rd", "psy", "psy_rd_q8", "slices", "trellis", "slices_plain", "dpb", "weightb", "psy_trellis_q8")]


class Pic(C.Structure):
    class W(C.Structure):
        _fields_ = [("on", C.c_int8), ("denom", C.c_int8), ("scale", C.c_int16), ("offset", C.c_int16)]
    class WC(C.Structure):
        _fields_ = [("on", C.c_int8 * 2), ("denom", C.c_int8), ("pad", C.c_int8), ("scale", C.c_int16 * 2), ("offset", C.c_int16 * 2)]
    _fields_ = [("slice_type", C.c_int), ("qp", C.c_int), ("poc", C.c_int), ("dst", C.c_int), ("keep", C.c_int), ("nref", C.c_int * 2),
                ("slot", (C.c_int8 * 8) * 2), ("wl0", W * 8), ("blind_dupe", C.c_int), ("qpm", C.c_float), ("wc0", WC * 8), ("direct_temporal", C.c_int), ("direct_auto", C.c_int)]


class Quality(C.Structure):
    _fields_ = [("ssd", C.c_uint64 * 3), ("ssim_sum", C.c_double), ("ssim_cnt", C.c_uint32), ("pad", C.c_uint32)]


class NrOffsets(C.Structure):
    _fields_ = [("off", (C.c_uint16 * 64) * 3)]


class NrSums(C.Structure):
    _fields_ = [("sum", (C.c_uint64 * 64) * 3), ("count", C.c_uint32 * 3), ("pad", C.c_uint32)]


def make_pic(slice_type, qp, poc, dst, keep, l0=(), l1=()):
    p = Pic(slice_type=slice_type, qp=qp, poc=poc, dst=dst, keep=keep, blind_dupe=-1)
    p.nref[0], p.nref[1] = len(l0), len(l1)
    for i, s in enumerate(l0):
        p.slot[0][i] = s
    for i, s in enumerate(l1):
        p.slot[1][i] = s
    return p


MB_LEVELS = 416

_SIGS = {
    "x264gpu_abi_version": (_i, []),
    "x264gpu_device_count": (_i, []),
    "x264gpu_set_device": (_i, [_i]),
    "x264gpu_last_error": (C.c_char_p, []),
    "x264gpu_malloc": (_i, [C.POINTER(_vp), _sz]),
    "x264gpu_free": (_i, [_vp]),
    "x264gpu_memcpy_h2d": (_i, [_vp, _vp, _sz, _vp]),
    "x264gpu_memcpy_d2h": (_i, [_vp, _vp, _sz, _vp]),
    "x264gpu_memcpy_d2d": (_i, [_vp, _vp, _sz, _vp]),
    "x264gpu_memset": (_i, [_vp, _i, _sz, _vp]),
    "x264gpu_stream_sync": (_i, [_vp]),
    "x264gpu_stream_create": (_i, [C.POINTER(_vp)]),
    "x264gpu_stream_destroy": (_i, [_vp]),
    "x264gpu_event_create": (_i, [C.POINTER(_vp)]),
    "x264gpu_event_destroy": (_i, [_vp]),
    "x264gpu_event_record": (_i, [_vp, _vp]),
    "x264gpu_event_sync": (_i, [_vp]),
    "x264gpu_stream_wait_event": (_i, [_vp, _vp]),
    "x264gpu_encoder_create_view": (_i, [C.POINTER(_vp), _vp]),
    "x264gpu_pixel_metric": (_i, [_i, _vp, _vp, _i, _i, _i, _vp, _vp]),
    "x264gpu_pixel_var": (_i, [_vp, _i, _i, _i, _vp, _vp]),
    "x264gpu_pixel_hadamard_ac": (_i, [_vp, _i, _i, _i, _vp, _vp]),
    "x264gpu_dctq4x4": (_i, [_vp, _vp, _i, _i, _i, _vp, _vp, _vp, _vp]),
    "x264gpu_dctq8x8": (_i, [_vp, _vp, _i, _i, _i, _vp, _vp, _vp, _vp]),
    "x264gpu_intra_predict": (_i, [_i, _vp, _i, _vp, _vp, _vp, _i, _vp, _vp]),
    "x264gpu_hpel_filter": (_i, [_vp, _sz, _i, _i, _i, _i, _vp]),
    "x264gpu_lowres": (_i, [_vp, _i, _i, _i, _vp, _sz, _i, _vp]),
    "x264gpu_mc_luma": (_i, [_vp, _sz, _i, _vp, _vp, _i, _i, _i, _vp, _vp]),
    "x264gpu_mc_avg": (_i, [_vp, _vp, _sz, _i, _vp, _vp]),
    "x264gpu_mc_weight": (_i, [_vp, _sz, _i, _i, _i, _vp, _vp]),
    "x264gpu_mc_chroma": (_i, [_vp, _i, _vp, _vp, _i, _i, _i, _vp, _vp]),
    "x264gpu_gather_rows": (_i, [_vp, _sz, _vp, _i, _vp]),
    "x264gpu_csp_img_fill": (C.c_long, [_i, _i, _i, C.POINTER(C.c_long), C.POINTER(_i)]),
    "x264gpu_csp_to_i420": (_i, [C.POINTER(_vp), C.POINTER(_i), _i, _i, _i, _i, _i, C.POINTER(_vp), C.POINTER(_i), _vp]),
    "x264gpu_csp_to_i420_batch": (_i, [C.POINTER(_vp), C.POINTER(_i), _sz, _i, _i, _i, _i, _i, C.POINTER(_vp), C.POINTER(_i), _sz, _i, _vp]),
    "x264gpu_encoder_direct_scores": (_i, [_vp, _vp]),
    "x264gpu_encoder_create": (_i, [C.POINTER(_vp), C.POINTER(Config)]),
    "x264gpu_encoder_destroy": (None, [_vp]),
    "x264gpu_encoder_mb_count": (_i, [_vp]),
    "x264gpu_encode_frames": (_i, [_vp, _vp, _i, _vp, _vp, _vp]),
    "x264gpu_encoder_get_recon": (_i, [_vp, _i, _vp, _vp]),
    "x264gpu_encode_pictures": (_i, [_vp, _vp, _vp, _vp, _vp, _vp]),
    "x264gpu_pack_levels": (_i, [_vp, _i, _i, _vp, _vp, _vp]),
    "x264gpu_encoder_get_recon_slot": (_i, [_vp, _i, _i, _vp, _vp]),
    "x264gpu_picture_quality": (_i, [_vp, _vp, _i, _i, _i, _i, _vp, _vp]),
    "x264gpu_encoder_quality": (_i, [_vp, _i, _vp, _vp]),
    "x264gpu_encoder_stage_count": (_i, []),
    "x264gpu_encoder_stage_name": (C.c_char_p, [_i]),
    "x264gpu_encoder_profile_begin": (_i, [_vp, _i]),
    "x264gpu_encoder_set_debug": (_i, [_vp, _vp]),
    "x264gpu_mb_kernels_seen": (_i, [C.POINTER(C.c_uint32), _i, _i]),
    "x264gpu_encoder_profile_end":(_i, [_vp, _vp, C.POINTER(C.c_double), C.POINTER(_i)]),
    "x264gpu_encoder_set_qp": (_i, [_vp, _i, _i]),
    "x264gpu_encoder_set_mb_qp_offsets": (_i, [_vp, _vp]),
    "x264gpu_encoder_set_stream_qpms": (_i, [_vp, _vp, _vp]),
    "x264gpu_encoder_set_qpm": (_i, [_vp, C.c_float]),
    "x264gpu_encoder_set_stream_qps": (_i, [_vp, _vp]),
    "x264gpu_encoder_set_lowres_mvs": (_i, [_vp, _vp]),
    "x264gpu_encoder_set_lowres_mvs1": (_i, [_vp, _vp]),
    "x264gpu_encoder_cabac_states": (_i, [_vp, _i, _i, _vp]),
    "x264gpu_trellis_blocks": (_i, [_vp, _i, _i, _i, _i, _vp, _vp, _vp, _vp]),
    "x264gpu_trellis_blocks_ex": (_i, [_vp, _i, _i, _i, _i, _vp, _vp, _vp, _i, _vp, _vp]),
    "x264gpu_trellis_blocks_psy": (_i, [_vp, _vp, _i, _i, _i, _i, _i, _vp, _vp, _vp, _i, _vp, _vp]),
    "x264gpu_encoder_set_nr": (_i, [_vp, _vp, _vp]),
    "x264gpu_nr_update": (_i, [_vp, _vp, _vp, _i, _i, _vp]),
    "x264gpu_denoise_blocks": (_i, [_vp, _i, _i, _vp, _vp, _vp]),
    "x264gpu_cabac_level_walk": (_i, [_vp, _vp, _i, _vp, _vp, _vp, _vp, _vp, _vp]),
    "x264gpu_encoder_deblock_pictures": (_i, [_vp, _vp, _vp, _vp, _vp]),
    "x264gpu_get_device": (_i, [_vp]),
    "x264gpu_lookahead_create": (_i, [C.POINTER(_vp), _i, _i, _i, _i, _i]),
    "x264gpu_lookahead_destroy": (None, [_vp]),
    "x264gpu_lookahead_frame_cost": (_i, [_vp, _vp, _i, _vp, _vp, _vp]),
    "x264gpu_lookahead_aq_offsets": (_i, [_vp, _vp, C.c_float, _vp, _vp]),
    "x264gpu_lookahead_aq_offsets_mode": (_i, [_vp, _vp, _i, C.c_float, _vp, _vp]),
    "x264gpu_lookahead_mbtree": (_i, [_vp, C.POINTER(_vp), C.POINTER(_vp), _i, C.c_float, _vp, _vp]),
    "x264gpu_slicetype_create": (_i, [C.POINTER(_vp)] + [_i] * 11),
    "x264gpu_slicetype_destroy": (None, [_vp]),
    "x264gpu_slicetype_put_frame": (_i, [_vp, _i, _vp, _vp]),
    "x264gpu_slicetype_frame_cost": (_i, [_vp, _i, _i, _i, _i, _i, _vp, _vp]),
    "x264gpu_slicetype_intra_mbs": (_i, [_vp, _i, _i, _i]),
    "x264gpu_slicetype_cost_est": (_i, [_vp, _i, _i, _i, _i]),
    "x264gpu_slicetype_lowres_mvs": (_vp, [_vp, _i, _i, _i]),
    "x264gpu_slicetype_lowres_mv_costs": (_vp, [_vp, _i, _i, _i]),
    "x264gpu_slicetype_intra_costs": (_vp, [_vp, _i]),
    "x264gpu_slicetype_lowres_costs": (_vp, [_vp, _i, _i, _i]),
    "x264gpu_slicetype_frame_cost_w": (_i, [_vp] + [_i] * 9 + [_vp, _vp]),
    "x264gpu_slicetype_pixel_stats": (_i, [_vp, _i, _vp, _vp, _vp]),
    "x264gpu_slicetype_weight_cost": (_i, [_vp, _i, _i, _i, _i, _i, _i, _i, _vp, _vp]),
    "x264gpu_slicetype_chroma_stats": (_i, [_vp, _i, _vp, _vp, _vp]),
    "x264gpu_slicetype_weight_cost_chroma": (_i, [_vp, _i, _vp, _vp, _i, _i, _i, _i, _i, _i, _vp, _vp]),
    "x264gpu_slicetype_set_aq": (_i, [_vp, _i, _vp, _vp]),
    "x264gpu_slicetype_set_row_mode": (_i, [_vp, _i]),
    "x264gpu_slicetype_set_bframe_bias": (_i, [_vp, _i]),
    "x264gpu_slicetype_cost_aq": (_i, [_vp, _i, _i, _i, _vp, _vp]),
    "x264gpu_slicetype_clear_propagate": (_i, [_vp, _i, _vp]),
    "x264gpu_slicetype_propagate": (_i, [_vp, _i, _i, _i, _i, _i, _i, _vp]),
    "x264gpu_slicetype_finish": (_i, [_vp, _i, C.c_float, C.c_float, _vp, _vp]),
    "x264gpu_slicetype_propagate_cost": (_vp, [_vp, _i]),
    "x264gpu_mbtree_pack": (_i, [_vp, _i, _vp, _vp]),
    "x264gpu_mbtree_unpack": (_i, [_vp, _i, _vp, _vp]),
}

EXPORTS = tuple(_SIGS)
_missing = []
for _name, (_res, _args) in _SIGS.items():
    try:
        _fn = getattr(_lib, _name)
    except AttributeError:
        _missing.append(_name)
        continue
    _fn.restype, _fn.argtypes = _res, _args
if _missing:
    raise X264GpuError(f"libx264gpu.so lacks symbols declared in include/x264gpu.h: {_missing}")


def check(rc, what="x264gpu call"):
    if rc != 0:
        raise X264GpuError(f"{what} failed ({rc}): {_lib.x264gpu_last_error().decode()}")


def __getattr__(name):
    return getattr(_lib, name)
```

Measured before the change: 744.1.

## Batch CABAC mode-context bins into per-lane bitstrings walked via chain table

Replaces the per-bin serial CABAC state update for the low contexts (0-104, 399-401) with one state per lane in two registers. Bins are appended to per-context bitstrings and resolved in batches through a precomputed chain table (cab_walk_a), so several bins are processed per table lookup instead of one readlane/writeback per bin. Intra prediction modes and coded_block_flag bins are gathered with ballot/ds_permute. The state export layout grows to 256 words and a standalone bins-walk kernel is added for testing. The batching adds flush and table-lookup overhead and is a risk to exact bit-cost equivalence.

```diff
diff --git a/include/x264gpu.h b/include/x264gpu.h
--- a/include/x264gpu.h
+++ b/include/x264gpu.h
@@ -59,6 +59,7 @@
 int x264gpu_mc_weight(const uint8_t *d_src, size_t bytes, int scale, int denom, int offset, uint8_t *d_out, void *stream);
 int x264gpu_gather_rows(const void *const *d_rows, size_t row_bytes, void *d_dst, int rows, void *stream);
 int x264gpu_cabac_level_walk(const int16_t *d_levels, const int32_t *d_what, int n, const uint32_t *d_r, const uint32_t *d_r8, uint32_t *d_r_out, uint32_t *d_r8_out, int32_t *d_bits, void *stream);
+int x264gpu_cabac_bins_walk(const int32_t *d_triples, const int32_t *d_first, int n, const uint8_t *d_states, uint8_t *d_states_out, int32_t *d_bits, void *stream);
 
 enum { X264GPU_CSP_MASK = 0xff, X264GPU_CSP_I420 = 1, X264GPU_CSP_YV12 = 2, X264GPU_CSP_YV16 = 3, X264GPU_CSP_YV24 = 4,
        X264GPU_CSP_NV12 = 5, X264GPU_CSP_YUYV = 6, X264GPU_CSP_UYVY = 7, X264GPU_CSP_BGR = 8, X264GPU_CSP_BGRA = 9,
diff --git a/x264vfw_amd/csrc/cabac_layout.hip.h b/x264vfw_amd/csrc/cabac_layout.hip.h
--- a/x264vfw_amd/csrc/cabac_layout.hip.h
+++ b/x264vfw_amd/csrc/cabac_layout.hip.h
@@ -6,8 +6,9 @@
 {
     const int sig_off[6] = { 105, 120, 134, 149, 152, 402 }, last_off[6] = { 166, 181, 195, 210, 213, 417 }, abs_off[6] = { 227, 237, 247, 257, 266, 426 };
     const int n_sig[6] = { 15, 14, 15, 3, 14, 15 }, n_last[6] = { 15, 14, 15, 3, 14, 9 }, n_abs[6] = { 10, 10, 10, 9, 10, 10 }, byte_of[6] = { 3, 1, 0, 3, 2, 0 };
-    if (ctx < 105) { reg = 0; lane = ctx >> 2; sh = (ctx & 3) * 8; return true; }
-    if (ctx >= 399 && ctx <= 401) { const int c = ctx - 399 + 105; reg = 0; lane = c >> 2; sh = (c & 3) * 8; return true; }
+    if (ctx < 64) { reg = 0; lane = ctx; sh = 0; return true; }
+    if (ctx < 105) { reg = 3; lane = ctx - 64; sh = 0; return true; }
+    if (ctx >= 399 && ctx <= 401) { reg = 3; lane = ctx - 399 + 41; sh = 0; return true; }
     for (int cat = 0; cat < 6; cat++) {
         int role = -1, i = 0;
         if (ctx >= sig_off[cat] && ctx < sig_off[cat] + n_sig[cat]) { role = 0; i = ctx - sig_off[cat]; }
diff --git a/x264vfw_amd/csrc/cabac_rd.hip.h b/x264vfw_amd/csrc/cabac_rd.hip.h
--- a/x264vfw_amd/csrc/cabac_rd.hip.h
+++ b/x264vfw_amd/csrc/cabac_rd.hip.h
@@ -17,7 +17,12 @@
 #include "cabac_entropy.inc"
 };
 
-struct Cab { uint32_t a, r, r8; int f8; int f8v; };
+struct Cab { uint32_t a0, a1, r, r8; int f8; int f8v; };
+
+#define CAB_STR_BITS 64
+typedef unsigned long long cab_str_t;
+struct CabStr { cab_str_t b0, b1; int room; const uint32_t *ctab; };
+__device__ __forceinline__ CabStr cab_str_begin(const uint32_t *ctab) { return CabStr{ 0, 0, CAB_STR_BITS, ctab }; }
 
 __device__ __forceinline__ uint32_t cab_model(int lane)
 {
@@ -30,7 +35,7 @@
 {
     namespace T = x264gpu_cabac;
     qp = min(max(qp, 0), 51);
-    uint32_t w[3] = { 0, 0, 0 };
+    uint32_t w[3] = { 0, 0, 0 }, wa1 = 0;
     auto seed = [&](int ctx) {
         int m = 0, n = 0;
         if (ctx < 276) { const T::CabacInitRow row = T::cabac_init_0_275[ctx]; m = pslice ? row.mp : row.mi; n = pslice ? row.np : row.ni; }
@@ -38,10 +43,8 @@
         const int pre = min(max(((m * qp) >> 4) + n, 1), 126);
         return (uint32_t)(pre <= 63 ? (63 - pre) << 1 : ((pre - 64) << 1) | 1);
     };
-    for (int j = 0; j < 4; j++) {
-        const int c = lane * 4 + j;
-        if (c < 105) w[0] |= seed(c) << (8 * j); else if (c < 108) w[0] |= seed(399 + c - 105) << (8 * j);
-    }
+    w[0] = seed(lane);
+    if (lane < 41) wa1 = seed(64 + lane); else if (lane < 44) wa1 = seed(399 + lane - 41);
     {
         const int role = lane >> 4, i = lane & 15;
         const int sig_off[5] = { 105, 120, 134, 149, 152 }, last_off[5] = { 166, 181, 195, 210, 213 }, abs_off[5] = { 227, 237, 247, 257, 266 }, n1[5] = { 15, 14, 15, 3, 14 };
@@ -60,22 +63,50 @@
         }
         if (role == 0 && i < 15) w[2] = seed(402 + i); else if (role == 1 && i < 9) w[2] = seed(417 + i); else if (role == 2 && i < 10) w[2] = seed(426 + i);
     }
-    cb.a = w[0]; cb.r = w[1]; cb.r8 = w[2]; cb.f8 = 0; cb.f8v = 0;
-}
-
-__device__ __forceinline__ void cab_bin(Cab &cb, uint32_t model, int lane, int ctx, int bin)
-{
-    ctx = __builtin_amdgcn_readfirstlane(ctx >= 399 ? ctx - 399 + 105 : ctx); bin = __builtin_amdgcn_readfirstlane(bin);
-    const int li = ctx >> 2, sh = (ctx & 3) * 8;
-    const uint32_t w = __builtin_amdgcn_readlane(cb.a, li);
-    const int st = (w >> sh) & 255, sg = st >> 1, mps = st & 1;
-    const uint32_t t = __builtin_amdgcn_readlane(model, sg);
-    const bool lps = (mps ^ bin) != 0;
-    cb.f8 += lps ? (t >> 9) & 0x7ff : t & 0x1ff;
-    const int ns = lps ? (int)(t >> 20) : min(sg + 1, 62);
-    const int nm = lps && sg == 0 ? mps ^ 1 : mps;
-    const uint32_t nw = (w & ~(255u << sh)) | ((uint32_t)((ns << 1) | nm) << sh);
-    cb.a = lane == li ? nw : cb.a;
+    cb.a0 = w[0]; cb.a1 = wa1; cb.r = w[1]; cb.r8 = w[2]; cb.f8 = 0; cb.f8v = 0;
+}
+
+__device__ __forceinline__ void cab_walk_a(Cab &cb, CabStr &s)
+{
+    int st0 = (int)(cb.a0 & 255u), n0 = (int)(cb.a0 >> 8), st1 = (int)(cb.a1 & 255u), n1 = (int)(cb.a1 >> 8);
+    while (__ballot((n0 | n1) != 0)) {
+        const int k0 = min(n0, CAB_WALK_BINS), k1 = min(n1, CAB_WALK_BINS);
+        const uint32_t e0 = s.ctab[((((1 << k0) - 1) + ((int)(unsigned)s.b0 & ((1 << k0) - 1))) << 7) + st0];
+        const uint32_t e1 = s.ctab[((((1 << k1) - 1) + ((int)(unsigned)s.b1 & ((1 << k1) - 1))) << 7) + st1];
+        st0 = (int)(e0 & 127u); st1 = (int)(e1 & 127u); cb.f8v += (int)(e0 >> 7) + (int)(e1 >> 7);
+        s.b0 >>= k0; s.b1 >>= k1; n0 -= k0; n1 -= k1;
+    }
+    cb.a0 = (uint32_t)st0; cb.a1 = (uint32_t)st1;
+    s.b0 = 0; s.b1 = 0; s.room = CAB_STR_BITS;
+}
+
+__device__ __forceinline__ void cab_reserve(Cab &cb, CabStr &s, int n) { if (s.room < n) cab_walk_a(cb, s); }
+
+__device__ __forceinline__ void cab_put_str(Cab &cb, CabStr &s, int lane, int ctx, unsigned long long bits, int n)
+{
+    ctx = __builtin_amdgcn_readfirstlane(ctx); n = __builtin_amdgcn_readfirstlane(n);
+    if (n <= 0) return;
+    const bool hi = ctx >= 64;
+    const int li = ctx >= 399 ? ctx - 399 + 41 : ctx & 63;
+    const bool mine = lane == li;
+    const cab_str_t part = (cab_str_t)bits & (n >= CAB_STR_BITS ? ~(cab_str_t)0 : (((cab_str_t)1 << n) - 1));
+    if (hi) { s.b1 |= mine ? part << (cb.a1 >> 8) : 0; cb.a1 += mine ? (uint32_t)n << 8 : 0u; }
+    else { s.b0 |= mine ? part << (cb.a0 >> 8) : 0; cb.a0 += mine ? (uint32_t)n << 8 : 0u; }
+    s.room -= n;
+}
+__device__ __forceinline__ void cab_put(Cab &cb, CabStr &s, int lane, int ctx, int bin, int n = 1)
+{
+    cab_put_str(cb, s, lane, ctx, __builtin_amdgcn_readfirstlane(bin) ? ~0ull : 0ull, n);
+}
+__device__ __forceinline__ void cab_put_any(Cab &cb, CabStr &s, int lane, int ctx, int bin, int n)
+{
+    n = __builtin_amdgcn_readfirstlane(n);
+    while (n > 0) {
+        cab_reserve(cb, s, 1);
+        const int k = min(n, s.room);
+        cab_put(cb, s, lane, ctx, bin, k);
+        n -= k;
+    }
 }
 __device__ __forceinline__ void cab_bypass(Cab &cb, int n = 1) { cb.f8 += 256 * n; }
 __device__ __forceinline__ void cab_ue_bypass(Cab &cb, int k, int v)
@@ -332,26 +363,42 @@
     return (nnz >> blkidx_of(bx, by)) & 1;
 }
 
-__device__ __forceinline__ void cab_mb_type_intra(Cab &cb, uint32_t model, int lane, const CabIn &in, int c0, int c1, int c2, int c3, int c4, int c5)
-{
-    if (in.type != X264GPU_MB_I16x16) { cab_bin(cb, model, lane, c0, 0); return; }
-    cab_bin(cb, model, lane, c0, 1);
+__device__ __forceinline__ void cab_mb_type_intra(Cab &cb, CabStr &cs, int lane, const CabIn &in, int c0, int c1, int c2, int c3, int c4, int c5)
+{
+    if (in.type != X264GPU_MB_I16x16) { cab_put(cb, cs, lane, c0, 0); return; }
+    cab_put(cb, cs, lane, c0, 1);
     if (in.size) cb.f8 += 7;
-    cab_bin(cb, model, lane, c1, in.cbp_luma != 0);
-    if (!in.cbp_chroma) cab_bin(cb, model, lane, c2, 0);
-    else { cab_bin(cb, model, lane, c2, 1); cab_bin(cb, model, lane, c3, in.cbp_chroma >> 1); }
-    cab_bin(cb, model, lane, c4, in.i16mode >> 1);
-    cab_bin(cb, model, lane, c5, in.i16mode & 1);
-}
-
-__device__ __forceinline__ void cab_mvd(Cab &cb, uint32_t model, int lane, int base, int sum, int val)
+    cab_put(cb, cs, lane, c1, in.cbp_luma != 0);
+    if (!in.cbp_chroma) cab_put(cb, cs, lane, c2, 0);
+    else { cab_put(cb, cs, lane, c2, 1); cab_put(cb, cs, lane, c3, in.cbp_chroma >> 1); }
+    cab_put(cb, cs, lane, c4, in.i16mode >> 1);
+    cab_put(cb, cs, lane, c5, in.i16mode & 1);
+}
+
+__device__ __forceinline__ void cab_mvd(Cab &cb, CabStr &cs, int lane, int base, int sum, int val)
 {
     const int a = abs(val), inc = (sum > 2) + (sum > 32);
-    if (!a) { cab_bin(cb, model, lane, base + inc, 0); return; }
-    cab_bin(cb, model, lane, base + inc, 1);
-    for (int i = 1; i < min(a, 9); i++) cab_bin(cb, model, lane, base + min(i + 2, 6), 1);
-    if (a < 9) cab_bin(cb, model, lane, base + min(a + 2, 6), 0); else cab_ue_bypass(cb, 3, a - 9);
+    if (!a) { cab_put(cb, cs, lane, base + inc, 0); return; }
+    cab_put(cb, cs, lane, base + inc, 1);
+    const int ones = min(a, 9) - 1;
+    if (a < 4) {
+        for (int i = 1; i <= ones; i++) cab_put(cb, cs, lane, base + i + 2, 1);
+        cab_put(cb, cs, lane, base + a + 2, 0);
+    } else {
+        cab_put(cb, cs, lane, base + 3, 1); cab_put(cb, cs, lane, base + 4, 1); cab_put(cb, cs, lane, base + 5, 1);
+        const int n6 = ones - 3 + (a < 9 ? 1 : 0);
+        cab_put_str(cb, cs, lane, base + 6, (1ull << (ones - 3)) - 1ull, n6);
+    }
+    if (a >= 9) cab_ue_bypass(cb, 3, a - 9);
     cab_bypass(cb);
+}
+__device__ __forceinline__ void cab_ref_idx(Cab &cb, CabStr &cs, int lane, int ctx, int r)
+{
+    if (r <= 0) { cab_put(cb, cs, lane, 54 + ctx, 0); return; }
+    cab_put(cb, cs, lane, 54 + ctx, 1);
+    if (r == 1) { cab_put(cb, cs, lane, 58, 0); return; }
+    cab_put(cb, cs, lane, 58, 1);
+    cab_put_str(cb, cs, lane, 59, (1ull << (r - 2)) - 1ull, r - 1);
 }
 
 template <class PROF>
@@ -366,14 +413,15 @@
     dqp_out = 0;
     const bool lavail = in.left, tavail = in.top;
     const bool intra = in.type < X264GPU_MB_P_L0;
+    CabStr cs = cab_str_begin(ctab);
     if (!in.pm) {
     if (in.bslice && !in.size) {
-        cab_bin(cb, model, lane, 24 + (lavail && !cab_is_skip(in.ltype)) + (tavail && !cab_is_skip(in.ttype)), in.type == X264GPU_MB_B_SKIP);
-        if (in.type == X264GPU_MB_B_SKIP) return 0;
+        cab_put(cb, cs, lane, 24 + (lavail && !cab_is_skip(in.ltype)) + (tavail && !cab_is_skip(in.ttype)), in.type == X264GPU_MB_B_SKIP);
+        if (in.type == X264GPU_MB_B_SKIP) { cab_walk_a(cb, cs); return 0; }
     }
     if (in.pslice && !in.bslice && !in.size) {
-        cab_bin(cb, model, lane, 11 + (lavail && in.ltype != X264GPU_MB_P_SKIP) + (tavail && in.ttype != X264GPU_MB_P_SKIP), in.type == X264GPU_MB_P_SKIP);
-        if (in.type == X264GPU_MB_P_SKIP) return 0;
+        cab_put(cb, cs, lane, 11 + (lavail && in.ltype != X264GPU_MB_P_SKIP) + (tavail && in.ttype != X264GPU_MB_P_SKIP), in.type == X264GPU_MB_P_SKIP);
+        if (in.type == X264GPU_MB_P_SKIP) { cab_walk_a(cb, cs); return 0; }
     }
     if (in.bslice) {
         const int ctx0 = (lavail && in.ltype != X264GPU_MB_B_SKIP && in.ltype != X264GPU_MB_B_DIRECT) + (tavail && in.ttype != X264GPU_MB_B_SKIP && in.ttype != X264GPU_MB_B_DIRECT);
@@ -388,50 +436,61 @@
             value = 4 + 2 * pair + (in.part == D_8x16);
         }
         const int len = c_btype_len[value], bits = c_btype_bits[value];
-        for (int i = 0; i < len; i++) cab_bin(cb, model, lane, i == 0 ? 27 + ctx0 : i == 1 ? 27 + 3 : i == 2 ? 27 + 5 - ((bits >> 1) & 1) : 27 + 5, (bits >> i) & 1);
-        if (intra) cab_mb_type_intra(cb, model, lane, in, 32, 32 + 1, 32 + 2, 32 + 2, 32 + 3, 32 + 3);
+        cab_put(cb, cs, lane, 27 + ctx0, bits & 1);
+        if (len > 1) {
+            cab_put(cb, cs, lane, 27 + 3, (bits >> 1) & 1);
+            cab_put(cb, cs, lane, 27 + 5 - ((bits >> 1) & 1), (bits >> 2) & 1);
+            if (len > 3) cab_put_str(cb, cs, lane, 27 + 5, (unsigned long long)(bits >> 3), len - 3);
+        }
+        if (intra) cab_mb_type_intra(cb, cs, lane, in, 32, 32 + 1, 32 + 2, 32 + 2, 32 + 3, 32 + 3);
     } else if (!in.pslice) {
         const int ctx = (lavail && in.ltype != X264GPU_MB_I4x4 && in.ltype != X264GPU_MB_I8x8) + (tavail && in.ttype != X264GPU_MB_I4x4 && in.ttype != X264GPU_MB_I8x8);
-        cab_mb_type_intra(cb, model, lane, in, 3 + ctx, 3 + 3, 3 + 4, 3 + 5, 3 + 6, 3 + 7);
-    } else if (intra) { cab_bin(cb, model, lane, 14, 1); cab_mb_type_intra(cb, model, lane, in, 17, 17 + 1, 17 + 2, 17 + 2, 17 + 3, 17 + 3); }
-    else if (in.part == D_8x8) { cab_bin(cb, model, lane, 14, 0); cab_bin(cb, model, lane, 15, 0); cab_bin(cb, model, lane, 16, 1); }
+        cab_mb_type_intra(cb, cs, lane, in, 3 + ctx, 3 + 3, 3 + 4, 3 + 5, 3 + 6, 3 + 7);
+    } else if (intra) { cab_put(cb, cs, lane, 14, 1); cab_mb_type_intra(cb, cs, lane, in, 17, 17 + 1, 17 + 2, 17 + 2, 17 + 3, 17 + 3); }
+    else if (in.part == D_8x8) { cab_put(cb, cs, lane, 14, 0); cab_put(cb, cs, lane, 15, 0); cab_put(cb, cs, lane, 16, 1); }
     else {
-        cab_bin(cb, model, lane, 14, 0);
-        if (in.part == D_16x16) { cab_bin(cb, model, lane, 15, 0); cab_bin(cb, model, lane, 16, 0); }
-        else { cab_bin(cb, model, lane, 15, 1); cab_bin(cb, model, lane, 17, in.part == D_16x8); }
+        cab_put(cb, cs, lane, 14, 0);
+        if (in.part == D_16x16) { cab_put(cb, cs, lane, 15, 0); cab_put(cb, cs, lane, 16, 0); }
+        else { cab_put(cb, cs, lane, 15, 1); cab_put(cb, cs, lane, 17, in.part == D_16x8); }
     }
     }
     const int t8ctx = 399 + (lavail && in.lt8) + (tavail && in.tt8);
     if (in.pm == 1) {
-        if (in.pm_lists & 1) { cab_mvd(cb, model, lane, 40, in.pm_sx, in.pm_dx); cab_mvd(cb, model, lane, 47, in.pm_sy, in.pm_dy); }
-        if (in.pm_lists & 2) { cab_mvd(cb, model, lane, 40, in.pm_sx1, in.pm_dx1); cab_mvd(cb, model, lane, 47, in.pm_sy1, in.pm_dy1); }
-        if (in.part == D_8x8 && !in.bslice) cab_bin(cb, model, lane, 21, 1);
+        if (in.pm_lists & 1) { cab_mvd(cb, cs, lane, 40, in.pm_sx, in.pm_dx); cab_mvd(cb, cs, lane, 47, in.pm_sy, in.pm_dy); }
+        if (in.pm_lists & 2) { cab_mvd(cb, cs, lane, 40, in.pm_sx1, in.pm_dx1); cab_mvd(cb, cs, lane, 47, in.pm_sy1, in.pm_dy1); }
+        if (in.part == D_8x8 && !in.bslice) cab_put(cb, cs, lane, 21, 1);
     } else if (intra) {
         if (in.type != X264GPU_MB_I16x16 && (!in.pm || in.pm == 2 || in.pm == 3)) {
             const bool i8 = in.type == X264GPU_MB_I8x8;
-            if (in.t8mode && !in.pm) cab_bin(cb, model, lane, t8ctx, i8);
+            if (in.t8mode && !in.pm) cab_put(cb, cs, lane, t8ctx, i8);
             int mode = 0, pm = 0;
             if (lane < 16) { const uint8_t *cur = i8 ? modes8 : modes4; mode = cur[lane]; pm = i4_pred_mode(nmodes, mbx, sy, lane, cur); }
-            const uint32_t w68 = __builtin_amdgcn_readlane(cb.a, 68 >> 2);
-            int stp = lane == 0 ? (int)(w68 & 255) : (int)((w68 >> 8) & 255);
-            for (int b = 0; b < 16; b += i8 ? 4 : 1) {
-                if (in.pm && b != (i8 ? 4 * in.pm_b0 : in.pm_b0)) continue;
-                int m = __builtin_amdgcn_readlane(mode, b);
-                const int p = __builtin_amdgcn_readlane(pm, b);
-                const bool same = m == p;
-                if (m > p) m--;
-                cab_step(stp, cb.f8v, model, lane == 0 || (lane == 1 && !same), lane == 0 ? same : m & 1);
-                if (!same) { cab_step(stp, cb.f8v, model, lane == 1, (m >> 1) & 1); cab_step(stp, cb.f8v, model, lane == 1, m >> 2); }
-            }
-            {
-                const uint32_t s68 = (uint32_t)__builtin_amdgcn_readlane(stp, 0), s69 = (uint32_t)__builtin_amdgcn_readlane(stp, 1);
-                cb.a = lane == (68 >> 2) ? (cb.a & ~0xffffu) | s68 | (s69 << 8) : cb.a;
-            }
+            const bool sends = lane < 16 && (!i8 || !(lane & 3)) && (!in.pm || lane == (i8 ? 4 * in.pm_b0 : in.pm_b0));
+            const bool same = mode == pm;
+            const int rem = mode > pm ? mode - 1 : mode;
+            const unsigned long long sm = __ballot(sends), fm = __ballot(sends && same), rm = sm & ~fm;
+            unsigned long long s68 = fm;
+            if (i8) s68 = (fm & 1ull) | ((fm >> 3) & 2ull) | ((fm >> 6) & 4ull) | ((fm >> 9) & 8ull);
+            if (in.pm) s68 = fm ? 1ull : 0ull;
+            const int dst = sends && !same ? 3 * cab_mbcnt(rm) : 63;
+            const int p0 = __builtin_amdgcn_ds_permute(dst << 2, sends && !same ? rem & 1 : 0);
+            const int p1 = __builtin_amdgcn_ds_permute((dst == 63 ? 63 : dst + 1) << 2, sends && !same ? (rem >> 1) & 1 : 0);
+            const int p2 = __builtin_amdgcn_ds_permute((dst == 63 ? 63 : dst + 2) << 2, sends && !same ? (rem >> 2) & 1 : 0);
+            const unsigned long long s69 = __ballot((p0 | p1 | p2) != 0);
+            const int n68 = __builtin_popcountll(sm), n69 = 3 * __builtin_popcountll(rm);
+            if (!in.pm) {
+                if (cs.room < max(n68, n69)) cab_walk_a(cb, cs);
+                const int room = cs.room;
+                cs.room = CAB_STR_BITS;
+                cab_put_str(cb, cs, lane, 68, s68, n68); cab_put_str(cb, cs, lane, 69, s69, n69);
+                cs.room = room - max(n68, n69);
+            } else { cab_put_str(cb, cs, lane, 68, s68, n68); cab_put_str(cb, cs, lane, 69, s69, n69); }
         }
         if (!in.pm || in.pm == 4) {
+        cab_reserve(cb, cs, 3);
         const int ctx = (lavail && in.ltype < X264GPU_MB_P_L0 && in.lcmode != 0) + (tavail && in.ttype < X264GPU_MB_P_L0 && in.tcmode != 0);
-        if (!in.cmode) cab_bin(cb, model, lane, 64 + ctx, 0);
-        else { cab_bin(cb, model, lane, 64 + ctx, 1); cab_bin(cb, model, lane, 64 + 3, in.cmode > 1); if (in.cmode > 1) cab_bin(cb, model, lane, 64 + 3, in.cmode > 2); }
+        if (!in.cmode) cab_put(cb, cs, lane, 64 + ctx, 0);
+        else { cab_put(cb, cs, lane, 64 + ctx, 1); cab_put(cb, cs, lane, 64 + 3, in.cmode > 1); if (in.cmode > 1) cab_put(cb, cs, lane, 64 + 3, in.cmode > 2); }
         }
     } else if (in.bslice) {
         if (in.type != X264GPU_MB_B_DIRECT) {
@@ -441,10 +500,10 @@
             if (part == D_8x8)
                 for (int kp = 0; kp < 4; kp++) {
                     const int u = use_of(kp);
-                    if (u == 3) { cab_bin(cb, model, lane, 36, 0); continue; }
-                    cab_bin(cb, model, lane, 36, 1);
-                    if (u == 2) { cab_bin(cb, model, lane, 37, 1); cab_bin(cb, model, lane, 38, 0); cab_bin(cb, model, lane, 39, 0); cab_bin(cb, model, lane, 39, 0); }
-                    else { cab_bin(cb, model, lane, 37, 0); cab_bin(cb, model, lane, 39, u == 1); }
+                    if (u == 3) { cab_put(cb, cs, lane, 36, 0); continue; }
+                    cab_put(cb, cs, lane, 36, 1);
+                    if (u == 2) { cab_put(cb, cs, lane, 37, 1); cab_put(cb, cs, lane, 38, 0); cab_put(cb, cs, lane, 39, 0, 2); }
+                    else { cab_put(cb, cs, lane, 37, 0); cab_put(cb, cs, lane, 39, u == 1); }
                 }
             const int sc0 = S.cref, sc1 = S.cmvx, sc2 = S.cmvy, sc3 = S.cdir;
             for (int l = 0; l < 2; l++) {
@@ -458,8 +517,7 @@
                     const int r = rl(l ? in.b_r1 : in.b_r0, b8 * 16);
                     if (sends) {
                         int ctx = (rl(S.cref, g0 - 1) > 0 && !rl(S.cdir, g0 - 1)) + 2 * (rl(S.cref, g0 - 4) > 0 && !rl(S.cdir, g0 - 4));
-                        for (int q = r; q > 0; q--) { cab_bin(cb, model, lane, 54 + ctx, 1); ctx = (ctx >> 2) + 4; }
-                        cab_bin(cb, model, lane, 54 + ctx, 0);
+                        cab_reserve(cb, cs, 16); cab_ref_idx(cb, cs, lane, ctx, r);
                     }
                     const bool mine = lane == g0 || (w8 == 2 && lane == g0 + 1) || (h8 == 2 && lane == g0 + 4) || (w8 == 2 && h8 == 2 && lane == g0 + 5);
                     S.cref = mine ? (sends ? r : u == 3 ? r : -1) : S.cref;
@@ -480,11 +538,12 @@
                     if (sends) {
                         int px, py;
                         mb_predict_mv(S, part, x8, y8, w8, r, px, py, go);
+                        cab_reserve(cb, cs, 18);
                         for (int comp = 0; comp < 2; comp++) {
                             const int la = x8 > 0 ? (int)((am >> (8 * ((y8 * 2 + x8 - 1) * 2 + comp))) & 255) : lavail ? (int)((nl >> (8 * ((y8 * 2 + 1) * 2 + comp))) & 255) : 0;
                             const int ta = y8 > 0 ? (int)((am >> (8 * (((y8 - 1) * 2 + x8) * 2 + comp))) & 255) : tavail ? (int)((nt >> (8 * ((2 + x8) * 2 + comp))) & 255) : 0;
                             const int d = comp ? vy - py : vx - px;
-                            cab_mvd(cb, model, lane, comp ? 47 : 40, la + ta, d);
+                            cab_mvd(cb, cs, lane, comp ? 47 : 40, la + ta, d);
                             const unsigned long long capped = (unsigned long long)min(abs(d), 66);
                             for (int yy = y8; yy < y8 + h8; yy++) for (int xx = x8; xx < x8 + w8; xx++) am |= capped << (8 * ((yy * 2 + xx) * 2 + comp));
                         }
@@ -500,7 +559,7 @@
     } else {
         const int part = in.part, np = part == D_16x16 ? 1 : part == D_8x8 ? 4 : 2;
         const int w8 = part == D_16x16 || part == D_16x8 ? 2 : 1, h8 = part == D_16x16 || part == D_8x16 ? 2 : 1;
-        if (part == D_8x8) for (int kp = 0; kp < 4; kp++) cab_bin(cb, model, lane, 21, 1);
+        if (part == D_8x8) cab_put(cb, cs, lane, 21, 1, 4);
         const int sc0 = S.cref, sc1 = S.cmvx, sc2 = S.cmvy;
         if (lane == 5 || lane == 6 || lane == 9 || lane == 10) S.cref = -2;
         if (in.nref > 1)
@@ -508,9 +567,8 @@
                 const int x8 = part == D_8x16 ? kp : part == D_8x8 ? kp & 1 : 0, y8 = part == D_16x8 ? kp : part == D_8x8 ? kp >> 1 : 0;
                 const int slot = part == D_16x16 ? ME_16 : part == D_16x8 ? ME_16x8 + kp : part == D_8x16 ? ME_8x16 + kp : ME_8 + kp;
                 const int r = rl(S.ref, slot), g0 = (y8 + 1) * 4 + x8 + 1;
-                int ctx = (rl(S.cref, g0 - 1) > 0) + 2 * (rl(S.cref, g0 - 4) > 0);
-                for (int q = r; q > 0; q--) { cab_bin(cb, model, lane, 54 + ctx, 1); ctx = (ctx >> 2) + 4; }
-                cab_bin(cb, model, lane, 54 + ctx, 0);
+                const int ctx = (rl(S.cref, g0 - 1) > 0) + 2 * (rl(S.cref, g0 - 4) > 0);
+                cab_reserve(cb, cs, 16); cab_ref_idx(cb, cs, lane, ctx, r);
                 const bool mine = lane == g0 || (w8 == 2 && lane == g0 + 1) || (h8 == 2 && lane == g0 + 4) || (w8 == 2 && h8 == 2 && lane == g0 + 5);
                 S.cref = mine ? r : S.cref;
             }
@@ -521,11 +579,12 @@
             const int r = rl(S.ref, slot), vx = rl(S.mvx, slot), vy = rl(S.mvy, slot), g0 = (y8 + 1) * 4 + x8 + 1;
             int px, py;
             mb_predict_mv(S, part, x8, y8, w8, r, px, py);
+            cab_reserve(cb, cs, 18);
             for (int comp = 0; comp < 2; comp++) {
                 const int la = x8 > 0 ? (int)((amvd >> (8 * ((y8 * 2 + x8 - 1) * 2 + comp))) & 255) : lavail ? (int)((in.lamvd >> (8 * ((y8 * 2 + 1) * 2 + comp))) & 255) : 0;
                 const int ta = y8 > 0 ? (int)((amvd >> (8 * (((y8 - 1) * 2 + x8) * 2 + comp))) & 255) : tavail ? (int)((in.tamvd >> (8 * ((2 + x8) * 2 + comp))) & 255) : 0;
                 const int d = comp ? vy - py : vx - px;
-                cab_mvd(cb, model, lane, comp ? 47 : 40, la + ta, d);
+                cab_mvd(cb, cs, lane, comp ? 47 : 40, la + ta, d);
                 const unsigned long long capped = (unsigned long long)min(abs(d), 66);
                 for (int yy = y8; yy < y8 + h8; yy++) for (int xx = x8; xx < x8 + w8; xx++) amvd |= capped << (8 * ((yy * 2 + xx) * 2 + comp));
             }
@@ -534,30 +593,33 @@
         }
         S.cref = sc0; S.cmvx = sc1; S.cmvy = sc2;
     }
+    cab_reserve(cb, cs, 7);
     if (in.pm ? in.pm == 3 : in.type != X264GPU_MB_I16x16)
         for (int b8 = 0; b8 < 4; b8++) {
             const int x = b8 & 1, y = b8 >> 1;
             const int a = x ? !((in.cbp_luma >> (b8 - 1)) & 1) : lavail ? !((in.lcbp_luma >> (b8 + 1)) & 1) : 0;
             const int b = y ? !((in.cbp_luma >> (b8 - 2)) & 1) : tavail ? !((in.tcbp_luma >> (b8 + 2)) & 1) : 0;
-            cab_bin(cb, model, lane, 73 + a + 2 * b, (in.cbp_luma >> b8) & 1);
+            cab_put(cb, cs, lane, 73 + a + 2 * b, (in.cbp_luma >> b8) & 1);
         }
     if (in.pm ? in.pm == 4 : in.type != X264GPU_MB_I16x16) {
-        cab_bin(cb, model, lane, 77 + (lavail && in.lcbp_chroma) + 2 * (tavail && in.tcbp_chroma), in.cbp_chroma != 0);
-        if (in.cbp_chroma) cab_bin(cb, model, lane, 77 + 4 + (lavail && in.lcbp_chroma == 2) + 2 * (tavail && in.tcbp_chroma == 2), in.cbp_chroma == 2);
-    }
-    if (!in.pm && !intra && in.t8mode && in.cbp_luma) cab_bin(cb, model, lane, t8ctx, in.t8);
+        cab_put(cb, cs, lane, 77 + (lavail && in.lcbp_chroma) + 2 * (tavail && in.tcbp_chroma), in.cbp_chroma != 0);
+        if (in.cbp_chroma) cab_put(cb, cs, lane, 77 + 4 + (lavail && in.lcbp_chroma == 2) + 2 * (tavail && in.tcbp_chroma == 2), in.cbp_chroma == 2);
+    }
+    if (!in.pm && !intra && in.t8mode && in.cbp_luma) cab_put(cb, cs, lane, t8ctx, in.t8);
     if (in.pm || in.cbp_luma || in.cbp_chroma || in.type == X264GPU_MB_I16x16) {
         const bool i16 = !in.pm && in.type == X264GPU_MB_I16x16;
         int dqp = in.qp - in.last_qp;
         if (i16 && !in.cbp_luma && !in.cbp_chroma && !((in.nnz >> 24) & 1) && dqp > 0) dqp = 0;
         if (!in.pm) {
-        int ctx = in.last_dqp != 0;
+        const int ctx = in.last_dqp != 0;
+        if (dqp < -26) dqp += 52; else if (dqp > 25) dqp -= 52;
+        const int val = dqp > 0 ? 2 * dqp - 1 : -2 * dqp;
+        cab_reserve(cb, cs, val + 1);
         if (dqp) {
-            if (dqp < -26) dqp += 52; else if (dqp > 25) dqp -= 52;
-            int val = dqp > 0 ? 2 * dqp - 1 : -2 * dqp;
-            do { cab_bin(cb, model, lane, 60 + ctx, 1); ctx = 2 + (ctx >> 1); } while (--val);
-        }
-        cab_bin(cb, model, lane, 60 + ctx, 0);
+            cab_put(cb, cs, lane, 60 + ctx, 1);
+            if (val == 1) cab_put(cb, cs, lane, 62, 0);
+            else { cab_put(cb, cs, lane, 62, 1); cab_put_str(cb, cs, lane, 63, (1ull << (val - 2)) - 1ull, val - 1); }
+        } else cab_put(cb, cs, lane, 60 + ctx, 0);
         dqp_out = dqp;
         }
         pf.mark2(17);
@@ -592,11 +654,12 @@
             constexpr int CAT = decltype(cat_tag)::value;
             static_assert(CAT == 0 || CAT == 3, "the DC categories");
             (void)shift;
+            cab_reserve(cb, cs, nblk);
             for (int b = 0; b < nblk; b++) {
                 if (!coded(b)) continue;
                 const int coef = coef_of(b);
                 const bool nz = __ballot(coef != 0) != 0;
-                cab_bin(cb, model, lane, 85 + CAT * 4 + inc_of(b), nz);
+                cab_put(cb, cs, lane, 85 + CAT * 4 + inc_of(b), nz);
                 if (nz) { if (CAT == 0) W.ldc = true; else W.nzdc |= 1u << b; }
             }
         };
@@ -607,25 +670,18 @@
             const bool mine_blk = lane < nblk && ((codedmask >> b_lane) & 1);
             const int inc = inc_of(b_lane);
             const unsigned long long nzm = (unsigned long long)(nzbits & codedmask);
-            unsigned long long seq = 0;
-#pragma unroll
-            for (int j = 0; j < 4; j++) { const unsigned long long m = __ballot(mine_blk && inc == j); seq = lane == j ? m : seq; }
-            const int cbase = 85 + CAT * 4;
-            int stc = 0;
-#pragma unroll
-            for (int j = 0; j < 4; j++) { const int c = cbase + j; const uint32_t w = __builtin_amdgcn_readlane(cb.a, c >> 2); stc = lane == j ? (int)((w >> ((c & 3) * 8)) & 255) : stc; }
-            while (__ballot(seq != 0)) {
-                const bool have = seq != 0;
-                const int b = have ? __builtin_ctzll(seq) : 0;
-                cab_step(stc, cb.f8v, model, have, (int)((nzm >> b) & 1));
-                seq &= seq - 1;
-            }
+            cab_reserve(cb, cs, nblk);
+            unsigned long long mem[4];
+            int pushed[4];
 #pragma unroll
             for (int j = 0; j < 4; j++) {
-                const int c = cbase + j, li = c >> 2, sh = (c & 3) * 8;
-                const uint32_t v = (uint32_t)__builtin_amdgcn_readlane(stc, j);
-                cb.a = lane == li ? (cb.a & ~(255u << sh)) | (v << sh) : cb.a;
-            }
+                const bool m = mine_blk && inc == j;
+                mem[j] = __ballot(m);
+                pushed[j] = __builtin_amdgcn_ds_permute((m ? cab_mbcnt(mem[j]) : 63) << 2, m ? (int)((nzm >> b_lane) & 1) : 0);
+            }
+#pragma unroll
+            for (int j = 0; j < 4; j++)
+                if (mem[j]) cab_put_str(cb, cs, lane, 85 + CAT * 4 + j, __ballot(pushed[j] != 0), __builtin_popcountll(mem[j]));
             (void)coef_of; (void)shift;
             if (CAT == 4) W.nzac |= (unsigned)nzm; else { W.cat0 = CAT; W.nz0 |= (unsigned)nzm; }
         };
@@ -658,8 +714,9 @@
             if (in.cbp_chroma == 2)
                 blocks_many(std::integral_constant<int, 4>{}, 16, 8, 0xffu, (in.nnz >> 16) & 0xffu, [&](int k) { return lane < 15 ? (int)lvs[X264GPU_LV_CHROMA_AC + k * 16 + 1 + lane] : 0; }, [&](int k) { return ac_inc((k >> 2) & 1, k & 3); });
         }
+        cab_walk_a(cb, cs);
         flush_levels();
-    }
+    } else cab_walk_a(cb, cs);
     return amvd;
 }
 
diff --git a/x264vfw_amd/csrc/encoder.hip b/x264vfw_amd/csrc/encoder.hip
--- a/x264vfw_amd/csrc/encoder.hip
+++ b/x264vfw_amd/csrc/encoder.hip
@@ -171,7 +171,7 @@
     for (int r = 1; r < (cfg->dpb > 0 ? 8 : cfg->refs); r++) alloc((void **)&e->mvr[r], S * k.nmb * 2 * sizeof(int16_t), 0);
     alloc((void **)&e->wf_progress, S * 2 * WFG_ROWS * sizeof(int), 0);
     if (cfg->rd && !cfg->cabac) alloc((void **)&e->tc, S * k.nmb * 24, 0);
-    if (cfg->rd && cfg->cabac) { alloc((void **)&e->amvd, S * k.nmb * (cfg->dpb > 0 ? 16 : 8), 0); alloc((void **)&e->cab_out, S * (cfg->slices > 1 ? cfg->slices : 1) * 192 * sizeof(uint32_t), 0); }
+    if (cfg->rd && cfg->cabac) { alloc((void **)&e->amvd, S * k.nmb * (cfg->dpb > 0 ? 16 : 8), 0); alloc((void **)&e->cab_out, S * (cfg->slices > 1 ? cfg->slices : 1) * 256 * sizeof(uint32_t), 0); }
     if (S >= 512 && !getenv("X264GPU_NO_BALANCE")) { alloc((void **)&e->perm, S * sizeof(int), 0); alloc((void **)&e->wtime, 4 * S * sizeof(unsigned), 0); }
     if (cfg->slices_plain && cfg->slices > 1) { alloc((void **)&e->sl_stat, 3 * S * cfg->slices * 4 * sizeof(int), 0);       alloc((void **)&e->sl_rerun, S * cfg->slices * sizeof(int), 0); }
 #ifdef MB_PROF
@@ -333,9 +333,9 @@
 {
     ARG_TRY(e && out460 && stream >= 0 && stream < e->cfg.streams && slice >= 0 && slice < (e->cfg.slices > 1 ? e->cfg.slices : 1));
     if (!e->cab_out) return X264GPU_EINVAL;
-    uint32_t w[192];
+    uint32_t w[256];
     HIP_TRY(hipDeviceSynchronize());
-    HIP_TRY(hipMemcpy(w, e->cab_out + ((size_t)stream * (e->cfg.slices > 1 ? e->cfg.slices : 1) + slice) * 192, sizeof(w), hipMemcpyDeviceToHost));
+    HIP_TRY(hipMemcpy(w, e->cab_out + ((size_t)stream * (e->cfg.slices > 1 ? e->cfg.slices : 1) + slice) * 256, sizeof(w), hipMemcpyDeviceToHost));
     for (int c = 0; c < 460; c++) {
         int reg, lane, sh;
         out460[c] = cab_locate(c, reg, lane, sh) ? (uint8_t)(w[reg * 64 + lane] >> sh) : 0;
diff --git a/x264vfw_amd/csrc/k_mb.hip.h b/x264vfw_amd/csrc/k_mb.hip.h
--- a/x264vfw_amd/csrc/k_mb.hip.h
+++ b/x264vfw_amd/csrc/k_mb.hip.h
@@ -1464,7 +1464,7 @@
     __builtin_amdgcn_s_waitcnt(0); __builtin_amdgcn_wave_barrier();
 #endif
     int last_qp = uni((int)k.mbqp[(size_t)s * k.nmb + mb_first]);
-    Cab cab = { 0, 0, 0, 0, 0 };
+    Cab cab = { 0, 0, 0, 0, 0, 0 };
     uint32_t cab_modelv = 0;
     int last_dqp = 0;
     if constexpr (RD >= 2) { cab_init(cab, lane, pslice, last_qp); cab_modelv = cab_model(lane); }
@@ -2973,7 +2973,7 @@
     if (PS && k.sl_stat && lane == 0) { int *st = k.sl_stat + ((size_t)s * nsl + blockIdx.y) * 4; st[0] = intra_count - L.slw[2]; st[1] = L.slw[0]; st[2] = L.slw[1]; }
     if (k.wtime && lane == 0 && blockIdx.y == 0) k.wtime[s] = (unsigned)min((unsigned long long)(__builtin_readcyclecounter() - wt0) >> 6, 0xffffffffull);
     if constexpr (RD >= 2) {
-        if (k.cab_out) { uint32_t *o = k.cab_out + ((size_t)s * (k.slices > 1 ? k.slices : 1) + blockIdx.y) * 192; o[lane] = cab.a; o[64 + lane] = cab.r; o[128 + lane] = cab.r8; }
+        if (k.cab_out) { uint32_t *o = k.cab_out + ((size_t)s * (k.slices > 1 ? k.slices : 1) + blockIdx.y) * 256; o[lane] = cab.a0; o[64 + lane] = cab.r; o[128 + lane] = cab.r8; o[192 + lane] = cab.a1; }
     }
 #ifdef MB_PROF
     if (lane == 0 && k.prof) for (int i = 0; i < 32; i++) k.prof[(size_t)s * 32 + i] = pf.acc[i];
diff --git a/x264vfw_amd/csrc/prim_kernels.hip b/x264vfw_amd/csrc/prim_kernels.hip
--- a/x264vfw_amd/csrc/prim_kernels.hip
+++ b/x264vfw_amd/csrc/prim_kernels.hip
@@ -459,7 +459,7 @@
     const int i = blockIdx.x, lane = threadIdx.x;
     for (int j = lane; j < X264GPU_MB_LEVELS; j += 64) l[j] = lv[(size_t)i * X264GPU_MB_LEVELS + j];
     __syncthreads();
-    Cab cb; cb.a = 0; cb.r = r_in[i * 64 + lane]; cb.r8 = r8_in[i * 64 + lane]; cb.f8 = 0; cb.f8v = 0;
+    Cab cb; cb.a0 = 0; cb.a1 = 0; cb.r = r_in[i * 64 + lane]; cb.r8 = r8_in[i * 64 + lane]; cb.f8 = 0; cb.f8v = 0;
     const uint32_t model = cab_model(lane);
     CabLv W = { what[i * 5], (unsigned)what[i * 5 + 1], (unsigned)what[i * 5 + 2], (unsigned)what[i * 5 + 3], what[i * 5 + 4] != 0 };
     Prof pf;
@@ -481,3 +481,41 @@
     return X264GPU_OK;
 }
 }
+
+namespace x264gpu {
+__global__ void k_cab_bins_walk(const int32_t *triples, const int32_t *first, const uint8_t *st_in, uint8_t *st_out, int *bits, const uint32_t *ctab)
+{
+    const int i = blockIdx.x, lane = threadIdx.x;
+    const uint8_t *si = st_in + (size_t)i * 460;
+    uint8_t *so = st_out + (size_t)i * 460;
+    const int c0 = lane, c1 = lane < 41 ? 64 + lane : lane < 44 ? 399 + lane - 41 : -1;
+    Cab cb; cb.a0 = si[c0] & 127u; cb.a1 = c1 >= 0 ? si[c1] & 127u : 0u;
+    cb.r = 0; cb.r8 = 0; cb.f8 = 0; cb.f8v = 0;
+    CabStr cs = cab_str_begin(ctab);
+    const int t0 = __builtin_amdgcn_readfirstlane(first[i]), t1 = __builtin_amdgcn_readfirstlane(first[i + 1]);
+    for (int t = t0; t < t1; t++) {
+        const int ctx = __builtin_amdgcn_readfirstlane(triples[3 * t]), bin = __builtin_amdgcn_readfirstlane(triples[3 * t + 1]) & 1;
+        const int rep = __builtin_amdgcn_readfirstlane(triples[3 * t + 2]);
+        if (!((ctx >= 0 && ctx < 105) || (ctx >= 399 && ctx <= 401))) continue;
+        cab_put_any(cb, cs, lane, ctx, bin, rep);
+    }
+    cab_walk_a(cb, cs);
+    for (int c = lane; c < 460; c += 64) if (c >= 105 && !(c >= 399 && c <= 401)) so[c] = si[c];
+    so[c0] = (uint8_t)cb.a0;
+    if (c1 >= 0) so[c1] = (uint8_t)cb.a1;
+    const int total = cab_total(cb);
+    if (lane == 0) bits[i] = total;
+}
+}
+extern "C" {
+int x264gpu_cabac_bins_walk(const int32_t *d_triples, const int32_t *d_first, int n, const uint8_t *d_states, uint8_t *d_states_out, int32_t *d_bits, void *stream)
+{
+    ARG_TRY(d_triples && d_first && d_states && d_states_out && d_bits && n >= 0);
+    if (!n) return X264GPU_OK;
+    const uint32_t *ctab = nullptr;
+    { const int rc = x264gpu::cabac_chain_table(&ctab); if (rc != X264GPU_OK) return rc; }
+    hipLaunchKernelGGL(x264gpu::k_cab_bins_walk, dim3(n), dim3(64), 0, (hipStream_t)stream, d_triples, d_first, d_states, d_states_out, d_bits, ctab);
+    HIP_TRY(hipGetLastError());
+    return X264GPU_OK;
+}
+}
diff --git a/x264vfw_amd/lib.py b/x264vfw_amd/lib.py
--- a/x264vfw_amd/lib.py
+++ b/x264vfw_amd/lib.py
@@ -140,6 +140,7 @@
     "x264gpu_nr_update": (_i, [_vp, _vp, _vp, _i, _i, _vp]),
     "x264gpu_denoise_blocks": (_i, [_vp, _i, _i, _vp, _vp, _vp]),
     "x264gpu_cabac_level_walk": (_i, [_vp, _vp, _i, _vp, _vp, _vp, _vp, _vp, _vp]),
+    "x264gpu_cabac_bins_walk": (_i, [_vp, _vp, _i, _vp, _vp, _vp, _vp]),
     "x264gpu_encoder_deblock_pictures": (_i, [_vp, _vp, _vp, _vp, _vp]),
     "x264gpu_get_device": (_i, [_vp]),
     "x264gpu_lookahead_create": (_i, [C.POINTER(_vp), _i, _i, _i, _i, _i]),
```

New measurement: 757.0, median of 6. 1.02x the previous value.
